# lukedan/libfluid

Hardware: AMD Instinct MI355X
Metric: particle_steps_per_sec (higher is better)
Workload: dtype f32

## Files before the change

libfluid_amd/csrc/common.h:

```cpp
#pragma once

#include <hip/hip_runtime.h>
#include <stdint.h>

#include <string>
#include <vector>

#include "../../include/libfluid_amd.h"
#include "slots.h"

hipError_t lfa_pool_malloc(void **p, size_t bytes);
hipError_t lfa_pool_free(void *p);
void lfa_pool_nosync_begin();
void lfa_pool_nosync_end();
template <typename T> inline hipError_t lfa_hip_malloc(T **p, size_t bytes) { return lfa_pool_malloc((void **)p, bytes); }
#define hipMalloc(p, n) lfa_hip_malloc((p), (n))
#define hipFree(p) lfa_pool_free((void *)(p))
struct lfa_stream_set;
lfa_stream_set *lfa_pool_take_set(int device);
void lfa_pool_park_set(lfa_stream_set *q);

#define LFA_TILE 8
#define LFA_TILE_CELLS 512
#define LFA_HALO 10
#define LFA_HALO_CELLS 1000
#define LFA_WAVE 64

#define CT_AIR 1
#define CT_FLUID 2
#define CT_SOLID 4
#define CT_OUTSIDE 0x80

#define AB_UNKNOWN 0x40
#define AB_FLUID 0x80

struct ParticleSoA {
	uint32_t *key = nullptr;
	float *t[3] = {nullptr, nullptr, nullptr};
	float *v[3] = {nullptr, nullptr, nullptr};
	float *c[9] = {nullptr};
	uint32_t *id = nullptr;
	void *base = nullptr;
};

#define LFA_CLOSED_MAX_UNKNOWNS 64

struct GridDims {
	int nx, ny, nz;
	int ntx, nty, ntz;
	int nt;
};

struct lfa_knobs {
	int mg_no_persist = 0;
	int mg_dist_single = 0;
	int mg_co_fault = 0;
	int mg_no_top = 0;
	int mg_no_prune = 0;
	int mg_dist_levels = 0;
	int mg_no_closed = 0;
	int mg_no_tagged = 0;
};

struct lfa_sim {
	int device = 0;
	lfa_knobs knobs;
	hipStream_t stream = nullptr;
	hipStream_t stream2 = nullptr;
	hipEvent_t ev_fork = nullptr, ev_join = nullptr;
	hipStream_t stream3 = nullptr;
	hipEvent_t ev_cfork = nullptr, ev_cjoin = nullptr;
	bool overlap_correction = true;
	bool corr_in_flight = false;
	bool counts_fresh = false;
	bool move_pending = false;
	bool corr_begun = false;
	bool corr_undo_valid = false;
	uint32_t *corr_ovf = nullptr;
	int corr_parts_tiles = 0;
	GridDims g{};
	size_t nc = 0, ncp = 0;
	lfa_params prm{};
	std::string err;

	size_t np = 0, pcap = 0;
	ParticleSoA pb[2];
	int cur = 0;
	uint32_t *rank = nullptr;
	bool binned = false;

	struct lfa_dist *dist = nullptr;
	int slab_lo = 0, slab_hi = 0;
	int slab_align = 0;
	int *ptiles_all = nullptr;
	int p_off = 0, n_ptiles_all = 0;
	int n_own_first = 0, n_own_last = 0;
	int n_ghost_lo = 0, n_ghost_hi = 0;
	int *halo_tiles = nullptr;
	int n_halo[4] = {0, 0, 0, 0};
	void *xbuf[4] = {nullptr, nullptr, nullptr, nullptr};
	size_t xcap[4] = {0, 0, 0, 0};
	double *dist_red = nullptr;
	size_t np_live = 0;
	bool holes = false;
	size_t arrivals_at = 0, n_arrivals = 0;
	size_t ghost_at[2] = {0, 0}, n_ghost_particles = 0;

	uint32_t *tile_count = nullptr, *tile_start = nullptr;
	uint32_t *tile_flag = nullptr, *tile_scan = nullptr;
	uint32_t *grid_flag = nullptr;
	int *ptiles = nullptr, *dtiles = nullptr;
	int *tile_pslot = nullptr;
	int n_ptiles = 0, n_dtiles = 0;
	uint32_t *scan_tmp = nullptr;
	size_t scan_tmp_len = 0;
	uint32_t *h_pinned = nullptr;

	float *u = nullptr, *v = nullptr, *w = nullptr;
	float *uo = nullptr, *vo = nullptr, *wo = nullptr;
	uint8_t *ctype = nullptr, *solid = nullptr;
	uint32_t *cell_count = nullptr;
// ... 211 lines not shown
struct IngestParams {
	double off[3], h;
};
inline IngestParams lfa_ingest_params(const lfa_sim *s) {
	IngestParams ip;
	for (int k = 0; k < 3; ++k) ip.off[k] = s->prm.grid_offset[k];
	ip.h = s->prm.cell_size;
	return ip;
}

__device__ inline void cell_and_fraction(double pos, double off, double h, int n, int &cell, float &t) {
	double gp = (pos - off) / h;
	double m = gp < 0.0 ? 0.0 : gp;
	int c = m >= (double)n ? n - 1 : (int)m;
	if (c > n - 1) c = n - 1;
	double td = gp - (double)c;
	float tf = (float)td;
	if (!(tf > 0.0f)) tf = 0.0f;
	if (td < 1.0 && tf >= 1.0f) tf = 0.99999994f;
	if (tf > 1.0f) tf = 1.0f;
	cell = c;
	t = tf;
}

__device__ inline void particle_world_position(const GridDims &g, const IngestParams &ip, uint32_t b, float t0, float t1, float t2,
                                               double (&x)[3]) {
	int c[3];
	cell_coords(g, b, c);
	const float t[3] = {t0, t1, t2};
#pragma unroll
	for (int k = 0; k < 3; ++k) x[k] = ip.off[k] + ((double)c[k] + (double)t[k]) * ip.h;
}

__device__ inline void particle_zero_c_set_id(const ParticleSoA &p, size_t d, uint32_t id) {
#pragma unroll
	for (int k = 0; k < 9; ++k) p.c[k][d] = 0.0f;
	p.id[d] = id;
}

#define TC_CHUNKS 8
template <int CH>
__device__ inline void lfa_wave_tile_ranks(const uint32_t (&tile)[CH], uint32_t *tile_count, uint32_t (&my_rank)[CH]) {
	const int lane = threadIdx.x & 63;
	const unsigned long long lt = (1ull << lane) - 1ull;
	unsigned long long todo[CH];
#pragma unroll
	for (int c = 0; c < CH; ++c) {
		todo[c] = __ballot(tile[c] != 0xFFFFFFFFu);
		my_rank[c] = 0;
	}
	for (;;) {
		uint32_t t = 0xFFFFFFFFu;
		bool found = false;
#pragma unroll
		for (int c = 0; c < CH; ++c)
			if (!found && todo[c]) {
				t = __shfl(tile[c], __ffsll((long long)todo[c]) - 1, 64);
				found = true;
			}
		if (!found) break;
		unsigned long long same[CH];
		uint32_t total = 0;
#pragma unroll
		for (int c = 0; c < CH; ++c) {
			same[c] = __ballot(tile[c] == t) & todo[c];
			total += (uint32_t)__popcll(same[c]);
// ... 146 lines not shown
```

libfluid_amd/csrc/core.hip:

```cpp
#include <math.h>

#include <algorithm>
#include <stdarg.h>
#include <stdio.h>
#include <string.h>

#include <mutex>

#include "common.h"
#include "pcg.h"
#include "stream_set.h"

static thread_local std::string g_create_error;

int lfa_fail(lfa_sim *s, int code, const char *fmt, ...) {
	char buf[512];
	va_list ap;
	va_start(ap, fmt);
	vsnprintf(buf, sizeof buf, fmt, ap);
	va_end(ap);
	if (s) s->err = buf;
	else g_create_error = buf;
	return code;
}
// ... 288 lines not shown
		rc = lfa_fail(s, LFA_E_HIP, "hipHostMalloc failed");
	if (rc == LFA_OK) {
		hipLaunchKernelGGL(k_init_ctype, dim3((unsigned)((s->ncp + 255) / 256)), dim3(256), 0, s->stream, s->ctype,
		                   s->solid, s->g, s->ncp);
		if (hipGetLastError() != hipSuccess || hipStreamSynchronize(s->stream) != hipSuccess)
			rc = lfa_fail(s, LFA_E_HIP, "grid initialisation kernel failed (is the code object built for this GPU?)");
	}
	if (rc != LFA_OK) {
		g_create_error = s->err;
		lfa_destroy(s);
		return rc;
	}
	lfa_co_gate_handle(device, +1);
	s->gate_counted = true;
	*out = s;
	return LFA_OK;
}

static void free_soa(ParticleSoA &p) {
	if (p.base) (void)hipFree(p.base);
	p = ParticleSoA();
}

extern "C" void lfa_destroy(lfa_sim *s) {
	if (!s) return;
	(void)hipSetDevice(s->device);
	if (s->gate_counted) lfa_co_gate_handle(s->device, -1);
	if (s->stream) (void)hipStreamSynchronize(s->stream);
	if (s->stream2) (void)hipStreamSynchronize(s->stream2);
	if (s->stream3) (void)hipStreamSynchronize(s->stream3);
	lfa_pool_nosync_begin();
	free_soa(s->pb[0]);
	free_soa(s->pb[1]);
	void *ptrs[] = {s->c_home, s->fine_start, s->corr_ovf, s->tile_clear, s->tile_epoch, s->tile_closed, s->src_cell, s->src_lo, s->src_target, s->src_of, s->src_need, s->src_vel, s->src_slab.words, s->coerce_map, s->grid_flag, s->rank, s->vc_src, s->tile_count, s->tile_start, s->tile_flag, s->tile_scan, s->ptiles_all, s->dtiles, s->halo_tiles, s->dist_red,
	                s->xbuf[0], s->xbuf[1], s->xbuf[2], s->xbuf[3],
	                s->tile_pslot, s->scan_tmp, s->u, s->v, s->w, s->uo, s->vo, s->wo, s->ctype, s->solid,
	                s->cell_count, s->stage, s->acc, s->abits, s->vp, s->vr, s->vz, s->vs, s->vpre, s->vq, s->vs2, s->c_as, s->nbr_table,
	                s->partials, s->frame_part, s->pcg_state, s->pcg_hist, s->level_tiles, s->io_buf, s->raw_scan, s->c_diag, s->c_w[0],
	                s->c_w[1], s->c_w[2], s->c_unk, s->c_pre, s->c_r, s->c_x, s->c_r2, s->c_x2, s->a2inv, s->slot_l1,
	                s->l1_tiles, s->l1_l2, s->tracers.base};
	for (void *p : ptrs)
		if (p) (void)hipFree(p);
	if (s->dist) delete s->dist;
	s->dist = nullptr;
	lfa_mg_free(s);
	lfa_pool_nosync_end();
	for (hipEvent_t e : s->frame_ev)
		if (e) (void)hipEventDestroy(e);
	for (hipEvent_t e : s->sample_ev)
		if (e) (void)hipEventDestroy(e);
	for (hipEvent_t e : s->tracers.ev)
		if (e) (void)hipEventDestroy(e);
	if (s->stream && s->stream2 && s->stream3 && s->ev_fork && s->ev_join && s->ev_cfork && s->ev_cjoin && s->h_pinned) {
		lfa_stream_set *q = new lfa_stream_set();
		q->device = s->device;
		q->stream = s->stream; q->stream2 = s->stream2; q->stream3 = s->stream3;
		q->ev_fork = s->ev_fork; q->ev_join = s->ev_join; q->ev_cfork = s->ev_cfork; q->ev_cjoin = s->ev_cjoin;
		for (int i = 0; i < LFA_EV_COUNT; ++i) q->ev[i] = s->ev[i];
		q->ev_created = s->ev_created;
		q->h_pinned = s->h_pinned;
		lfa_pool_park_set(q);
	} else {
		if (s->h_pinned) (void)hipHostFree(s->h_pinned);
		if (s->ev_created)
			for (auto &e : s->ev) (void)hipEventDestroy(e);
		if (s->ev_fork) (void)hipEventDestroy(s->ev_fork);
		if (s->ev_join) (void)hipEventDestroy(s->ev_join);
// ... 32 lines not shown
	s->prm = *p;
	return LFA_OK;
}
extern "C" int lfa_get_params(const lfa_sim *s, lfa_params *p) {
	if (!s || !p) return LFA_E_INVALID;
	*p = s->prm;
	return LFA_OK;
}
extern "C" int lfa_synchronize(lfa_sim *s) {
	if (!s) return LFA_E_INVALID;
	LFA_HIP(s, hipStreamSynchronize(s->stream));
	if (s->corr_in_flight) LFA_HIP(s, hipStreamSynchronize(s->stream3));
	return LFA_OK;
}
extern "C" void *lfa_stream(lfa_sim *s) { return s ? (void *)s->stream : nullptr; }
extern "C" uint64_t lfa_num_particles(const lfa_sim *s) { return s ? s->np : 0; }

int lfa_ensure_io(lfa_sim *s, size_t bytes) {
	if (bytes <= s->io_cap) return LFA_OK;
	if (s->io_buf) LFA_HIP(s, hipFree(s->io_buf));
	s->io_buf = nullptr;
	s->io_cap = 0;
	hipError_t e = hipMalloc(&s->io_buf, bytes);
	if (e != hipSuccess) return lfa_fail(s, LFA_E_OOM, "hipMalloc(%zu) for the boundary buffer failed", bytes);
	s->io_cap = bytes;
	return LFA_OK;
}

static int alloc_soa(lfa_sim *s, ParticleSoA &p, size_t cap) {
	p = ParticleSoA();
	hipError_t e = hipMalloc(&p.base, cap * 17 * 4);
	if (e != hipSuccess) return lfa_fail(s, LFA_E_OOM, "hipMalloc of particle SoA (%zu particles) failed", cap);
	float *f = (float *)p.base;
	p.key = (uint32_t *)f;
	for (int k = 0; k < 3; ++k) p.t[k] = f + cap * (1 + k);
	for (int k = 0; k < 3; ++k) p.v[k] = f + cap * (4 + k);
	for (int k = 0; k < 9; ++k) p.c[k] = f + cap * (7 + k);
	p.id = (uint32_t *)(f + cap * 16);
	return LFA_OK;
}

int lfa_particles_alloc(lfa_sim *s, size_t n) {
	if (n <= s->pcap) return LFA_OK;
	LFA_HIP(s, hipStreamSynchronize(s->stream));
	const size_t cap = (n + 1023) & ~(size_t)1023;
	ParticleSoA nb[2];
	uint32_t *rank = nullptr, *vc_src = nullptr;
	int rc = alloc_soa(s, nb[0], cap);
	if (rc == LFA_OK) rc = alloc_soa(s, nb[1], cap);
	if (rc == LFA_OK && hipMalloc(&rank, cap * 4) != hipSuccess) rc = lfa_fail(s, LFA_E_OOM, "hipMalloc of the rank array failed");
	if (rc == LFA_OK && hipMalloc(&vc_src, cap * 4) != hipSuccess) rc = lfa_fail(s, LFA_E_OOM, "hipMalloc of the source-index array failed");
	if (rc != LFA_OK) {
		free_soa(nb[0]);
		free_soa(nb[1]);
		if (rank) (void)hipFree(rank);
		if (vc_src) (void)hipFree(vc_src);
		return rc;
	}
	free_soa(s->pb[0]);
	free_soa(s->pb[1]);
	if (s->rank) (void)hipFree(s->rank);
	if (s->vc_src) (void)hipFree(s->vc_src);
	s->pb[0] = nb[0];
	s->pb[1] = nb[1];
	s->rank = rank;
	s->vc_src = vc_src;
	s->vc_pending = false;
	s->pcap = cap;
	return LFA_OK;
}

int lfa_particles_reserve(lfa_sim *s, size_t n_keep, size_t n_total) {
	if (n_total <= s->pcap) return LFA_OK;
	LFA_TRY(lfa_particles_materialize(s));
	LFA_HIP(s, hipStreamSynchronize(s->stream));
	const size_t cap = ((n_total + n_total / 8) + 1023) & ~(size_t)1023;
	ParticleSoA keep = s->pb[s->cur];
	const size_t old_cap = s->pcap;
	s->pb[s->cur] = ParticleSoA();
	s->pcap = 0;
	int rc = lfa_particles_alloc(s, cap);
	if (rc != LFA_OK) {
		s->pb[s->cur] = keep;
		s->pcap = old_cap;
		return rc;
	}
	ParticleSoA &dst = s->pb[s->cur];
	const uint32_t *src_arrays[17];
	uint32_t *dst_arrays[17];
	src_arrays[0] = keep.key; dst_arrays[0] = dst.key;
	for (int k = 0; k < 3; ++k) { src_arrays[1 + k] = (uint32_t *)keep.t[k]; dst_arrays[1 + k] = (uint32_t *)dst.t[k]; }
	for (int k = 0; k < 3; ++k) { src_arrays[4 + k] = (uint32_t *)keep.v[k]; dst_arrays[4 + k] = (uint32_t *)dst.v[k]; }
	for (int k = 0; k < 9; ++k) { src_arrays[7 + k] = (uint32_t *)keep.c[k]; dst_arrays[7 + k] = (uint32_t *)dst.c[k]; }
	src_arrays[16] = keep.id; dst_arrays[16] = dst.id;
	for (int a = 0; a < 17; ++a)
		if (n_keep) LFA_HIP(s, hipMemcpyAsync(dst_arrays[a], src_arrays[a], n_keep * 4, hipMemcpyDeviceToDevice, s->stream));
	LFA_HIP(s, hipStreamSynchronize(s->stream));
	free_soa(keep);
	return LFA_OK;
}

__global__ void k_ingest(const double *aos, size_t n, ParticleSoA p, GridDims g, IngestParams ip, int slab_lo, int slab_hi) {
	size_t i = (size_t)blockIdx.x * blockDim.x + threadIdx.x;
	if (i >= n) return;
	const double *q = aos + i * 19;
	int c[3];
	float t[3];
	cell_and_fraction(q[0], ip.off[0], ip.h, g.nx, c[0], t[0]);
	cell_and_fraction(q[1], ip.off[1], ip.h, g.ny, c[1], t[1]);
	cell_and_fraction(q[2], ip.off[2], ip.h, g.nz, c[2], t[2]);
	p.key[i] = ((c[2] >> 3) >= slab_lo && (c[2] >> 3) < slab_hi) ? blocked_index(g, c[0], c[1], c[2]) : 0xFFFFFFFFu;
#pragma unroll
	for (int k = 0; k < 3; ++k) {
		p.t[k][i] = t[k];
		p.v[k][i] = (float)q[3 + k];
	}
#pragma unroll
	for (int k = 0; k < 9; ++k) p.c[k][i] = (float)q[6 + k];
	p.id[i] = (uint32_t)i;
}

extern "C" int lfa_upload_particles(lfa_sim *s, const void *aos152, uint64_t n) {
	if (!s || (!aos152 && n)) return LFA_E_INVALID;
	s->vc_pending = false;
	s->c_home_valid = false;
	s->move_pending = false;
	s->vmax2_valid = false;
	if (!(s->prm.cell_size > 0.0)) return lfa_fail(s, LFA_E_INVALID, "set cell_size (lfa_set_params) before uploading");
	if (n >= ((uint64_t)1 << 32)) return lfa_fail(s, LFA_E_INVALID, "more than 2^32 particles");
	LFA_HIP(s, hipSetDevice(s->device));
	LFA_TRY(lfa_corr_commit(s));
	LFA_TRY(lfa_particles_alloc(s, n));
	s->np = n;
	s->np_live = n;
	s->next_global_id = n;
	s->binned = false;
	s->system_valid = false;
	s->unknown_count_valid = false;
	s->cur = 0;
	if (n == 0) return LFA_OK;
	LFA_TRY(lfa_ensure_io(s, n * 152));
	LFA_HIP(s, hipMemcpyAsync(s->io_buf, aos152, n * 152, hipMemcpyHostToDevice, s->stream));
	const IngestParams ip = lfa_ingest_params(s);
	hipLaunchKernelGGL(k_ingest, dim3((unsigned)((n + 255) / 256)), dim3(256), 0, s->stream, (const double *)s->io_buf,
	                   (size_t)n, s->pb[0], s->g, ip, s->slab_lo, s->slab_hi);
	LFA_LAUNCH_CHECK(s);
	LFA_HIP(s, hipStreamSynchronize(s->stream));
	return LFA_OK;
}

__global__ void k_valid_flags(const uint32_t *key, size_t n, uint32_t *valid) {
	size_t i = (size_t)blockIdx.x * blockDim.x + threadIdx.x;
	if (i < n) valid[i] = key[i] != 0xFFFFFFFFu ? 1u : 0u;
}
__global__ void k_export_ids(const uint32_t *key, const uint32_t *id, const uint32_t *slot, size_t n, uint32_t *out) {
	size_t i = (size_t)blockIdx.x * blockDim.x + threadIdx.x;
	if (i < n && key[i] != 0xFFFFFFFFu) out[slot ? slot[i] : i] = id[i];
}

__global__ void k_export(double *aos, size_t n, ParticleSoA p, GridDims g, IngestParams ip, int flags, int by_slot, const uint32_t *slot,
                         ParticleSoA old, int have_old, const float *c_home, size_t c_home_stride) {
	size_t i = (size_t)blockIdx.x * blockDim.x + threadIdx.x;
	if (i >= n) return;
	uint32_t b = p.key[i];
	if (slot && b == 0xFFFFFFFFu) return;
	double *q = aos + (by_slot ? (slot ? (size_t)slot[i] : i) : (size_t)p.id[i]) * 19;
	if (flags & LFA_DL_POSITIONS) {
		double x[3];
		particle_world_position(g, ip, b, p.t[0][i], p.t[1][i], p.t[2][i], x);
#pragma unroll
		for (int k = 0; k < 3; ++k) {
			q[k] = x[k];
			q[15 + k] = x[k];
		}
		if (have_old) {
			particle_world_position(g, ip, old.key[i], old.t[0][i], old.t[1][i], old.t[2][i], x);
#pragma unroll
			for (int k = 0; k < 3; ++k) q[15 + k] = x[k];
		}
	}
#pragma unroll
	for (int k = 0; k < 3; ++k) q[3 + k] = (double)p.v[k][i];
#pragma unroll
	for (int k = 0; k < 9; ++k) q[6 + k] = (double)(c_home ? c_home[k * c_home_stride + p.id[i]] : p.c[k][i]);
	if (!(flags & LFA_DL_KEEP_RAW)) ((uint64_t *)q)[18] = raw_from_blocked(g, b);
}

int lfa_slab_download_slots(lfa_sim *s, const uint32_t **slot) {
	*slot = nullptr;
	if (!s->dist || !s->holes || !s->np_live) return LFA_OK;
	hipLaunchKernelGGL(k_valid_flags, dim3((unsigned)((s->np_live + 255) / 256)), dim3(256), 0, s->stream, (const uint32_t *)s->pb[s->cur].key,
	                   s->np_live, s->rank);
	LFA_LAUNCH_CHECK(s);
	uint32_t *tot = (uint32_t *)(s->pcg_state + LFA_DW_SCAN_TOTAL);
	LFA_TRY(lfa_exclusive_scan_u32(s, s->rank, s->rank, s->np_live, tot));
	uint32_t h = 0;
	LFA_HIP(s, hipMemcpyAsync(&h, tot, 4, hipMemcpyDeviceToHost, s->stream));
	LFA_HIP(s, hipStreamSynchronize(s->stream));
	if ((size_t)h != s->np) return lfa_fail(s, LFA_E_INVALID, "slab download: %u resident records but %zu expected", h, s->np);
	*slot = s->rank;
	return LFA_OK;
}

__global__ void __launch_bounds__(256) k_close_holes(size_t n, ParticleSoA src, ParticleSoA dst, const uint32_t *slot, size_t n_dst) {
	const size_t i = (size_t)blockIdx.x * 256 + threadIdx.x;
	if (i >= n || src.key[i] == 0xFFFFFFFFu) return;
	const size_t d = slot[i];
	if (d >= n_dst) return;
	dst.key[d] = src.key[i];
#pragma unroll
	for (int k = 0; k < 3; ++k) {
		dst.t[k][d] = src.t[k][i];
		dst.v[k][d] = src.v[k][i];
	}
#pragma unroll
	for (int k = 0; k < 9; ++k) dst.c[k][d] = src.c[k][i];
	dst.id[d] = src.id[i];
}

int lfa_particles_close_holes(lfa_sim *s, size_t n_rec) {
	hipLaunchKernelGGL(k_valid_flags, dim3((unsigned)((n_rec + 255) >> 8)), dim3(256), 0, s->stream, (const uint32_t *)s->pb[s->cur].key,
	                   n_rec, s->rank);
	LFA_LAUNCH_CHECK(s);
	size_t n_dst = 0;
	LFA_TRY(lfa_scan_total(s, s->rank, s->rank, n_rec, (uint32_t *)(s->pcg_state + LFA_DW_SCAN_TOTAL), LFA_PIN_RESIDENT, &n_dst));
	if (s->binned && n_dst != s->np) return lfa_fail(s, LFA_E_INVALID, "seeding: %u resident records but %zu expected", (uint32_t)n_dst, s->np);
	hipLaunchKernelGGL(k_close_holes, dim3((unsigned)((n_rec + 255) >> 8)), dim3(256), 0, s->stream, n_rec, s->pb[s->cur], s->pb[s->cur ^ 1],
	                   (const uint32_t *)s->rank, n_dst);
	LFA_LAUNCH_CHECK(s);
	s->cur ^= 1;
	s->binned = false;
	s->np = s->np_live = n_dst;
	s->holes = false;
	return LFA_OK;
}

extern "C" int lfa_download_particles(lfa_sim *s, void *aos152, uint64_t n, int flags) {
	if (!s || (!aos152 && n)) return LFA_E_INVALID;
	LFA_HIP(s, hipSetDevice(s->device));
	LFA_TRY(lfa_particles_materialize(s));
	if (n != s->np) return lfa_fail(s, LFA_E_INVALID, "download of %llu particles but %zu are resident",
	                                (unsigned long long)n, s->np);
	if (n == 0) return LFA_OK;
	if (s->dist && !s->binned)
		return lfa_fail(s, LFA_E_INVALID, "slab decomposition: call lfa_hash_particles before downloading particles");
	LFA_TRY(lfa_corr_join(s));
	const uint32_t *slot = nullptr;
	LFA_TRY(lfa_slab_download_slots(s, &slot));
	LFA_TRY(lfa_ensure_io(s, n * 152));
	LFA_HIP(s, hipMemcpyAsync(s->io_buf, aos152, n * 152, hipMemcpyHostToDevice, s->stream));
	const IngestParams ip = lfa_ingest_params(s);
	const size_t n_rec = s->binned ? s->np_live : s->np;
	hipLaunchKernelGGL(k_export, dim3((unsigned)((n_rec + 255) / 256)), dim3(256), 0, s->stream, (double *)s->io_buf,
	                   n_rec, s->pb[s->cur], s->g, ip, flags, s->dist ? 1 : 0, slot, s->pb[s->cur ^ 1],
	                   (s->move_pending && !s->dist) ? 1 : 0, s->c_home_valid ? (const float *)s->c_home : (const float *)nullptr,
	                   s->c_home_cap);
	LFA_LAUNCH_CHECK(s);
	LFA_HIP(s, hipMemcpyAsync(aos152, s->io_buf, n * 152, hipMemcpyDeviceToHost, s->stream));
	LFA_HIP(s, hipStreamSynchronize(s->stream));
	return LFA_OK;
}

extern "C" int lfa_download_particle_ids(lfa_sim *s, uint32_t *ids, uint64_t n) {
	if (!s || (!ids && n)) return LFA_E_INVALID;
	LFA_HIP(s, hipSetDevice(s->device));
	if (n != s->np) return lfa_fail(s, LFA_E_INVALID, "download of %llu ids but %zu particles are resident", (unsigned long long)n, s->np);
	if (n == 0) return LFA_OK;
	LFA_TRY(lfa_corr_join(s));
	if (!s->dist) {
		for (uint64_t i = 0; i < n; ++i) ids[i] = (uint32_t)i;
		return LFA_OK;
	}
	if (!s->binned) return lfa_fail(s, LFA_E_INVALID, "slab decomposition: call lfa_hash_particles before downloading ids");
	const uint32_t *slot = nullptr;
	LFA_TRY(lfa_slab_download_slots(s, &slot));
	if (slot) {
		LFA_TRY(lfa_ensure_io(s, n * 4));
		hipLaunchKernelGGL(k_export_ids, dim3((unsigned)((s->np_live + 255) / 256)), dim3(256), 0, s->stream, (const uint32_t *)s->pb[s->cur].key,
		                   (const uint32_t *)s->pb[s->cur].id, slot, s->np_live, (uint32_t *)s->io_buf);
		LFA_LAUNCH_CHECK(s);
		LFA_HIP(s, hipMemcpyAsync(ids, s->io_buf, n * 4, hipMemcpyDeviceToHost, s->stream));
		LFA_HIP(s, hipStreamSynchronize(s->stream));
		return LFA_OK;
	}
	LFA_HIP(s, hipMemcpyAsync(ids, s->pb[s->cur].id, n * 4, hipMemcpyDeviceToHost, s->stream));
	LFA_HIP(s, hipStreamSynchronize(s->stream));
	return LFA_OK;
}

__device__ inline uint64_t splitmix64(uint64_t x) {
	x ^= x >> 30; x *= 0xBF58476D1CE4E5B9ull;
	x ^= x >> 27; x *= 0x94D049BB133111EBull;
	x ^= x >> 31;
	return x;
}
__global__ void k_seed_block(size_t n, size_t first, ParticleSoA p, GridDims g, IngestParams ip, int lox, int loy, int loz,
                             int ex, int ey, uint64_t seed, int global_ids) {
	size_t j = (size_t)blockIdx.x * blockDim.x + threadIdx.x;
	if (j >= n) return;
	const size_t i = j + first;
	size_t ci = i >> 3;
	int sub = (int)(i & 7);
	int cell[3] = {lox + (int)(ci % ex), loy + (int)((ci / ex) % ey), loz + (int)(ci / ((size_t)ex * ey))};
	int sb[3] = {sub & 1, (sub >> 1) & 1, (sub >> 2) & 1};
	int c[3];
	float t[3];
	const int nn[3] = {g.nx, g.ny, g.nz};
#pragma unroll
	for (int a = 0; a < 3; ++a) {
		uint64_t ctr = 3ull * (uint64_t)i + (uint64_t)a;
		uint64_t x = seed + (ctr + 1ull) * 0x9E3779B97F4A7C15ull;
		double uu = (double)(splitmix64(x) >> 11) * (1.0 / 9007199254740992.0);
		double pos = ip.off[a] + ((double)cell[a] + ((double)sb[a] + uu) * 0.5) * ip.h;
		cell_and_fraction(pos, ip.off[a], ip.h, nn[a], c[a], t[a]);
	}
	p.key[j] = blocked_index(g, c[0], c[1], c[2]);
#pragma unroll
	for (int k = 0; k < 3; ++k) {
		p.t[k][j] = t[k];
		p.v[k][j] = 0.0f;
	}
	particle_zero_c_set_id(p, j, (uint32_t)(global_ids ? i : j));
}

extern "C" int lfa_seed_block(lfa_sim *s, const int64_t lo[3], const int64_t hi[3], uint64_t seed) {
	if (!s || !lo || !hi) return LFA_E_INVALID;
	LFA_TRY(lfa_corr_commit(s));
	LFA_TRY(lfa_particles_materialize(s));
	if (!(s->prm.cell_size > 0.0)) return lfa_fail(s, LFA_E_INVALID, "set cell_size before seeding");
	const int nn[3] = {s->g.nx, s->g.ny, s->g.nz};
	for (int a = 0; a < 3; ++a)
		if (lo[a] < 0 || hi[a] > nn[a] || lo[a] >= hi[a]) return lfa_fail(s, LFA_E_INVALID, "seed block outside the grid");
	int64_t zlo = lo[2], zhi = hi[2];
	if (s->dist) {
		zlo = zlo > (int64_t)s->slab_lo * 8 ? zlo : (int64_t)s->slab_lo * 8;
		zhi = zhi < (int64_t)s->slab_hi * 8 ? zhi : (int64_t)s->slab_hi * 8;
		if (zhi < zlo) zhi = zlo;
	}
	const size_t per_layer = (size_t)(hi[0] - lo[0]) * (size_t)(hi[1] - lo[1]) * 8;
	const size_t n = per_layer * (size_t)(zhi - zlo), first = per_layer * (size_t)(zlo - lo[2]);
	if (per_layer * (size_t)(hi[2] - lo[2]) >= ((size_t)1 << 32)) return lfa_fail(s, LFA_E_INVALID, "more than 2^32 particles");
	LFA_HIP(s, hipSetDevice(s->device));
	LFA_TRY(lfa_particles_alloc(s, n));
	s->next_global_id = per_layer * (size_t)(hi[2] - lo[2]);
	s->np = n;
	s->np_live = n;
	s->c_home_valid = false;
	s->vmax2_valid = false;
	s->binned = false;
	s->grid_valid = false;
	s->system_valid = false;
	s->unknown_count_valid = false;
	s->cur = 0;
	const IngestParams ip = lfa_ingest_params(s);
// ... 84 lines not shown
	if (!s->uo) return lfa_fail(s, LFA_E_INVALID, "no old grid: FLIP P2G has not run");
	return export_cells(s, aos32, s->uo, s->vo, s->wo, true);
}

__global__ void k_import_cells(const CellAos *in, GridDims g, size_t nc, float *u, float *v, float *w, uint8_t *ctype,
                               uint8_t *solid) {
	size_t r = (size_t)blockIdx.x * blockDim.x + threadIdx.x;
	if (r >= nc) return;
	int x = (int)(r % g.nx), y = (int)((r / g.nx) % g.ny), z = (int)(r / ((size_t)g.nx * g.ny));
	uint32_t b = blocked_index(g, x, y, z);
	CellAos c = in[r];
	u[b] = (float)c.vel[0]; v[b] = (float)c.vel[1]; w[b] = (float)c.vel[2];
	ctype[b] = c.type & 7;
	solid[b] = (c.type & CT_SOLID) ? 1 : 0;
}

extern "C" int lfa_upload_cells(lfa_sim *s, const void *aos32) {
	if (!s || !aos32) return LFA_E_INVALID;
	++s->solid_epoch;
	LFA_HIP(s, hipSetDevice(s->device));
	LFA_TRY(lfa_corr_join(s));
	LFA_TRY(lfa_ensure_io(s, s->nc * 32));
	LFA_HIP(s, hipMemcpyAsync(s->io_buf, aos32, s->nc * 32, hipMemcpyHostToDevice, s->stream));
	hipLaunchKernelGGL(k_import_cells, dim3((unsigned)((s->nc + 255) / 256)), dim3(256), 0, s->stream,
	                   (const CellAos *)s->io_buf, s->g, s->nc, s->u, s->v, s->w, s->ctype, s->solid);
	LFA_LAUNCH_CHECK(s);
	LFA_HIP(s, hipStreamSynchronize(s->stream));
	s->grid_valid = false;
	s->bg[0] = s->bg[1] = s->bg[2] = 0.0;
	s->system_valid = false;
	return LFA_OK;
}

__global__ void __launch_bounds__(256) k_tile_count(const uint32_t *key, size_t n, uint32_t *tile_count, uint32_t *rank) {
	const int lane = threadIdx.x & 63;
	const size_t wave = ((size_t)blockIdx.x * blockDim.x + threadIdx.x) >> 6;
	const size_t i0 = wave * (64 * TC_CHUNKS) + lane;
	uint32_t tile[TC_CHUNKS], my_rank[TC_CHUNKS];
#pragma unroll
	for (int c = 0; c < TC_CHUNKS; ++c) {
		const size_t i = i0 + 64 * c;
		const uint32_t k = i < n ? key[i] : 0xFFFFFFFFu;
		tile[c] = k != 0xFFFFFFFFu ? k >> 9 : 0xFFFFFFFFu;
	}
	lfa_wave_tile_ranks(tile, tile_count, my_rank);
#pragma unroll
	for (int c = 0; c < TC_CHUNKS; ++c) {
		const size_t i = i0 + 64 * c;
		if (tile[c] != 0xFFFFFFFFu) rank[i] = my_rank[c];
	}
}

__global__ void k_tile_flags(const uint32_t *tile_count, uint32_t *flag, int nt) {
	int t = blockIdx.x * blockDim.x + threadIdx.x;
	if (t < nt) flag[t] = tile_count[t] > 0 ? 1u : 0u;
}
__global__ void k_compact_tiles(const uint32_t *flag, const uint32_t *scan, int *list, int *slot_of, int nt) {
	int t = blockIdx.x * blockDim.x + threadIdx.x;
	if (t >= nt) return;
	if (flag[t]) {
		list[scan[t]] = t;
		if (slot_of) slot_of[t] = (int)scan[t];
	} else if (slot_of) {
		slot_of[t] = -1;
	}
}
__global__ void k_dilate(const int *ptiles, int n_ptiles, uint32_t *flag, GridDims g) {
	int i = blockIdx.x * blockDim.x + threadIdx.x;
	if (i >= n_ptiles * 27) return;
	int t = ptiles[i / 27], o = i % 27, tx, ty, tz;
	tile_coords(g, t, tx, ty, tz);
	int x = tx + o % 3 - 1, y = ty + (o / 3) % 3 - 1, z = tz + o / 9 - 1;
	if ((unsigned)x < (unsigned)g.ntx && (unsigned)y < (unsigned)g.nty && (unsigned)z < (unsigned)g.ntz)
		flag[x + g.ntx * (y + g.nty * z)] = 1u;
}

__global__ void k_tile_scatter(size_t n, ParticleSoA src, ParticleSoA dst, const uint32_t *rank,
                               const uint32_t *tile_start, const uint32_t *tile_count, int shuffle, uint32_t *from) {
	size_t i = (size_t)blockIdx.x * blockDim.x + threadIdx.x;
	if (i >= n) return;
	uint32_t key = src.key[i], tile = key >> 9, r = rank[i];
	if (key == 0xFFFFFFFFu) return;
	if (shuffle) {
		uint32_t cnt = tile_count[tile];
		if (cnt % 1000003u != 0) r = (uint32_t)(((uint64_t)r * 1000003ull) % cnt);
	}
	size_t d = (size_t)tile_start[tile] + r;
	dst.key[d] = key;
#pragma unroll
	for (int k = 0; k < 3; ++k) dst.t[k][d] = src.t[k][i];
	dst.id[d] = src.id[i];
	from[d] = (uint32_t)i;
}
__global__ void k_c_to_home(size_t n, ParticleSoA p, float *home, size_t stride) {
	size_t i = (size_t)blockIdx.x * blockDim.x + threadIdx.x;
	if (i >= n || p.key[i] == 0xFFFFFFFFu) return;
	const size_t j = p.id[i];
#pragma unroll
	for (int k = 0; k < 9; ++k) home[k * stride + j] = p.c[k][i];
}
__global__ void k_c_from_home(size_t n, ParticleSoA p, const float *home, size_t stride) {
	size_t i = (size_t)blockIdx.x * blockDim.x + threadIdx.x;
	if (i >= n || p.key[i] == 0xFFFFFFFFu) return;
	const size_t j = p.id[i];
#pragma unroll
	for (int k = 0; k < 9; ++k) p.c[k][i] = home[k * stride + j];
}
__global__ void k_gather_vc(size_t n, ParticleSoA old, ParticleSoA cur, const uint32_t *from, int with_c) {
	size_t d = (size_t)blockIdx.x * blockDim.x + threadIdx.x;
	if (d >= n) return;
	const uint32_t i = from[d];
#pragma unroll
	for (int k = 0; k < 3; ++k) cur.v[k][d] = old.v[k][i];
	if (with_c) {
#pragma unroll
		for (int k = 0; k < 9; ++k) cur.c[k][d] = old.c[k][i];
	}
}

#define CC_UNROLL 16
__global__ void __launch_bounds__(256)
k_cell_count(const int *dtiles, int n_dtiles, const uint32_t *key, const uint32_t *tile_start, uint32_t *cell_count) {
	__shared__ uint32_t cnt[LFA_TILE_CELLS];
	for (int slot = blockIdx.x; slot < n_dtiles; slot += gridDim.x) {
		int tile = dtiles[slot];
		cnt[threadIdx.x] = 0;
		cnt[threadIdx.x + 256] = 0;
		__syncthreads();
		uint32_t b = tile_start[tile], e = tile_start[tile + 1];
		for (uint32_t base = b + threadIdx.x; base - threadIdx.x < e; base += 256 * CC_UNROLL) {
			uint32_t k[CC_UNROLL];
#pragma unroll
			for (int q = 0; q < CC_UNROLL; ++q) {
				const uint32_t i = base + 256 * q;
				k[q] = key[i < e ? i : e - 1];
			}
// ... 82 lines not shown
	LFA_LAUNCH_CHECK(s);
	return LFA_OK;
}

int lfa_particles_materialize(lfa_sim *s) {
	if (!s->vc_pending) return LFA_OK;
	LFA_TRY(lfa_corr_commit(s));
	s->vc_pending = false;
	LFA_HIP(s, hipSetDevice(s->device));
	const size_t n = s->np_live;
	if (!n) return LFA_OK;
	hipLaunchKernelGGL(k_gather_vc, dim3((unsigned)((n + 255) / 256)), dim3(256), 0, s->stream, n, s->pb[s->cur ^ 1], s->pb[s->cur],
	                   (const uint32_t *)s->vc_src, s->vc_with_c ? 1 : 0);
	LFA_LAUNCH_CHECK(s);
	return LFA_OK;
}

extern "C" int lfa_hash_particles(lfa_sim *s) { return lfa_hash_particles_impl(s, false); }
int lfa_hash_particles_impl(lfa_sim *s, bool counts_done) {
	if (!s) return LFA_E_INVALID;
	LFA_HIP(s, hipSetDevice(s->device));
	LFA_TRY(lfa_corr_commit(s));
	LFA_TRY(lfa_particles_materialize(s));
	const GridDims &g = s->g;
	const int nt = g.nt, L = g.ntx * g.nty;
	const size_t n = s->binned ? s->np_live : s->np;
	ParticleSoA &src = s->pb[s->cur], &dst = s->pb[s->cur ^ 1];
	const int own_lo = s->slab_lo * L, own_hi = s->slab_hi * L;
	const int all_lo = lfa_has_lo(s) ? own_lo - L : own_lo, all_hi = lfa_has_hi(s) ? own_hi + L : own_hi;

	if (!counts_done) {
		LFA_HIP(s, hipMemsetAsync(s->tile_count, 0, (size_t)(nt + 1) * 4, s->stream));
		if (n) {
			hipLaunchKernelGGL(k_tile_count, dim3((unsigned)((n + 256 * TC_CHUNKS - 1) / (256 * TC_CHUNKS))), dim3(256), 0, s->stream, src.key, n,
			                   s->tile_count, s->rank);
			LFA_LAUNCH_CHECK(s);
		}
	}
	LFA_TRY(lfa_exclusive_scan_u32(s, s->tile_count, s->tile_start, (size_t)nt + 1, nullptr));
	LFA_HIP(s, hipMemcpyAsync(s->h_pinned + LFA_PIN_NP_LIVE, s->tile_start + nt, 4, hipMemcpyDeviceToHost, s->stream));

	hipLaunchKernelGGL(k_tile_flags, dim3((nt + 255) / 256), dim3(256), 0, s->stream, s->tile_count, s->tile_flag, nt);
	LFA_LAUNCH_CHECK(s);
	LFA_TRY(lfa_dist_exchange_tile_layers_u32(s, s->tile_flag));
	hipLaunchKernelGGL(k_fill_i32, dim3((nt + 255) / 256), dim3(256), 0, s->stream, s->tile_pslot, nt, -1);
	LFA_LAUNCH_CHECK(s);
	const bool one_sync = !s->dist;
	if (one_sync) {
		uint32_t *tot = (uint32_t *)s->pcg_state + LFA_DW_N_PTILES;
		LFA_TRY(compact_tiles_async(s, s->tile_flag, 0, nt, s->ptiles_all, s->tile_pslot, tot));
		LFA_HIP(s, hipMemsetAsync(s->tile_flag, 0, (size_t)(nt + 1) * 4, s->stream));
		hipLaunchKernelGGL(k_dilate_slots, dim3((nt + 255) / 256), dim3(256), 0, s->stream, (const int *)s->tile_pslot, s->tile_flag, g);
		LFA_LAUNCH_CHECK(s);
		LFA_TRY(compact_tiles_async(s, s->tile_flag, 0, nt, s->dtiles, nullptr, (uint32_t *)s->pcg_state + LFA_DW_N_DTILES));
		LFA_HIP(s, hipMemcpyAsync(s->h_pinned + LFA_PIN_N_PTILES, tot, 8, hipMemcpyDeviceToHost, s->stream));
		LFA_HIP(s, hipStreamSynchronize(s->stream));
		s->n_ptiles_all = (int)s->h_pinned[LFA_PIN_N_PTILES];
		s->n_dtiles = (int)s->h_pinned[LFA_PIN_N_DTILES];
		s->p_off = 0;
		s->n_ptiles = s->n_ptiles_all;
		s->n_own_first = s->n_own_last = s->n_ghost_lo = s->n_ghost_hi = 0;
		s->ptiles = s->ptiles_all;
	} else {
		uint32_t *tot = (uint32_t *)s->pcg_state + LFA_DW_SLAB;
		LFA_TRY(compact_tiles_async(s, s->tile_flag, all_lo, all_hi, s->ptiles_all, s->tile_pslot, tot));
		int marks[4] = {own_lo, own_lo + L < own_hi ? own_lo + L : own_hi, own_hi - L > own_lo ? own_hi - L : own_lo, own_hi};
		int *didx = s->pcg_state + LFA_DW_SLAB_MARKS;
// ... 17 lines not shown
		LFA_HIP(s, hipMemcpyAsync(s->h_pinned + LFA_PIN_SLAB, tot, LFA_SLAB_WORDS * 4, hipMemcpyDeviceToHost, s->stream));
		LFA_HIP(s, hipStreamSynchronize(s->stream));
		const uint32_t *h = s->h_pinned + LFA_PIN_SLAB;
		s->n_ptiles_all = (int)h[LFA_SLAB_N_PTILES];
		int vals[4];
		for (int k = 0; k < 4; ++k) vals[k] = marks[k] >= all_hi ? s->n_ptiles_all : (int)h[LFA_SLAB_MARK_SCAN + k];
		s->p_off = vals[0];
		s->n_ptiles = vals[3] - vals[0];
		s->n_own_first = vals[1] - vals[0];
		s->n_own_last = vals[3] - vals[2];
		s->n_ghost_lo = s->p_off;
		s->n_ghost_hi = s->n_ptiles_all - vals[3];
		s->ptiles = s->ptiles_all + s->p_off;
		s->n_dtiles = (int)h[LFA_SLAB_N_DTILES];
		for (int w = 0; w < 4; ++w) s->n_halo[w] = (int)h[LFA_SLAB_N_HALO + w];
	}
	s->np_live = s->h_pinned[LFA_PIN_NP_LIVE];
	if (s->dist) s->np = s->np_live;
	s->holes = false;
	s->n_arrivals = 0;
	s->move_pending = false;
	if (n) {
		const dim3 sgrid((unsigned)((n + 255) / 256));
		const bool home = s->prm.simulation_method != LFA_APIC;
		if (home && !s->c_home_valid) {
			LFA_TRY(lfa_c_home_ensure(s, s->dist ? std::max<size_t>(s->pcap, (size_t)s->next_global_id) : s->pcap));
			hipLaunchKernelGGL(k_c_to_home, sgrid, dim3(256), 0, s->stream, n, src, s->c_home, s->c_home_cap);
			LFA_LAUNCH_CHECK(s);
			s->c_home_valid = true;
		} else if (!home && s->c_home_valid) {
			LFA_TRY(lfa_c_home_restore(s));
		}
		hipLaunchKernelGGL(k_tile_scatter, sgrid, dim3(256), 0, s->stream, n, src, dst, s->rank, s->tile_start, s->tile_count,
		                   s->binned ? 0 : 1, s->vc_src);
		LFA_LAUNCH_CHECK(s);
		s->cur ^= 1;
		s->vc_pending = true;
		s->vc_extent = n;
		s->vc_with_c = !home;
	}
	if (s->n_dtiles) {
		int grid = s->n_dtiles < 8192 ? s->n_dtiles : 8192;
		hipLaunchKernelGGL(k_cell_count, dim3(grid), dim3(256), 0, s->stream, s->dtiles, s->n_dtiles,
		                   s->pb[s->cur].key, s->tile_start, s->cell_count);
		LFA_LAUNCH_CHECK(s);
	}
	s->binned = true;
	s->system_valid = false;
	s->unknown_count_valid = false;
	return LFA_OK;
}

int lfa_dist_build_halo_lists(lfa_sim *s, const uint32_t *flag, int *lists, int n[4]) {
	const int L = s->g.ntx * s->g.nty;
	const int lo[4] = {s->slab_lo * L, (s->slab_hi - 1) * L, (s->slab_lo - 1) * L, s->slab_hi * L};
	const bool on[4] = {lfa_has_lo(s), lfa_has_hi(s), lfa_has_lo(s), lfa_has_hi(s)};
	uint32_t *tot = (uint32_t *)s->pcg_state + LFA_DW_SLAB + LFA_SLAB_N_HALO;
	LFA_HIP(s, hipMemsetAsync(tot, 0, 16, s->stream));
	for (int w = 0; w < 4; ++w)
		if (on[w]) LFA_TRY(compact_tiles_async(s, flag, lo[w], lo[w] + L, lists + (size_t)w * L, nullptr, tot + w));
	LFA_HIP(s, hipMemcpyAsync(s->h_pinned + LFA_PIN_SLAB + LFA_SLAB_N_HALO, tot, 16, hipMemcpyDeviceToHost, s->stream));
	LFA_HIP(s, hipStreamSynchronize(s->stream));
	for (int w = 0; w < 4; ++w) n[w] = (int)s->h_pinned[LFA_PIN_SLAB + LFA_SLAB_N_HALO + w];
	return LFA_OK;
}

__global__ void k_raw_unknown_flags(GridDims g, size_t nc, const uint32_t *cell_count, const uint32_t *tile_flag,
                                    uint32_t *flag, int z0, int z1) {
	size_t r = (size_t)blockIdx.x * blockDim.x + threadIdx.x;
	if (r >= nc) return;
	int x = (int)(r % g.nx), y = (int)((r / g.nx) % g.ny), z = (int)(r / ((size_t)g.nx * g.ny));
	uint32_t b = blocked_index(g, x, y, z);
	flag[r] = (z >= z0 && z < z1 && tile_flag[b >> 9] && cell_count[b] > 0) ? 1u : 0u;
}

int lfa_number_unknowns(lfa_sim *s) {
	if (s->unknown_count_valid) return LFA_OK;
// ... 245 lines not shown
```

libfluid_amd/csrc/dist.hip:

```cpp
#include <dlfcn.h>
#include <fcntl.h>
#include <math.h>
#include <sched.h>
#include <string.h>
#include <sys/mman.h>
#include <sys/stat.h>
#include <unistd.h>
#include <rccl/rccl.h>

#include <algorithm>
#include <atomic>
#include <chrono>
#include <condition_variable>
#include <mutex>
#include <vector>

#include "common.h"

namespace {
struct FieldList {
	void *ptr[8];
	int words[8];
	int n, tile_words;
};
// ... 254 lines not shown
}

int lfa_dist_allreduce(lfa_sim *s, const double *partials, int n, int slot, bool is_max) {
	hipLaunchKernelGGL(k_reduce_partials, dim3(1), dim3(256), 0, s->stream, partials, n, s->dist_red + slot, is_max ? 1 : 0);
	LFA_LAUNCH_CHECK(s);
	return s->dist->allreduce(s, s->dist_red + slot, 1, is_max);
}


double *lfa_dist_gather_buf(lfa_sim *s, int parity) { return s->dist_red + LFA_DR_GATHER + (size_t)parity * (3 * s->dist->nranks + 1); }
int lfa_dist_gather_pair(lfa_sim *s, const double *pmax, int n_max, const double *psum, int n_sum, int parity) {
	return lfa_dist_gather_triple(s, pmax, n_max, psum, n_sum, nullptr, 0, parity);
}
int lfa_dist_gather_triple(lfa_sim *s, const double *pmax, int n_max, const double *psum, int n_sum, const double *psum2, int n_sum2,
                           int parity) {
	const int n = s->dist->nranks;
	if (n > 32) return lfa_fail(s, LFA_E_UNSUPPORTED, "more than 32 slabs");
	double *out = lfa_dist_gather_buf(s, parity);
	hipLaunchKernelGGL(k_gather_pair, dim3(1), dim3(256), 0, s->stream, pmax, n_max, psum, n_sum, psum2, n_sum2, out, n, s->dist->rank,
	                   (const int *)s->pcg_state);
	LFA_LAUNCH_CHECK(s);
	return s->dist->allreduce_buf(s, out, (size_t)3 * n + 1, LFA_RED_F64, false);
}

namespace {
__global__ void __launch_bounds__(256)
k_pack_leavers(size_t n, ParticleSoA p, int tiles_per_layer, int slab_lo, int slab_hi, uint32_t *counters, uint32_t *buf_lo,
               uint32_t *buf_hi, int count_only, const float *c_home, size_t c_home_stride, ParticleSoA pvc, const uint32_t *from,
               int c_deferred) {
	size_t i = (size_t)blockIdx.x * blockDim.x + threadIdx.x;
	int dest = -1;
	uint32_t key = 0xFFFFFFFFu;
	if (i < n) {
		key = p.key[i];
		if (key != 0xFFFFFFFFu) {
			const int tz = (int)(key >> 9) / tiles_per_layer;
			dest = tz < slab_lo ? 0 : (tz >= slab_hi ? 1 : -1);
		}
	}
	const int lane = threadIdx.x & 63;
#pragma unroll
	for (int d = 0; d < 2; ++d) {
		const unsigned long long m = __ballot(dest == d);
		if (!m) continue;
		const int leader = __ffsll((long long)m) - 1;
		uint32_t base = 0;
		if (lane == leader) base = atomicAdd(&counters[d], (uint32_t)__popcll(m));
		base = __shfl(base, leader, 64);
		if (dest == d && !count_only) {
			uint32_t *rec = (d == 0 ? buf_lo : buf_hi) + (size_t)(base + (uint32_t)__popcll(m & ((1ull << lane) - 1ull))) * 17;
			rec[0] = key;
			const size_t j = from ? (size_t)from[i] : i;
#pragma unroll
			for (int k = 0; k < 3; ++k) {
				rec[1 + k] = __float_as_uint(p.t[k][i]);
				rec[4 + k] = __float_as_uint(from ? pvc.v[k][j] : p.v[k][i]);
			}
#pragma unroll
			for (int k = 0; k < 9; ++k)
				rec[7 + k] = __float_as_uint(c_home ? c_home[k * c_home_stride + p.id[i]]
				                                    : (from && c_deferred ? pvc.c[k][j] : p.c[k][i]));
			rec[16] = p.id[i];
			p.key[i] = 0xFFFFFFFFu;
		}
	}
}
__global__ void k_offset_u32(const uint32_t *in, uint32_t *out, int n, uint32_t base) {
	int i = blockIdx.x * blockDim.x + threadIdx.x;
	if (i < n) out[i] = in[i] + base;
}
__global__ void __launch_bounds__(256) k_unpack_arrivals(size_t n, const uint32_t *buf, ParticleSoA p, size_t at, float *c_home,
                                                         size_t c_home_stride, ParticleSoA pvc, uint32_t *from, size_t ext) {
	size_t i = (size_t)blockIdx.x * blockDim.x + threadIdx.x;
	if (i >= n) return;
	const uint32_t *rec = buf + i * 17;
	const size_t d = at + i, e = from ? ext + i : d;
	const ParticleSoA &q = from ? pvc : p;
	p.key[d] = rec[0];
#pragma unroll
	for (int k = 0; k < 3; ++k) {
		p.t[k][d] = __uint_as_float(rec[1 + k]);
		q.v[k][e] = __uint_as_float(rec[4 + k]);
	}
#pragma unroll
	for (int k = 0; k < 9; ++k) {
		if (c_home) c_home[k * c_home_stride + rec[16]] = __uint_as_float(rec[7 + k]);
		else q.c[k][e] = __uint_as_float(rec[7 + k]);
	}
	p.id[d] = rec[16];
	if (from) from[d] = (uint32_t)e;
}
}

int lfa_particles_reserve(lfa_sim *s, size_t n_keep, size_t n_total);

int lfa_dist_migrate(lfa_sim *s, bool vc_dead) {
	if (!s->dist) return LFA_OK;
	(void)vc_dead;
	const size_t n = s->binned ? s->np_live : s->np;
	uint32_t *cnt = (uint32_t *)(s->dist_red + LFA_DR_MIGRATE_COUNTS);
	LFA_HIP(s, hipMemsetAsync(cnt, 0, 16, s->stream));
	const int tpl = s->g.ntx * s->g.nty;
	const dim3 grid((unsigned)((n + 255) / 256 ? (n + 255) / 256 : 1));
	ParticleSoA &p = s->pb[s->cur];
	hipLaunchKernelGGL(k_pack_leavers, grid, dim3(256), 0, s->stream, n, p, tpl, s->slab_lo, s->slab_hi, cnt, (uint32_t *)nullptr,
	                   (uint32_t *)nullptr, 1, (const float *)nullptr, (size_t)0, p, (const uint32_t *)nullptr, 0);
	LFA_LAUNCH_CHECK(s);
	LFA_TRY(s->dist->exchange(s, lfa_has_lo(s) ? cnt + 0 : nullptr, lfa_has_lo(s) ? 4 : 0, lfa_has_lo(s) ? cnt + 2 : nullptr,
	                          lfa_has_lo(s) ? 4 : 0, lfa_has_hi(s) ? cnt + 1 : nullptr, lfa_has_hi(s) ? 4 : 0,
	                          lfa_has_hi(s) ? cnt + 3 : nullptr, lfa_has_hi(s) ? 4 : 0));
	uint32_t h[4];
	LFA_HIP(s, hipMemcpyAsync(h, cnt, 16, hipMemcpyDeviceToHost, s->stream));
	LFA_HIP(s, hipStreamSynchronize(s->stream));
	if (!lfa_has_lo(s)) h[0] = h[2] = 0;
	if (!lfa_has_hi(s)) h[1] = h[3] = 0;
	for (int w = 0; w < 4; ++w) LFA_TRY(lfa_dist_ensure_xbuf(s, w, (size_t)h[w] * 68));
// ... 34 lines not shown
	if (!s->dist) return LFA_OK;
	const int L = s->g.ntx * s->g.nty;
	const size_t own_lo = (size_t)s->slab_lo * L, own_hi = (size_t)s->slab_hi * L;
	LFA_TRY(lfa_dist_exchange_tile_layers_u32(s, s->tile_count));
	uint32_t hs[4];
	const size_t marks[4] = {own_lo, own_lo + L < own_hi ? own_lo + L : own_hi, own_hi - L > own_lo ? own_hi - L : own_lo, own_hi};
	for (int k = 0; k < 4; ++k)
		LFA_HIP(s, hipMemcpyAsync(&hs[k], s->tile_start + marks[k], 4, hipMemcpyDeviceToHost, s->stream));
	uint32_t *tot = (uint32_t *)(s->dist_red + LFA_DR_GHOST_TOTALS);
	size_t n_g[2] = {0, 0};
	uint32_t hg[2] = {0, 0};
	if (lfa_has_lo(s)) LFA_TRY(lfa_exclusive_scan_u32(s, s->tile_count + own_lo - L, s->tile_scan + own_lo - L, (size_t)L, tot));
	if (lfa_has_hi(s)) LFA_TRY(lfa_exclusive_scan_u32(s, s->tile_count + own_hi, s->tile_scan + own_hi, (size_t)L, tot + 1));
	LFA_HIP(s, hipMemcpyAsync(hg, tot, 8, hipMemcpyDeviceToHost, s->stream));
	LFA_HIP(s, hipStreamSynchronize(s->stream));
	n_g[0] = lfa_has_lo(s) ? hg[0] : 0;
	n_g[1] = lfa_has_hi(s) ? hg[1] : 0;
	const size_t n = s->np_live;
	LFA_TRY(lfa_particles_reserve(s, n, n + n_g[0] + n_g[1]));
	ParticleSoA &p = s->pb[s->cur];
	const size_t at_hi = n, at_lo = n + n_g[1];
	if (lfa_has_hi(s)) {
		hipLaunchKernelGGL(k_offset_u32, dim3((L + 255) / 256), dim3(256), 0, s->stream, s->tile_scan + own_hi, s->tile_start + own_hi,
		                   L, (uint32_t)at_hi);
		LFA_LAUNCH_CHECK(s);
	}
	if (lfa_has_lo(s)) {
		hipLaunchKernelGGL(k_offset_u32, dim3((L + 255) / 256), dim3(256), 0, s->stream, s->tile_scan + own_lo - L,
		                   s->tile_start + own_lo - L, L, (uint32_t)at_lo);
		LFA_LAUNCH_CHECK(s);
	}
	const size_t send_lo_at = hs[0], send_lo_n = lfa_has_lo(s) ? hs[1] - hs[0] : 0;
	const size_t send_hi_at = hs[2], send_hi_n = lfa_has_hi(s) ? hs[3] - hs[2] : 0;
	uint32_t *arr[5] = {p.key, (uint32_t *)p.t[0], (uint32_t *)p.t[1], (uint32_t *)p.t[2], p.id};
	for (int a = 0; a < 5; ++a)
		LFA_TRY(s->dist->exchange(s, arr[a] + send_lo_at, send_lo_n * 4, arr[a] + at_lo, n_g[0] * 4, arr[a] + send_hi_at,
		                          send_hi_n * 4, arr[a] + at_hi, n_g[1] * 4));
	s->ghost_at[0] = at_lo;
	s->ghost_at[1] = at_hi;
	s->n_ghost_particles = n_g[0] + n_g[1];
	return LFA_OK;
}

struct lfa_hub {
	int n = 0;
	std::mutex m;
	std::condition_variable cv;
	int arrived = 0;
	long generation = 0;
	struct Mail {
		const void *lo = nullptr, *hi = nullptr;
		size_t n_lo = 0, n_hi = 0;
		double val = 0.0;
		std::vector<uint8_t> buf;
	};
	std::vector<Mail> mail;
	bool failed = false;
	bool barrier() {
		std::unique_lock<std::mutex> lk(m);
		if (failed) return false;
		long gen = generation;
		if (++arrived == n) {
			arrived = 0;
			++generation;
			cv.notify_all();
			return true;
		}
		if (!cv.wait_for(lk, std::chrono::seconds(20), [&] { return generation != gen || failed; }) || failed) {
			failed = true;
			cv.notify_all();
// ... 493 lines not shown
```

libfluid_amd/csrc/frame.hip:

```cpp
#include "common.h"

#include <cmath>
#include <cstring>
#include <limits>

#define FRAME_GRID_CAP 1024
#define FRAME_FIELDS 11
#define FRAME_PART_DOUBLES ((FRAME_GRID_CAP + 1) * FRAME_FIELDS)

struct FrameAcc {
	double e, ea, m, lo[3], hi[3];
	unsigned long long n, nin;
};
__device__ inline FrameAcc frame_neutral() {
	FrameAcc a;
	a.e = a.ea = a.m = 0.0;
#pragma unroll
	for (int k = 0; k < 3; ++k) {
		a.lo[k] = INFINITY;
		a.hi[k] = -INFINITY;
	}
	a.n = a.nin = 0ull;
	return a;
}
// ... 42 lines not shown
	a.m = f[2 * stride];
#pragma unroll
	for (int k = 0; k < 3; ++k) {
		a.lo[k] = f[(3 + k) * stride];
		a.hi[k] = f[(6 + k) * stride];
	}
	a.n = (unsigned long long)__double_as_longlong(f[9 * stride]);
	a.nin = (unsigned long long)__double_as_longlong(f[10 * stride]);
	return a;
}

__device__ inline void frame_block_reduce(FrameAcc &a) {
	__shared__ double lds[4][FRAME_FIELDS];
#pragma unroll
	for (int o = 32; o > 0; o >>= 1) {
		const FrameAcc b = frame_shfl_xor(a, o);
		frame_merge(a, b);
	}
	if ((threadIdx.x & 63) == 0) frame_store(a, lds[threadIdx.x >> 6], 1);
	__syncthreads();
	if (threadIdx.x == 0)
		for (int w = 1; w < 4; ++w) {
			const FrameAcc b = frame_load(lds[w], 1);
			frame_merge(a, b);
		}
}

struct FrameParams {
	IngestParams ip;
	double g[3];
};

template <bool OCC>
__global__ void __launch_bounds__(256) k_frame_stats(size_t n, const uint32_t *key, const float *t0, const float *t1, const float *t2,
                                                     const float *v0, const float *v1, const float *v2, GridDims g, FrameParams q,
                                                     uint32_t *occupation, double *part) {
	FrameAcc a = frame_neutral();
	for (size_t i = (size_t)blockIdx.x * 256 + threadIdx.x; i < n; i += (size_t)gridDim.x * 256) {
		const uint32_t b = key[i];
		if (b == 0xFFFFFFFFu) continue;
		double x[3];
		particle_world_position(g, q.ip, b, t0[i], t1[i], t2[i], x);
		const double vx = (double)v0[i], vy = (double)v1[i], vz = (double)v2[i];
		double sq = vx * vx;
		sq += vy * vy;
		sq += vz * vz;
		double dot = q.g[0] * x[0];
		dot += q.g[1] * x[1];
		dot += q.g[2] * x[2];
		const double half = 0.5 * sq;
		a.e += half - dot;
		a.ea += half + fabs(dot);
		a.m = sq > a.m ? sq : a.m;
#pragma unroll
		for (int k = 0; k < 3; ++k) {
			a.lo[k] = x[k] < a.lo[k] ? x[k] : a.lo[k];
			a.hi[k] = x[k] > a.hi[k] ? x[k] : a.hi[k];
		}
		++a.n;
		const int ix = (int)((x[0] - q.ip.off[0]) / q.ip.h), iy = (int)((x[1] - q.ip.off[1]) / q.ip.h), iz = (int)((x[2] - q.ip.off[2]) / q.ip.h);
		if (in_grid(g, ix, iy, iz)) {
			++a.nin;
			if (OCC) atomicAdd(&occupation[(size_t)ix + (size_t)g.nx * ((size_t)iy + (size_t)g.ny * (size_t)iz)], 1u);
		}
	}
	frame_block_reduce(a);
	if (threadIdx.x == 0) frame_store(a, part + blockIdx.x, FRAME_GRID_CAP);
}

__global__ void __launch_bounds__(256) k_frame_finish(int n_part, double *part) {
	FrameAcc a = frame_neutral();
	for (int i = (int)threadIdx.x; i < n_part; i += 256) {
		const FrameAcc b = frame_load(part + i, FRAME_GRID_CAP);
		frame_merge(a, b);
	}
	frame_block_reduce(a);
	if (threadIdx.x == 0) frame_store(a, part + (size_t)FRAME_GRID_CAP * FRAME_FIELDS, 1);
}

__global__ void __launch_bounds__(256) k_export_positions(double *xyz, size_t n, size_t n_out, const uint32_t *key, const float *t0,
                                                          const float *t1, const float *t2, const uint32_t *id, GridDims g, IngestParams ip,
                                                          int by_slot, const uint32_t *slot) {
	const size_t i = (size_t)blockIdx.x * 256 + threadIdx.x;
	if (i >= n) return;
	const uint32_t b = key[i];
	if (b == 0xFFFFFFFFu) return;
	const size_t d = by_slot ? (slot ? (size_t)slot[i] : i) : (size_t)id[i];
	if (d >= n_out) return;
	double x[3];
	particle_world_position(g, ip, b, t0[i], t1[i], t2[i], x);
#pragma unroll
	for (int k = 0; k < 3; ++k) xyz[3 * d + k] = x[k];
}

static void frame_neutral_host(struct lfa_frame_stats *out) {
	memset(out, 0, sizeof(*out));
	for (int k = 0; k < 3; ++k) {
		out->lo[k] = std::numeric_limits<double>::infinity();
		out->hi[k] = -std::numeric_limits<double>::infinity();
	}
}

extern "C" int lfa_frame_stats(lfa_sim *s, struct lfa_frame_stats *out, uint32_t *occupation) {
	if (!s) return LFA_E_INVALID;
	if (!out) return lfa_fail(s, LFA_E_INVALID, "lfa_frame_stats: out is NULL");
	if (!(s->prm.cell_size > 0.0)) return lfa_fail(s, LFA_E_INVALID, "set cell_size (lfa_set_params) before lfa_frame_stats");
	LFA_HIP(s, hipSetDevice(s->device));
	LFA_TRY(lfa_particles_materialize(s));
	if (s->np == 0) {
		frame_neutral_host(out);
		if (occupation) memset(occupation, 0, s->nc * 4);
		s->frame_timed = false;
		return LFA_OK;
	}
	if (s->dist && !s->binned)
		return lfa_fail(s, LFA_E_INVALID, "slab decomposition: call lfa_hash_particles before downloading particles");
	LFA_TRY(lfa_corr_join(s));
	if (!s->frame_part) {
		hipError_t e = hipMalloc(&s->frame_part, (size_t)FRAME_PART_DOUBLES * 8);
		if (e != hipSuccess) return lfa_fail(s, LFA_E_OOM, "hipMalloc of the frame summary's partials failed");
	}
	for (hipEvent_t &e : s->frame_ev)
		if (!e) LFA_HIP(s, hipEventCreate(&e));
	if (occupation) LFA_TRY(lfa_ensure_io(s, s->nc * 4));
	FrameParams q;
	q.ip = lfa_ingest_params(s);
	for (int k = 0; k < 3; ++k) q.g[k] = s->prm.gravity[k];
	const size_t n_rec = s->binned ? s->np_live : s->np;
	size_t blocks = (n_rec + 255) / 256;
	if (blocks > FRAME_GRID_CAP) blocks = FRAME_GRID_CAP;
	const ParticleSoA &p = s->pb[s->cur];
	s->frame_timed = false;
	LFA_HIP(s, hipEventRecord(s->frame_ev[0], s->stream));
	if (occupation) {
		LFA_HIP(s, hipMemsetAsync(s->io_buf, 0, s->nc * 4, s->stream));
		hipLaunchKernelGGL(k_frame_stats<true>, dim3((unsigned)blocks), dim3(256), 0, s->stream, n_rec, (const uint32_t *)p.key,
		                   (const float *)p.t[0], (const float *)p.t[1], (const float *)p.t[2], (const float *)p.v[0], (const float *)p.v[1],
		                   (const float *)p.v[2], s->g, q, (uint32_t *)s->io_buf, s->frame_part);
	} else {
		hipLaunchKernelGGL(k_frame_stats<false>, dim3((unsigned)blocks), dim3(256), 0, s->stream, n_rec, (const uint32_t *)p.key,
		                   (const float *)p.t[0], (const float *)p.t[1], (const float *)p.t[2], (const float *)p.v[0], (const float *)p.v[1],
		                   (const float *)p.v[2], s->g, q, (uint32_t *)nullptr, s->frame_part);
	}
	LFA_LAUNCH_CHECK(s);
	hipLaunchKernelGGL(k_frame_finish, dim3(1), dim3(256), 0, s->stream, (int)blocks, s->frame_part);
	LFA_LAUNCH_CHECK(s);
	LFA_HIP(s, hipEventRecord(s->frame_ev[1], s->stream));
	double r[FRAME_FIELDS];
	LFA_HIP(s, hipMemcpyAsync(r, s->frame_part + (size_t)FRAME_GRID_CAP * FRAME_FIELDS, sizeof(r), hipMemcpyDeviceToHost, s->stream));
	if (occupation) LFA_HIP(s, hipMemcpyAsync(occupation, s->io_buf, s->nc * 4, hipMemcpyDeviceToHost, s->stream));
	LFA_HIP(s, hipStreamSynchronize(s->stream));
	s->frame_timed = true;
	out->energy = r[0];
	out->energy_abs = r[1];
	out->max_speed2 = r[2];
	for (int k = 0; k < 3; ++k) {
		out->lo[k] = r[3 + k];
		out->hi[k] = r[6 + k];
	}
	memcpy(&out->n, &r[9], 8);
	memcpy(&out->n_in_grid, &r[10], 8);
	return LFA_OK;
}

extern "C" int lfa_frame_stats_time(lfa_sim *s, double *ms) {
	if (!s || !ms) return LFA_E_INVALID;
	if (!s->frame_timed) return lfa_fail(s, LFA_E_INVALID, "lfa_frame_stats_time: no lfa_frame_stats has run on the device");
	LFA_HIP(s, hipSetDevice(s->device));
	float f = 0.0f;
	LFA_HIP(s, hipEventElapsedTime(&f, s->frame_ev[0], s->frame_ev[1]));
	*ms = (double)f;
	return LFA_OK;
}

extern "C" int lfa_download_positions(lfa_sim *s, double *xyz, uint64_t n) {
	if (!s || (!xyz && n)) return LFA_E_INVALID;
	if (!(s->prm.cell_size > 0.0)) return lfa_fail(s, LFA_E_INVALID, "set cell_size (lfa_set_params) before lfa_download_positions");
	LFA_HIP(s, hipSetDevice(s->device));
	LFA_TRY(lfa_particles_materialize(s));
	if (n != s->np) return lfa_fail(s, LFA_E_INVALID, "download of %llu positions but %zu particles are resident",
	                                (unsigned long long)n, s->np);
	if (n == 0) return LFA_OK;
	if (s->dist && !s->binned)
		return lfa_fail(s, LFA_E_INVALID, "slab decomposition: call lfa_hash_particles before downloading particles");
	LFA_TRY(lfa_corr_join(s));
	const uint32_t *slot = nullptr;
	LFA_TRY(lfa_slab_download_slots(s, &slot));
	LFA_TRY(lfa_ensure_io(s, n * 24));
	const IngestParams ip = lfa_ingest_params(s);
	const size_t n_rec = s->binned ? s->np_live : s->np;
	const ParticleSoA &p = s->pb[s->cur];
	hipLaunchKernelGGL(k_export_positions, dim3((unsigned)((n_rec + 255) / 256)), dim3(256), 0, s->stream, (double *)s->io_buf, n_rec,
	                   (size_t)n, (const uint32_t *)p.key, (const float *)p.t[0], (const float *)p.t[1], (const float *)p.t[2],
	                   (const uint32_t *)p.id, s->g, ip, s->dist ? 1 : 0, slot);
	LFA_LAUNCH_CHECK(s);
	LFA_HIP(s, hipMemcpyAsync(xyz, s->io_buf, n * 24, hipMemcpyDeviceToHost, s->stream));
	LFA_HIP(s, hipStreamSynchronize(s->stream));
	return LFA_OK;
}
```

libfluid_amd/csrc/grid_ops.hip:

```cpp
#include "common.h"
#include "pcg.h"

namespace {

struct GridView {
	GridDims g;
	const uint8_t *ctype, *solid;
	const uint32_t *cell_count, *tile_flag;
};
__device__ inline bool is_unknown_at(const GridView &gv, int x, int y, int z) {
	if (!in_grid(gv.g, x, y, z)) return false;
	uint32_t b = blocked_index(gv.g, x, y, z);
	return gv.tile_flag[b >> 9] && gv.cell_count[b] > 0;
}

#define HT_UNKNOWN 8
__device__ inline void stage_halo_types(const GridView &gv, int tx, int ty, int tz, uint8_t *H) {
	for (int i = threadIdx.x; i < LFA_HALO_CELLS; i += 256) {
		const int x = 8 * tx + i % 10 - 1, y = 8 * ty + (i / 10) % 10 - 1, z = 8 * tz + i / 100 - 1;
		uint8_t t = CT_SOLID;
		if (in_grid(gv.g, x, y, z)) {
			const uint32_t b = blocked_index(gv.g, x, y, z);
			if (gv.tile_flag[b >> 9]) t = (uint8_t)((gv.ctype[b] & 7) | (gv.cell_count[b] > 0 ? HT_UNKNOWN : 0));
			else t = gv.solid[b] ? CT_SOLID : CT_AIR;
// ... 262 lines not shown
#pragma unroll
			for (int k = 0; k < 8; ++k) {
				const float px = f[0] - (float)(k & 1), py = f[1] - (float)((k >> 1) & 1), pz = f[2] - (float)(k >> 2);
				const float sx = px > 0.f ? -1.f : 1.f, sy = py > 0.f ? -1.f : 1.f, sz = pz > 0.f ? -1.f : 1.f;
				const float ax = 1.f - fabsf(px), ay = 1.f - fabsf(py), az = 1.f - fabsf(pz);
				cx = cx + (sx * ay * az * gp.inv_h) * s[k];
				cy = cy + (ax * sy * az * gp.inv_h) * s[k];
				cz = cz + (ax * ay * sz * gp.inv_h) * s[k];
			}
			cvec[3 * comp] = cx; cvec[3 * comp + 1] = cy; cvec[3 * comp + 2] = cz;
		}
	}
	if (METHOD == LFA_FLIP_BLEND) {
#pragma unroll
		for (int k = 0; k < 3; ++k) vout[k] = vnew[k] + (vp[k] - vold[k]) * gp.blend;
	} else {
#pragma unroll
		for (int k = 0; k < 3; ++k) vout[k] = vnew[k];
	}
	return vout[0] * vout[0] + vout[1] * vout[1] + vout[2] * vout[2];
}
template <int METHOD>
__device__ inline void g2p_store(const ParticleSoA &p, uint32_t i, const float (&vout)[3], const float (&cvec)[9]) {
#pragma unroll
	for (int k = 0; k < 3; ++k) p.v[k][i] = vout[k];
	if (METHOD == LFA_APIC) {
#pragma unroll
		for (int k = 0; k < 9; ++k) p.c[k][i] = cvec[k];
	}
}
template <int METHOD, typename Corner, typename Fetch>
__device__ inline float g2p_particle(const ParticleSoA &p, uint32_t i, const ParticleSoA &pold, uint32_t j, const G2PParams &gp,
                                    Corner &&corner, Fetch &&fetch) {
	const float t[3] = {p.t[0][i], p.t[1][i], p.t[2][i]};
	float vp[3] = {0.0f, 0.0f, 0.0f}, vout[3], cvec[9];
	if (METHOD == LFA_FLIP_BLEND) {
#pragma unroll
		for (int k = 0; k < 3; ++k) vp[k] = pold.v[k][j];
	}
	const float v2 = g2p_transfer<METHOD>(t, vp, gp, corner, fetch, vout, cvec);
	g2p_store<METHOD>(p, i, vout, cvec);
	return v2;
}

template <typename A, typename B, typename C, typename D>
__device__ inline void lfa_take_delivery(A &a, B &b, C &c, D &d) {
	asm volatile("" : "+v"(a), "+v"(b), "+v"(c), "+v"(d) : : "memory");
}

#define G2P_LV_CAP 256
#ifndef G2P_THREADS
#define G2P_THREADS 256
#endif
template <int METHOD, bool STALE>
__global__ void __launch_bounds__(G2P_THREADS)
k_g2p(const int *ptiles, int n_ptiles, GridDims g, ParticleSoA p, const uint32_t *tile_start, const float *u,
      const float *v, const float *w, const float *uo, const float *vo, const float *wo, G2PParams gp, uint32_t *leavers,
      uint32_t *n_leavers, ParticleSoA pold, const uint32_t *from, uint32_t *vmax2_bits) {
	constexpr int NF = METHOD == LFA_FLIP_BLEND ? 6 : 3;
	__shared__ float lds[NF * LFA_HALO_CELLS];
	__shared__ uint32_t lv[STALE ? G2P_LV_CAP : 1], lv_n, lv_base;
	float vmax2 = 0.0f;
	for (int slot = blockIdx.x; slot < n_ptiles; slot += gridDim.x) {
		const int tile = ptiles[slot];
		int tx, ty, tz;
		tile_coords(g, tile, tx, ty, tz);
		constexpr int HR = (LFA_HALO_CELLS + G2P_THREADS - 1) / G2P_THREADS;
// ... 4 lines not shown
#pragma unroll
		for (int r = 0; r < HR; ++r) {
			const int i = min((int)threadIdx.x + G2P_THREADS * r, LFA_HALO_CELLS - 1);
			const int x = tx * 8 + i % 10 - 1, y = ty * 8 + (i / 10) % 10 - 1, z = tz * 8 + i / 100 - 1;
			hb[r] = blocked_index(g, min(max(x, 0), g.nx - 1), min(max(y, 0), g.ny - 1), min(max(z, 0), g.nz - 1));
		}
#pragma unroll
		for (int r = 0; r < HR; ++r) {
#pragma unroll
			for (int f = 0; f < NF; ++f) hv[r][f] = F[f][hb[r]];
		}
		__syncthreads();
		if (STALE && threadIdx.x == 0) lv_n = 0;
#pragma unroll
		for (int r = 0; r < HR; ++r) {
			const int i = (int)threadIdx.x + G2P_THREADS * r;
			if (i < LFA_HALO_CELLS) {
				const int c[3] = {tx * 8 + i % 10 - 1, ty * 8 + (i / 10) % 10 - 1, tz * 8 + i / 100 - 1};
#pragma unroll
				for (int f = 0; f < NF; ++f) {
					const int comp = f % 3;
					lds[f * LFA_HALO_CELLS + i] = (c[comp] < 0 || c[comp] >= nn[comp] - 1) ? 0.0f : hv[r][f];
				}
			}
		}
		__syncthreads();
		const uint32_t beg = tile_start[tile], end = tile_start[tile + 1];
		constexpr bool FLIP = METHOD == LFA_FLIP_BLEND;
		struct Regs {
			uint32_t key;
			float t[3], vp[3];
		} cur, nxt;
		auto load = [&](uint32_t i, uint32_t j, Regs &r) {
			r.key = p.key[i];
#pragma unroll
			for (int k = 0; k < 3; ++k) {
				r.t[k] = p.t[k][i];
				r.vp[k] = FLIP ? pold.v[k][j] : 0.0f;
			}
		};
		if (beg < end) {
			const uint32_t last = end - 1;
			uint32_t i = beg + threadIdx.x;
			uint32_t jn = 0;
			if (FLIP) jn = from ? from[min(i + G2P_THREADS, last)] : min(i + G2P_THREADS, last);
			load(min(i, last), FLIP ? (from ? from[min(i, last)] : min(i, last)) : 0u, cur);
			lfa_take_delivery(cur.key, cur.t[0], cur.t[1], cur.t[2]);
			if (FLIP) lfa_take_delivery(jn, cur.vp[0], cur.vp[1], cur.vp[2]);
			for (; i < end; i += G2P_THREADS) {
				const uint32_t in = min(i + G2P_THREADS, last);
				uint32_t jnn = 0;
				if (FLIP) jnn = from ? from[min(i + 2 * G2P_THREADS, last)] : min(i + 2 * G2P_THREADS, last);
				load(in, jn, nxt);
				jn = jnn;
				const uint32_t key = cur.key;
				const bool leaver = STALE && (int)(key >> 9) != tile;
				float vout[3], cvec[9];
				if (leaver) {
					const uint32_t at = atomicAdd(&lv_n, 1u);
					if (at < G2P_LV_CAP) lv[at] = i;
					else leavers[atomicAdd(n_leavers, 1u)] = i;
				} else {
					const int l = (int)(key & 511);
					const int cell = ((l & 7) + 1) + 10 * (((l >> 3) & 7) + 1) + 100 * ((l >> 6) + 1);
					const float v2 = g2p_transfer<METHOD>(
					    cur.t, cur.vp, gp, [&](int b0, int b1, int b2) { return cell + b0 + 10 * b1 + 100 * b2; },
					    [&](int field, int, int base, int k) { return lds[field * LFA_HALO_CELLS + base + (k & 1) + 10 * ((k >> 1) & 1) + 100 * (k >> 2)]; },
					    vout, cvec);
					vmax2 = fmaxf(vmax2, v2);
				}
// ... 2 lines not shown
				if (FLIP) lfa_take_delivery(jn, cur.vp[0], cur.vp[1], cur.vp[2]);
				if (!leaver) g2p_store<METHOD>(p, i, vout, cvec);
			}
		}
		if (STALE) {
			__syncthreads();
			const uint32_t n = lv_n < G2P_LV_CAP ? lv_n : G2P_LV_CAP;
			if (threadIdx.x == 0 && n) lv_base = atomicAdd(n_leavers, n);
			__syncthreads();
			for (uint32_t k = threadIdx.x; k < n; k += G2P_THREADS) leavers[lv_base + k] = lv[k];
		}
	}
	vmax2 = wave_max(vmax2);
	if ((threadIdx.x & 63) == 0 && vmax2 > 0.0f) atomicMax(vmax2_bits, __float_as_uint(vmax2));
}

__global__ void k_g2p_append_range(uint32_t *leavers, uint32_t *n_leavers, uint32_t first, uint32_t count) {
	__shared__ uint32_t base;
	const uint32_t i = blockIdx.x * blockDim.x + threadIdx.x;
	const uint32_t mine = count - min(count, blockIdx.x * blockDim.x);
	if (threadIdx.x == 0) base = atomicAdd(n_leavers, mine < blockDim.x ? mine : blockDim.x);
	__syncthreads();
	if (i < count) leavers[base + threadIdx.x] = first + i;
}

template <int METHOD>
__global__ void __launch_bounds__(256)
k_g2p_leavers(GridDims g, ParticleSoA p, const float *u, const float *v, const float *w, const float *uo, const float *vo,
              const float *wo, G2PParams gp, const uint32_t *leavers, const uint32_t *n_leavers, ParticleSoA pold, const uint32_t *from,
              uint32_t *vmax2_bits) {
	const uint32_t n = *n_leavers;
	float vmax2 = 0.0f;
	for (uint32_t k = blockIdx.x * 256 + threadIdx.x; k < n; k += gridDim.x * 256) {
		const uint32_t i = leavers[k], key = p.key[i];
		if (key == 0xFFFFFFFFu) continue;
		const int tile = (int)(key >> 9), l = (int)(key & 511);
		int tx, ty, tz;
		tile_coords(g, tile, tx, ty, tz);
		const int cx = tx * 8 + (l & 7), cy = ty * 8 + ((l >> 3) & 7), cz = tz * 8 + (l >> 6);
		const float *F[6] = {u, v, w, uo, vo, wo};
		const float v2 = g2p_particle<METHOD>(
		    p, i, pold, (METHOD == LFA_FLIP_BLEND && from) ? from[i] : i, gp,
		    [&](int b0, int b1, int b2) { return make_int3(cx + b0, cy + b1, cz + b2); },
		    [&](int field, int comp, int3 c, int k) { return clamped_sample(g, F[field], comp, c.x + (k & 1), c.y + ((k >> 1) & 1), c.z + (k >> 2)); });
		vmax2 = fmaxf(vmax2, v2);
	}
	vmax2 = wave_max(vmax2);
	if ((threadIdx.x & 63) == 0 && vmax2 > 0.0f) atomicMax(vmax2_bits, __float_as_uint(vmax2));
}
}

static int grid_blocks(int n) { return n < 16384 ? (n > 0 ? n : 1) : 16384; }

int lfa_dist_refresh_grid(lfa_sim *s, bool with_topology) {
	if (!s->dist) return LFA_OK;
	void *f[9];
	int e[9], n = 0;
	f[n] = s->u; e[n++] = 4;
	f[n] = s->v; e[n++] = 4;
	f[n] = s->w; e[n++] = 4;
	if (with_topology) {
		f[n] = s->ctype; e[n++] = 1;
		f[n] = s->cell_count; e[n++] = 4;
		if (s->prm.simulation_method == LFA_FLIP_BLEND && s->uo) {
			f[n] = s->uo; e[n++] = 4;
			f[n] = s->vo; e[n++] = 4;
			f[n] = s->wo; e[n++] = 4;
// ... 147 lines not shown
```

libfluid_amd/csrc/mesher.hip:

```cpp
#include "common.h"
#include "mc_tables.h"

#include <math.h>
#include <stdio.h>
#include <string.h>

#include <algorithm>

struct lfa_mesher {
	int device = 0;
	hipStream_t stream = nullptr;
	uint64_t n[3] = {0, 0, 0};
	uint64_t z0 = 0, nzl = 0, s_lo = 0, s_hi = 0, c_lo = 0, c_hi = 0, own_lo = 0;
	uint32_t *ids = nullptr;
	size_t ncell = 0, npts = 0;
	double off[3] = {0, 0, 0}, cs = 0.0, extent = 0.5;
	uint64_t radius = 2;
	double *values = nullptr;
	uint32_t *cell_start = nullptr;
	uint32_t *cell_fill = nullptr;
	uint32_t *order = nullptr;
	double *pos = nullptr;
	double *spos = nullptr;
	uint8_t *blk_flag = nullptr;
// ... 612 lines not shown
		if (q) MSH_HIP(m, hipFree(q));
	m->pos = nullptr; m->order = nullptr; m->spos = nullptr; m->ids = nullptr;
	m->pcap = 0;
	MSH_HIP(m, hipMalloc(&m->pos, n * 24));
	MSH_HIP(m, hipMalloc(&m->spos, n * 24));
	MSH_HIP(m, hipMalloc(&m->order, n * 4));
	MSH_HIP(m, hipMalloc(&m->ids, n * 4));
	m->pcap = n;
	return LFA_OK;
}

extern "C" int lfa_mesher_sample_ids(lfa_mesher *m, const double *positions, const uint32_t *ids, uint64_t n, double r) {
	if (!m || (!positions && n)) return LFA_E_INVALID;
	if (n >= (1ull << 32)) return mfail(m, LFA_E_INVALID, "lfa_mesher_sample: more than 2^32 particles");
	MSH_HIP(m, hipSetDevice(m->device));
	int rc = ensure_particle_capacity(m, (size_t)n);
	if (rc != LFA_OK) return rc;
	if (n) MSH_HIP(m, hipMemcpyAsync(m->pos, positions, (size_t)n * 24, hipMemcpyHostToDevice, m->stream));
	if (n && ids) MSH_HIP(m, hipMemcpyAsync(m->ids, ids, (size_t)n * 4, hipMemcpyHostToDevice, m->stream));
	rc = sample_device_positions(m, m->pos, n, r, ids ? (const uint32_t *)m->ids : (const uint32_t *)nullptr);
	if (rc != LFA_OK) return rc;
	MSH_HIP(m, hipStreamSynchronize(m->stream));
	return LFA_OK;
}
extern "C" int lfa_mesher_sample(lfa_mesher *m, const double *positions, uint64_t n, double r) {
	return lfa_mesher_sample_ids(m, positions, nullptr, n, r);
}

__global__ void k_sim_positions(ParticleSoA p, size_t first, size_t n, size_t out_at, int by_slot, GridDims g, double ox, double oy,
                                double oz, double h, double *pos, uint32_t *ids) {
	const size_t k = (size_t)blockIdx.x * blockDim.x + threadIdx.x;
	if (k >= n) return;
	const size_t i = first + k;
	const uint32_t b = p.key[i];
	const int tile = (int)(b >> 9), l = (int)(b & 511);
	int tx, ty, tz;
	tile_coords(g, tile, tx, ty, tz);
	const int c[3] = {tx * 8 + (l & 7), ty * 8 + ((l >> 3) & 7), tz * 8 + (l >> 6)};
	const double off[3] = {ox, oy, oz};
	const size_t at = by_slot ? out_at + k : (size_t)p.id[i];
	double *q = pos + 3 * at;
#pragma unroll
	for (int d = 0; d < 3; ++d) q[d] = off[d] + ((double)c[d] + (double)p.t[d][i]) * h;
	if (by_slot) ids[at] = p.id[i];
}

extern "C" int lfa_mesher_sample_sim(lfa_mesher *m, lfa_sim *s, double r) {
	if (!m || !s) return LFA_E_INVALID;
	if (s->device != m->device) return mfail(m, LFA_E_INVALID, "lfa_mesher_sample_sim: handles live on different devices");
	MSH_HIP(m, hipSetDevice(m->device));
	if (lfa_corr_join(s) < 0) return mfail(m, LFA_E_HIP, "lfa_mesher_sample_sim: joining the simulation's position correction failed");
	size_t n = s->np, n_live = s->np;
	if (s->dist) {
		if (!s->binned || s->holes) return mfail(m, LFA_E_INVALID, "lfa_mesher_sample_sim: slab decomposition: call lfa_hash_particles first");
		const double h = s->prm.cell_size, lo = s->prm.grid_offset[2] + h * 8.0 * (double)(lfa_has_lo(s) ? s->slab_lo - 1 : 0),
		             hi = s->prm.grid_offset[2] + h * 8.0 * (double)(lfa_has_hi(s) ? s->slab_hi + 1 : s->g.ntz);
		const double need_lo = m->off[2] + m->cs * ((double)m->s_lo - (double)m->radius), need_hi = m->off[2] + m->cs * ((double)m->s_hi + (double)m->radius);
		if ((lfa_has_lo(s) && need_lo < lo) || (lfa_has_hi(s) && need_hi > hi))
			return mfail(m, LFA_E_INVALID, "lfa_mesher_sample_sim: the mesher window reaches beyond this rank's slab and ghost tile layers");
		if (lfa_particles_materialize(s) != LFA_OK || lfa_dist_exchange_ghost_particles(s) != LFA_OK)
			return mfail(m, LFA_E_HIP, lfa_last_error(s));
		n_live = s->np_live;
		n = n_live + s->n_ghost_particles;
	}
	if (n >= (1ull << 32)) return mfail(m, LFA_E_INVALID, "lfa_mesher_sample_sim: more than 2^32 particles");
	int rc = ensure_particle_capacity(m, n);
	if (rc != LFA_OK) return rc;
	MSH_HIP(m, hipStreamSynchronize(s->stream));
	if (n) {
		hipLaunchKernelGGL(k_sim_positions, dim3((unsigned)((n + 255) / 256)), dim3(256), 0, m->stream, s->pb[s->cur], (size_t)0, n,
		                   (size_t)0, s->dist ? 1 : 0, s->g, s->prm.grid_offset[0], s->prm.grid_offset[1], s->prm.grid_offset[2],
		                   s->prm.cell_size, m->pos, m->ids);
		MSH_HIP(m, hipGetLastError());
	}
	rc = sample_device_positions(m, m->pos, n, r, s->dist ? (const uint32_t *)m->ids : (const uint32_t *)nullptr);
	if (rc != LFA_OK) return rc;
// ... 356 lines not shown
```

libfluid_amd/csrc/p2g.hip:

```cpp
#include "common.h"

namespace {

__device__ inline void axis_bf(float t, bool own, int &b, float &f) {
	if (own) {
		b = t >= 1.0f ? 0 : -1;
		f = t >= 1.0f ? 0.0f : t;
	} else {
		b = t < 0.5f ? -1 : 0;
		f = t < 0.5f ? t + 0.5f : t - 0.5f;
	}
}

template <bool APIC, bool QUIRK, typename AddFn>
__device__ inline void scatter_particle(int lx, int ly, int lz, const float t[3], const float v[3], const float c[9],
                                        float hworld, int rot, AddFn add) {
	if (QUIRK) {
#pragma unroll
		for (int comp = 0; comp < 3; ++comp) {
			float w1[3][3], a1[3][3];
			const float *cc = c + 3 * comp;
#pragma unroll
			for (int a = 0; a < 3; ++a)
#pragma unroll
// ... 72 lines not shown
		            wz[2] = {r2 ? wz_hi : wz_lo, r2 ? wz_lo : wz_hi};
		const uint32_t ox[2] = {r0 ? 8u : 0u, r0 ? 0u : 8u}, oy[2] = {r1 ? 80u : 0u, r1 ? 0u : 80u};
		const uint32_t oz[2] = {a0 + (r2 ? 800u : 0u), a0 + (r2 ? 0u : 800u)};
		const uint32_t oxy[4] = {ox[0] + oy[0], ox[1] + oy[0], ox[0] + oy[1], ox[1] + oy[1]};
		float ax[2] = {0.f, 0.f}, ay[2] = {0.f, 0.f}, az[2] = {0.f, 0.f};
		const float vs = v[comp] * sv;
		if (APIC) {
			const float *cc = c + 3 * comp;
			const float ax_lo = (-hworld * cc[0] * f[0]) * sv, ax_hi = (-hworld * cc[0] * (f[0] - 1.0f)) * sv;
			const float ay_lo = (-hworld * cc[1] * f[1]) * sv, ay_hi = (-hworld * cc[1] * (f[1] - 1.0f)) * sv;
			const float az_lo = (-hworld * cc[2] * f[2]) * sv, az_hi = (-hworld * cc[2] * (f[2] - 1.0f)) * sv;
			ax[0] = r0 ? ax_hi : ax_lo; ax[1] = r0 ? ax_lo : ax_hi;
			ay[0] = r1 ? ay_hi : ay_lo; ay[1] = r1 ? ay_lo : ay_hi;
			az[0] = r2 ? az_hi : az_lo; az[1] = r2 ? az_lo : az_hi;
		}
#pragma unroll
		for (int n = 0; n < 8; ++n) {
			const int i = n & 1, j = (n >> 1) & 1, k = n >> 2;
			const float wgt = (wx[i] * wy[j]) * wz[k];
			const float val = APIC ? vs + ((ax[i] + ay[j]) + az[k]) : vs;
			unsigned long long *a = (unsigned long long *)((char *)acc + (oxy[i + 2 * j] + oz[k]));
			atomicAdd(a, conv(wgt * val));
			atomicAdd(a + LFA_HALO_CELLS, conv(wgt));
		}
	}
}

struct ParticleRegs {
	uint32_t key;
	float t[3], v[3], c[9];
};
template <bool APIC>
__device__ inline void load_particle(const ParticleSoA &p, const ParticleSoA &pvc, uint32_t i, uint32_t j, ParticleRegs &r) {
	r.key = p.key[i];
#pragma unroll
	for (int k = 0; k < 3; ++k) {
		r.t[k] = p.t[k][i];
		r.v[k] = pvc.v[k][j];
	}
	if (APIC) {
#pragma unroll
		for (int k = 0; k < 9; ++k) r.c[k] = pvc.c[k][j];
	}
}

#ifndef P2G_THREADS
#define P2G_THREADS 512
#endif
template <bool APIC, bool QUIRK>
__global__ void __launch_bounds__(P2G_THREADS)
k_p2g_binned(const int *ptiles, int n_ptiles, ParticleSoA p, ParticleSoA pvc, const uint32_t *from, const uint32_t *tile_start,
             float *stage, float hworld, int rot_mask) {
	__shared__ unsigned long long acc[6 * LFA_HALO_CELLS];
	for (int slot = blockIdx.x; slot < n_ptiles; slot += gridDim.x) {
		const int tile = ptiles[slot];
		for (int i = threadIdx.x; i < 6 * LFA_HALO_CELLS; i += P2G_THREADS) acc[i] = 0ull;
		__syncthreads();
		const uint32_t beg = tile_start[tile], end = tile_start[tile + 1];
		ParticleRegs cur, nxt;
		uint32_t i = beg + threadIdx.x;
		uint32_t jn = i + P2G_THREADS < end ? (from ? from[i + P2G_THREADS] : i + P2G_THREADS) : 0u;
		if (i < end) load_particle<APIC>(p, pvc, i, from ? from[i] : i, cur);
		for (; i < end; i += P2G_THREADS) {
			const uint32_t in = i + P2G_THREADS;
			const uint32_t jnn = in + P2G_THREADS < end ? (from ? from[in + P2G_THREADS] : in + P2G_THREADS) : 0u;
			if (in < end) load_particle<APIC>(p, pvc, in, jn, nxt);
			jn = jnn;
			const int l = (int)(cur.key & 511);
			if (!QUIRK)
				scatter_particle_lds<APIC>(acc, l & 7, (l >> 3) & 7, l >> 6, cur.t, cur.v, cur.c, hworld, (int)(threadIdx.x & rot_mask));
// ... 2 lines not shown
				                       [&](int comp, int hx, int hy, int hz, float wv, float wgt) {
					                       unsigned long long *a = acc + comp * 2 * LFA_HALO_CELLS + hx + 10 * hy + 100 * hz;
					                       atomicAdd(a, to_fixed(wv, P2G_FIX_SCALE_V));
					                       atomicAdd(a + LFA_HALO_CELLS, to_fixed(wgt, P2G_FIX_SCALE_W));
				                       });
			cur = nxt;
		}
		__syncthreads();
		float *out = stage + (size_t)slot * 6 * LFA_HALO_CELLS;
		for (int k = threadIdx.x; k < 6 * LFA_HALO_CELLS; k += P2G_THREADS) {
			const int ch = k / LFA_HALO_CELLS;
			out[k] = (float)((double)(long long)acc[ch * LFA_HALO_CELLS + lfa_stage_source(k - ch * LFA_HALO_CELLS)] *
			                 ((ch & 1) ? 1.0 / P2G_FIX_SCALE_W : 1.0 / P2G_FIX_SCALE_V));
		}
		__syncthreads();
	}
}

__global__ void k_zero_acc(const int *dtiles, int n_dtiles, float *acc, size_t ncp) {
	int slot = blockIdx.x;
	if (slot >= n_dtiles) return;
	size_t base = (size_t)dtiles[slot] * LFA_TILE_CELLS;
	for (int k = 0; k < 6; ++k) {
		acc[k * ncp + base + threadIdx.x] = 0.0f;
		acc[k * ncp + base + 256 + threadIdx.x] = 0.0f;
	}
}

template <bool APIC, bool QUIRK>
__global__ void __launch_bounds__(256)
k_p2g_atomic(size_t n, ParticleSoA p, float *acc, size_t ncp, GridDims g, float hworld) {
	size_t i = (size_t)blockIdx.x * blockDim.x + threadIdx.x;
	if (i >= n) return;
	const uint32_t key = p.key[i];
	const int tile = (int)(key >> 9), l = (int)(key & 511);
	int tx, ty, tz;
	tile_coords(g, tile, tx, ty, tz);
	const int cx = tx * 8 + (l & 7), cy = ty * 8 + ((l >> 3) & 7), cz = tz * 8 + (l >> 6);
	float t[3] = {p.t[0][i], p.t[1][i], p.t[2][i]};
	float v[3] = {p.v[0][i], p.v[1][i], p.v[2][i]};
	float c[9];
	if (APIC) {
#pragma unroll
		for (int k = 0; k < 9; ++k) c[k] = p.c[k][i];
	}
	scatter_particle<APIC, QUIRK>(0, 0, 0, t, v, c, hworld, 0, [&](int comp, int hx, int hy, int hz, float wv, float wgt) {
		int x = cx + hx - 1, y = cy + hy - 1, z = cz + hz - 1;
		if (!in_grid(g, x, y, z)) return;
		size_t b = blocked_index(g, x, y, z);
		unsafeAtomicAdd(acc + (size_t)(2 * comp) * ncp + b, wv);
		unsafeAtomicAdd(acc + (size_t)(2 * comp + 1) * ncp + b, wgt);
	});
}

struct FinalizeParams {
	int method;
	float g[3];
	int fuse_gravity;
};

template <bool BINNED>
__global__ void __launch_bounds__(256)
k_p2g_finalize(const int *dtiles, int n_dtiles, GridDims g, const int *tile_pslot, const float *stage, const float *acc,
               size_t ncp, const uint32_t *cell_count, const uint8_t *solid, float *u, float *v, float *w, float *uo,
               float *vo, float *wo, uint8_t *ctype, FinalizeParams fp) {
	__shared__ int ps27[27];
	for (int slot = blockIdx.x; slot < n_dtiles; slot += gridDim.x) {
		const int tile = dtiles[slot];
		int tx, ty, tz;
		tile_coords(g, tile, tx, ty, tz);
		if (BINNED) {
			__syncthreads();
// ... 240 lines not shown
```

libfluid_amd/csrc/particles.hip:

```cpp
#include <math.h>

#include <algorithm>
#include <utility>

#include "common.h"
#include "pcg.h"

namespace {

__device__ inline bool solid_or_outside(const GridDims &g, const uint8_t *solid, int x, int y, int z) {
	if (!in_grid(g, x, y, z)) return true;
	return solid[blocked_index(g, x, y, z)] != 0;
}

__device__ inline void collide(const GridDims &g, const uint8_t *solid, double from[3], double to[3], double skin) {
	for (int bounce = 0; bounce < 3; ++bounce) {
		bool hit = false;
		double diff[3], inv[3], t[3];
		int cur[3], last[3], adv[3];
#pragma unroll
		for (int d = 0; d < 3; ++d) {
			cur[d] = (int)floor(from[d]);
			last[d] = (int)floor(to[d]);
			diff[d] = to[d] - from[d];
// ... 101 lines not shown
};

__global__ void __launch_bounds__(256) k_tile_has_solid(const uint8_t *solid, int nt, uint8_t *tile_solid) {
	for (int t = blockIdx.x; t < nt; t += gridDim.x) {
		const uint8_t *c = solid + (size_t)t * LFA_TILE_CELLS;
		const int any = __syncthreads_or((c[threadIdx.x] | c[threadIdx.x + 256]) != 0);
		if (threadIdx.x == 0) tile_solid[t] = (uint8_t)(any ? 1 : 0);
	}
}
__global__ void k_tile_clear(GridDims g, const uint8_t *tile_solid, uint8_t *tile_clear) {
	const int t = blockIdx.x * blockDim.x + threadIdx.x;
	if (t >= g.nt) return;
	int tx, ty, tz;
	tile_coords(g, t, tx, ty, tz);
	int any = 0;
	for (int dz = -1; dz <= 1; ++dz)
		for (int dy = -1; dy <= 1; ++dy)
			for (int dx = -1; dx <= 1; ++dx) {
				const int x = tx + dx, y = ty + dy, z = tz + dz;
				if ((unsigned)x < (unsigned)g.ntx && (unsigned)y < (unsigned)g.nty && (unsigned)z < (unsigned)g.ntz)
					any |= tile_solid[x + g.ntx * (y + g.nty * z)];
			}
	tile_clear[t] = (uint8_t)(any ? 0 : 1);
}

struct AdvectSlot {
	uint32_t key;
	float t[3];
	float v[3];
	uint32_t clear;
	uint32_t src;
};
__device__ inline void advect_load(size_t i, const ParticleSoA &p, AdvectSlot &a) {
	a.key = p.key[i];
#pragma unroll
	for (int d = 0; d < 3; ++d) {
		a.t[d] = p.t[d][i];
		a.v[d] = p.v[d][i];
	}
}
template <bool COERCE>
__device__ inline void advect_load_by_key(const uint8_t *coerce_map, const uint8_t *tile_clear, AdvectSlot &a) {
	const uint32_t k = a.key != 0xFFFFFFFFu ? a.key : 0u;
	a.clear = tile_clear[k >> 9];
	a.src = COERCE ? (uint32_t)coerce_map[k] : 0u;
}
template <bool COERCE>
__device__ inline uint32_t advect_move(AdvectSlot &a, const GridDims &g, const uint8_t *solid, const MoveParams &mp, const float *src_vel) {
	const uint32_t key = a.key;
	if (key == 0xFFFFFFFFu) return key;
	int c[3];
	cell_of_key(g, key, c);
	const int nn[3] = {g.nx, g.ny, g.nz};
	if (COERCE && a.src) {
#pragma unroll
		for (int d = 0; d < 3; ++d) a.v[d] = src_vel[3 * (a.src - 1) + d];
	}
	double from[3], to[3];
#pragma unroll
	for (int d = 0; d < 3; ++d) {
		from[d] = (double)c[d] + (double)a.t[d];
		double x = from[d] + (double)a.v[d] * mp.dt_over_h;
		const double lo = mp.skin, hi = (double)nn[d] - mp.skin;
		to[d] = x < lo ? lo : (hi < x ? hi : x);
	}
	const bool open_water = (a.clear & 1) && fabs(to[0] - from[0]) < 7.0 && fabs(to[1] - from[1]) < 7.0 &&
	                        fabs(to[2] - from[2]) < 7.0;
	if (!open_water && mp.collide) collide(g, solid, from, to, mp.skin);
	int nc[3];
#pragma unroll
	for (int d = 0; d < 3; ++d) split_position(to[d], nn[d], nc[d], a.t[d]);
	a.key = blocked_index(g, nc[0], nc[1], nc[2]);
	return a.key;
}
template <bool COERCE>
__device__ inline void advect_store(size_t i, const ParticleSoA &p, const MoveParams &mp, const AdvectSlot &a) {
	if (a.key == 0xFFFFFFFFu) return;
	p.key[i] = a.key;
#pragma unroll
	for (int d = 0; d < 3; ++d) p.t[d][i] = a.t[d];
	if (COERCE && a.src) {
#pragma unroll
		for (int d = 0; d < 3; ++d) p.v[d][i] = a.v[d];
		if (mp.c_home) {
			const size_t j = p.id[i];
#pragma unroll
			for (int k = 0; k < 9; ++k) mp.c_home[k * mp.c_home_stride + j] = 0.0f;
		} else {
#pragma unroll
			for (int k = 0; k < 9; ++k) p.c[k][i] = 0.0f;
		}
	}
}

template <bool COERCE>
__global__ void __launch_bounds__(256)
k_advect_collide(size_t n, ParticleSoA p, GridDims g, const uint8_t *solid, MoveParams mp, const uint8_t *coerce_map,
                 const float *src_vel, const uint8_t *tile_clear) {
	const size_t i = (size_t)blockIdx.x * blockDim.x + threadIdx.x;
	if (i >= n) return;
	AdvectSlot a;
	advect_load(i, p, a);
	advect_load_by_key<COERCE>(coerce_map, tile_clear, a);
	advect_move<COERCE>(a, g, solid, mp, src_vel);
	advect_store<COERCE>(i, p, mp, a);
}

#define AC_CHUNKS 8
template <bool COERCE>
__global__ void __launch_bounds__(256)
k_advect_collide_count(size_t n, ParticleSoA p, GridDims g, const uint8_t *solid, MoveParams mp, const uint8_t *coerce_map,
                       const float *src_vel, const uint8_t *tile_clear, uint32_t *tile_count, uint32_t *rank) {
	const int lane = threadIdx.x & 63;
// ... 44 lines not shown
#define FB_N (FBX * FB * FBZ)
#define FB_ROWS (FB * FBZ)
#define FINE_CAP 5632
#define FINE_CAP_BIG 12288
#define FIDX_THREADS 512
#define FIDX_CNT (((FT3 + 1 + FIDX_THREADS - 1) / FIDX_THREADS) * FIDX_THREADS)
#define FIDX_STAGE 4608

__device__ inline int fine_coord(int l, float t) {
	const int f = (int)(((float)l + t) * FT_INV);
	return f < FT - 1 ? f : FT - 1;
}
__device__ inline int fine_coord_x(int l, float t) {
	const int f = (int)(((float)l + t) * FTX_INV);
	return f < FTX - 1 ? f : FTX - 1;
}
__device__ inline float4 fine_record(int lx, int ly, int lz, float t0, float t1, float t2, uint32_t index) {
	const uint32_t b0 = (__float_as_uint(t0) & 0x3FFFFFFFu) | ((uint32_t)(lx & 3) << 30);
	const uint32_t b1 = (__float_as_uint(t1) & 0x3FFFFFFFu) | ((uint32_t)(lx >> 2) << 31) | ((uint32_t)(ly & 1) << 30);
	const uint32_t b2 = (__float_as_uint(t2) & 0x3FFFFFFFu) | ((uint32_t)(lz & 1) << 31);
	return make_float4(__uint_as_float(b0), __uint_as_float(b1), __uint_as_float(b2), __uint_as_float(index));
}
__device__ inline void fine_decode_at(const float4 &r, int y0, int z0, float t[3], int l[3]) {
	const uint32_t b0 = __float_as_uint(r.x), b1 = __float_as_uint(r.y), b2 = __float_as_uint(r.z);
	t[0] = __uint_as_float(b0 & 0x3FFFFFFFu); t[1] = __uint_as_float(b1 & 0x3FFFFFFFu); t[2] = __uint_as_float(b2 & 0x3FFFFFFFu);
	l[0] = (int)(b0 >> 30) | ((int)(b1 >> 31) << 2);
	l[1] = y0 + ((y0 ^ (int)(b1 >> 30)) & 1);
	l[2] = z0 + ((z0 ^ (int)(b2 >> 31)) & 1);
}
__device__ inline void fine_decode(const float4 &r, int fy, int fz, float t[3], int l[3]) {
	fine_decode_at(r, (8 * fy) / FT, (8 * fz) / FT, t, l);
}

__global__ void __launch_bounds__(FIDX_THREADS)
k_build_fine_index(const int *ptiles, int n_ptiles, const uint32_t *key, const float *t0, const float *t1, const float *t2,
                   const uint32_t *tile_start, const uint32_t *tile_count, uint32_t *fine_start, float4 *spos, uint32_t *key_copy) {
	__shared__ uint32_t cnt[FIDX_CNT / 2];
	__shared__ uint32_t wsum[FIDX_THREADS / 64];
	__shared__ float4 stage[FIDX_STAGE];
	static_assert(FIDX_CNT % (2 * FIDX_THREADS) == 0 && FIDX_STAGE % FIDX_THREADS == 0 && FIDX_STAGE < 65536 && FIDX_CNT <= 4 * FIDX_STAGE,
	              "index kernel sizing");
	constexpr int PER = FIDX_CNT / FIDX_THREADS;
	uint32_t *cnt_big = (uint32_t *)stage;
	auto fine_of = [&](uint32_t i, int l[3], float t[3]) -> int {
		const uint32_t k = key[i];
		l[0] = (int)(k & 7); l[1] = (int)((k >> 3) & 7); l[2] = (int)((k >> 6) & 7);
		t[0] = t0[i]; t[1] = t1[i]; t[2] = t2[i];
		return fine_coord_x(l[0], t[0]) + FTX * (fine_coord(l[1], t[1]) + FT * fine_coord(l[2], t[2]));
	};
	constexpr int RPT = FIDX_STAGE / FIDX_THREADS;
	for (int slot = blockIdx.x; slot < n_ptiles; slot += gridDim.x) {
		const int tile = ptiles[slot];
		const uint32_t b = tile_start[tile], e = b + tile_count[tile];
		const bool staged = e - b <= FIDX_STAGE;
		if (staged) {
#pragma unroll
			for (int k = 0; k < PER / 2; ++k) cnt[threadIdx.x + FIDX_THREADS * k] = 0;
		} else {
#pragma unroll
			for (int k = 0; k < PER; ++k) cnt_big[threadIdx.x + FIDX_THREADS * k] = 0;
		}
		__syncthreads();
		uint32_t rf[RPT];
		float r0[RPT], r1[RPT], r2[RPT];
		if (staged) {
			const uint32_t last = e > b ? e - 1 : 0u;
#pragma unroll
			for (int r = 0; r < RPT; ++r) {
				const uint32_t i = min(b + threadIdx.x + FIDX_THREADS * r, last);
				rf[r] = key[i];
				r0[r] = t0[i]; r1[r] = t1[i]; r2[r] = t2[i];
			}
#pragma unroll
			for (int r = 0; r < RPT; ++r) {
				if (b + threadIdx.x + FIDX_THREADS * r < e) {
					const int l[3] = {(int)(rf[r] & 7), (int)((rf[r] >> 3) & 7), (int)((rf[r] >> 6) & 7)};
					const int f = fine_coord_x(l[0], r0[r]) + FTX * (fine_coord(l[1], r1[r]) + FT * fine_coord(l[2], r2[r]));
					rf[r] = ((uint32_t)f << 9) | (uint32_t)(l[0] | (l[1] << 3) | (l[2] << 6));
					atomicAdd(&cnt[f >> 1], 1u << (16 * (f & 1)));
				} else {
					rf[r] = 0xFFFFFFFFu;
				}
			}
		} else {
			for (uint32_t i = b + threadIdx.x; i < e; i += FIDX_THREADS) {
				int l[3];
				float t[3];
				atomicAdd(&cnt_big[fine_of(i, l, t)], 1u);
			}
		}
		__syncthreads();
		uint32_t c[PER], incl = 0;
#pragma unroll
		for (int k = 0; k < PER; ++k) {
			c[k] = staged ? (cnt[(PER / 2) * threadIdx.x + k / 2] >> (16 * (k & 1))) & 0xFFFFu : cnt_big[PER * threadIdx.x + k];
			incl += c[k];
		}
		const uint32_t sum = incl;
		const int lane = threadIdx.x & 63, wid = threadIdx.x >> 6;
#pragma unroll
		for (int o = 1; o < 64; o <<= 1) {
			uint32_t t = __shfl_up(incl, o, 64);
			if (lane >= o) incl += t;
		}
// ... 5 lines not shown
#pragma unroll
		for (int k = 0; k < PER; ++k) {
			const int f = PER * threadIdx.x + k;
			if (!staged) cnt_big[f] = ex;
			else if (k & 1) cnt[f >> 1] = (ex - c[k - (k & 1)]) | (ex << 16);
			if (!staged && f <= FT3) fine_start[(size_t)tile * FT_STRIDE + f] = b + ex;
			ex += c[k];
		}
		__syncthreads();
		if (staged) {
#pragma unroll
			for (int r = 0; r < RPT; ++r)
				if (rf[r] != 0xFFFFFFFFu) {
					const uint32_t f = rf[r] >> 9;
					const uint32_t at = (atomicAdd(&cnt[f >> 1], 1u << (16 * (f & 1))) >> (16 * (f & 1))) & 0xFFFFu;
					stage[at] = fine_record((int)(rf[r] & 7), (int)((rf[r] >> 3) & 7), (int)((rf[r] >> 6) & 7), r0[r], r1[r], r2[r],
					                        b + threadIdx.x + FIDX_THREADS * r);
				}
			if (key_copy) {
#pragma unroll
				for (int r = 0; r < RPT; ++r)
					if (rf[r] != 0xFFFFFFFFu) key_copy[b + threadIdx.x + FIDX_THREADS * r] = ((uint32_t)tile << 9) | (rf[r] & 511u);
			}
			__syncthreads();
			for (int f = threadIdx.x; f <= FT3; f += FIDX_THREADS)
				fine_start[(size_t)tile * FT_STRIDE + f] = b + (f ? (cnt[(f - 1) >> 1] >> (16 * ((f - 1) & 1))) & 0xFFFFu : 0u);
			for (uint32_t k = threadIdx.x; k < e - b; k += FIDX_THREADS) spos[b + k] = stage[k];
		} else {
			for (uint32_t i = b + threadIdx.x; i < e; i += FIDX_THREADS) {
				int l[3];
				float t[3];
				const uint32_t at = atomicAdd(&cnt_big[fine_of(i, l, t)], 1u);
				spos[b + at] = fine_record(l[0], l[1], l[2], t[0], t[1], t[2], i);
				if (key_copy) key_copy[i] = key[i];
			}
		}
		__syncthreads();
	}
}

__device__ inline int fine_source(const GridDims &g, const uint32_t *tile_count, int tx, int ty, int tz, int gx, int gy, int gz, int &fx,
                                  int &fy, int &fz) {
	const int dx = gx < 0 ? -1 : (gx >= FTX ? 1 : 0), dy = gy < 0 ? -1 : (gy >= FT ? 1 : 0), dz = gz < 0 ? -1 : (gz >= FT ? 1 : 0);
	fx = gx - FTX * dx; fy = gy - FT * dy; fz = gz - FT * dz;
	const int x = tx + dx, y = ty + dy, z = tz + dz;
	if ((unsigned)x >= (unsigned)g.ntx || (unsigned)y >= (unsigned)g.nty || (unsigned)z >= (unsigned)g.ntz) return -1;
	const int tile = x + g.ntx * (y + g.nty * z);
	return tile_count[tile] ? tile : -1;
}

__device__ inline void correct_collide_record(size_t rk, const ParticleSoA &p, uint32_t *out_key, float *out_tx, float *out_ty, float *out_tz,
                                              const GridDims &g, const uint8_t *solid, const uint32_t *tile_count, const uint32_t *fine_start,
                                              const float4 *spos, const MoveParams &mp, const uint32_t *only_flagged, const int *tile_pslot,
                                              int p_off, const uint32_t *key_before) {
	const float4 me = spos[rk];
	const size_t i = __float_as_uint(me.w);
	const uint32_t key_i = key_before ? key_before[i] : p.key[i];
	if (key_i == 0xFFFFFFFFu) return;
	const int tile = (int)(key_i >> 9);
	const int l[3] = {(int)(key_i & 7), (int)((key_i >> 3) & 7), (int)((key_i >> 6) & 7)};
	const float t[3] = {__uint_as_float(__float_as_uint(me.x) & 0x3FFFFFFFu), __uint_as_float(__float_as_uint(me.y) & 0x3FFFFFFFu),
	                    __uint_as_float(__float_as_uint(me.z) & 0x3FFFFFFFu)};
	const int f[3] = {fine_coord_x(l[0], t[0]), fine_coord(l[1], t[1]), fine_coord(l[2], t[2])};
	if (only_flagged) {
		const int work = CORR_PARTS * (tile_pslot[tile] - p_off) + f[2] / FT_PL;
		if (!((only_flagged[1 + (work >> 5)] >> (work & 31)) & 1u)) return;
	}
	int tx, ty, tz;
	tile_coords(g, tile, tx, ty, tz);
	const int nn[3] = {g.nx, g.ny, g.nz};
	const float inv_re2 = (float)mp.inv_re2;
	double spring[3] = {0.0, 0.0, 0.0};
	for (int dz = -1; dz <= 1; ++dz)
		for (int dy = -1; dy <= 1; ++dy)
			for (int dx = -2; dx <= 2; ++dx) {
				int sf[3];
				const int src = fine_source(g, tile_count, tx, ty, tz, f[0] + dx, f[1] + dy, f[2] + dz, sf[0], sf[1], sf[2]);
				if (src < 0) continue;
				const uint32_t *fs = fine_start + (size_t)src * FT_STRIDE + (sf[0] + FTX * (sf[1] + FT * sf[2]));
				const uint32_t kb = fs[0], ke = fs[1];
				int stx, sty, stz;
				tile_coords(g, src, stx, sty, stz);
				for (uint32_t k = kb; k < ke; ++k) {
					const float4 rec = spos[k];
					if (__float_as_uint(rec.w) == (uint32_t)i) continue;
					float nt[3];
					int nl[3];
					fine_decode(rec, sf[1], sf[2], nt, nl);
					const float ddx = ((float)(8 * (tx - stx) + l[0] - nl[0]) + t[0]) - nt[0];
					const float ddy = ((float)(8 * (ty - sty) + l[1] - nl[1]) + t[1]) - nt[1];
					const float ddz = ((float)(8 * (tz - stz) + l[2] - nl[2]) + t[2]) - nt[2];
					const float d2 = ddx * ddx + ddy * ddy + ddz * ddz;
					if (d2 < 1e-12f) {
						const uint32_t j = __float_as_uint(rec.w);
						spring[0] += hash_unit((uint32_t)i, j, 0); spring[1] += hash_unit((uint32_t)i, j, 1);
						spring[2] += hash_unit((uint32_t)i, j, 2);
					} else {
						const float kl = 1.0f - d2 * inv_re2;
						if (kl > 0.0f) {
							const float fr = kl * kl * kl * rsqrtf(d2);
							spring[0] += (double)(fr * ddx); spring[1] += (double)(fr * ddy); spring[2] += (double)(fr * ddz);
						}
					}
				}
			}
	const int c[3] = {8 * tx + l[0], 8 * ty + l[1], 8 * tz + l[2]};
	double from[3], to[3];
#pragma unroll
	for (int d = 0; d < 3; ++d) {
		from[d] = (double)c[d] + (double)t[d];
		double x = from[d] + spring[d] * mp.corr;
		to[d] = x < 0.0 ? 0.0 : ((double)nn[d] < x ? (double)nn[d] : x);
	}
	if (mp.collide) collide(g, solid, from, to, mp.skin);
	int nc[3];
	float ntt[3];
#pragma unroll
	for (int d = 0; d < 3; ++d) split_position(to[d], nn[d], nc[d], ntt[d]);
	out_key[i] = blocked_index(g, nc[0], nc[1], nc[2]);
	out_tx[i] = ntt[0]; out_ty[i] = ntt[1]; out_tz[i] = ntt[2];
}

__global__ void __launch_bounds__(256)
k_correct_collide(size_t n, ParticleSoA p, uint32_t *out_key, float *out_tx, float *out_ty, float *out_tz, GridDims g,
                   const uint8_t *solid, const uint32_t *tile_count, const uint32_t *fine_start, const float4 *spos, MoveParams mp,
                   const uint32_t *only_flagged, const int *tile_pslot, int p_off, const uint32_t *key_before) {
	if (only_flagged && only_flagged[0] == 0) return;
	for (size_t rk = (size_t)blockIdx.x * blockDim.x + threadIdx.x; rk < n; rk += (size_t)gridDim.x * blockDim.x)
		correct_collide_record(rk, p, out_key, out_tx, out_ty, out_tz, g, solid, tile_count, fine_start, spos, mp, only_flagged, tile_pslot,
		                       p_off, key_before);
}

#ifdef CORR_PROFILE
__device__ unsigned long long g_corr_prof[8];
#define CORR_STAMP(k)                                                                   \
	do {                                                                                \
		if (!ONLY && threadIdx.x == 0) {                                                \
			const unsigned long long now_ = wall_clock64();                             \
			atomicAdd(&g_corr_prof[k], now_ - stamp_);                                  \
			stamp_ = now_;                                                              \
		}                                                                               \
	} while (0)
#else
#define CORR_STAMP(k) do { } while (0)
#endif
template <int CAP, bool ONLY>
__global__ void __launch_bounds__(ONLY ? CORR_THREADS_BIG : CORR_THREADS, 4)
k_correct_fine(const int *ptiles, int n_ptiles, uint32_t *out_key, float *out_tx, float *out_ty, float *out_tz, GridDims g,
                const uint8_t *solid, const uint32_t *tile_count, const uint32_t *fine_start, const float4 *spos, MoveParams mp,
                uint32_t *overflow_tiles, const uint8_t *tile_clear, const uint32_t *only) {
	constexpr int T = ONLY ? CORR_THREADS_BIG : CORR_THREADS;
	constexpr int CNT0 = ((FB_N + 1 + 2 * T - 1) / (2 * T)) * (2 * T);
	constexpr int CNT = ONLY && CNT0 < 4096 ? 4096 : CNT0;
	__shared__ float px[CAP], py[CAP], pz[CAP];
	__shared__ uint16_t own[CNT];
	__shared__ uint32_t foff2[(FB_N + 2) / 2];
	const uint16_t *foff = (const uint16_t *)foff2;
	__shared__ __attribute__((aligned(16))) uint32_t rowd[FB_ROWS * 4];
	__shared__ uint32_t rowe[FB_ROWS];
	constexpr int ROW_NOT_OWN = -32768;
	__shared__ uint32_t ownoff[FT * FT_PL + 1];
	__shared__ int srct[27];
	__shared__ uint32_t wsum[T / 64];
	static_assert(CNT > FB_N && CNT % (2 * T) == 0 && FBX % 2 == 0 && CAP < 32768 && CNT < 32768, "own list and cell rounds sizing");
	const int nn[3] = {g.nx, g.ny, g.nz};
	const int lane = threadIdx.x & 63, wid = threadIdx.x >> 6;
	if (ONLY && only[0] == 0) return;
	constexpr int SLICES = ONLY ? CORR_BIG_SLICES : 1;
	for (int item = blockIdx.x; item < SLICES * CORR_PARTS * n_ptiles; item += gridDim.x) {
		int work = item / SLICES;
		const int slice = item % SLICES;
		if (!ONLY && (item / (8 * CORR_PARTS)) * 8 + 8 <= n_ptiles)
			work = CORR_PARTS * ((item / (8 * CORR_PARTS)) * 8 + item % 8) + (item % (8 * CORR_PARTS)) / 8;
		if (ONLY && !((only[1 + (work >> 5)] >> (work & 31)) & 1u)) continue;
		const int tile = ptiles[work / CORR_PARTS], part = work % CORR_PARTS;
		int tx, ty, tz;
		tile_coords(g, tile, tx, ty, tz);
		const int own_lo = part * FT_PL, own_n = (own_lo + FT_PL <= FT ? FT_PL : FT - own_lo);
		const int gz0 = own_lo - 1;
		const int nzb = own_n + 2;
		const int nrows = FB * nzb, nown_rows = FT * (nzb - 2);
// ... 266 lines not shown
			sy += s2y.x + s2y.y;
			sz += s2z.x + s2z.y;
#ifdef CORR_PROFILE
			if (!ONLY && threadIdx.x == 0) atomicAdd(&g_corr_prof[4], wall_clock64() - w0_);
#endif
			float tme[3];
			int lme[3];
			const float4 rec = spos[grec];
			const uint32_t yz = rowe[myrow];
			fine_decode_at(rec, (int)(yz & 7u), (int)((yz >> 3) & 7u), tme, lme);
			const uint32_t jj = __float_as_uint(rec.w);
			const int c[3] = {8 * tx + lme[0], 8 * ty + lme[1], 8 * tz + lme[2]};
			const double spring[3] = {(double)sx, (double)sy, (double)sz};
			double from[3], to[3];
#pragma unroll
			for (int d = 0; d < 3; ++d) {
				from[d] = (double)c[d] + (double)tme[d];
				to[d] = from[d] + spring[d] * mp.corr;
			}
			if (!(lean && fabs(to[0] - from[0]) < 7.0 && fabs(to[1] - from[1]) < 7.0 && fabs(to[2] - from[2]) < 7.0)) {
#pragma unroll
				for (int d = 0; d < 3; ++d) to[d] = to[d] < 0.0 ? 0.0 : ((double)nn[d] < to[d] ? (double)nn[d] : to[d]);
				if (mp.collide) {
					if (!open_water || fabs(to[0] - from[0]) >= 7.0 || fabs(to[1] - from[1]) >= 7.0 || fabs(to[2] - from[2]) >= 7.0)
						collide(g, solid, from, to, mp.skin);
					else
						collide_walls_only(g, to, mp.skin);
				}
			}
			int nc[3];
			float nt[3];
#pragma unroll
			for (int d = 0; d < 3; ++d) split_position(to[d], nn[d], nc[d], nt[d]);
			out_key[jj] = blocked_index(g, nc[0], nc[1], nc[2]);
			out_tx[jj] = nt[0]; out_ty[jj] = nt[1]; out_tz[jj] = nt[2];
		}
#ifdef CORR_PROFILE
		CORR_STAMP(2);
		__syncthreads();
		CORR_STAMP(3);
#endif
	}
}

}
#ifdef CORR_PROFILE
extern "C" int lfa_debug_corr_prof(uint64_t out[8], int reset) {
	unsigned long long h[8] = {0};
	if (hipMemcpyFromSymbol(h, HIP_SYMBOL(g_corr_prof), sizeof h) != hipSuccess) return -1;
	for (int i = 0; i < 8; ++i) out[i] = h[i];
	if (reset) {
		unsigned long long z[8] = {0};
		if (hipMemcpyToSymbol(HIP_SYMBOL(g_corr_prof), z, sizeof z) != hipSuccess) return -1;
	}
	return 0;
}
#endif

static MoveParams move_params(const lfa_sim *s, double dt) {
	MoveParams mp;
	const double h = s->prm.cell_size, re = h / sqrt(2.0);
	mp.dt_over_h = dt / h;
	mp.skin = s->prm.boundary_skin_width / h;
	mp.corr = dt * s->prm.correction_stiffness * re / h;
	mp.inv_re2 = h * h / (re * re);
	mp.collide = 1;
	mp.c_home = s->c_home_valid ? s->c_home : nullptr;
	mp.c_home_stride = s->c_home_cap;
// ... 6 lines not shown
	const size_t i = (size_t)blockIdx.x * blockDim.x + threadIdx.x;
	if (i < n) map[cell[i]] = (uint8_t)src1[i];
}
__global__ void k_source_need(const uint32_t *cell, const uint32_t *lo, const uint32_t *target, size_t n, const uint32_t *cell_count,
                              const uint32_t *tile_flag, uint32_t *need) {
	const size_t i = (size_t)blockIdx.x * blockDim.x + threadIdx.x;
	if (i >= n) return;
	const uint32_t b = cell[i];
	const uint32_t have = lo[i] != 0xFFFFFFFFu ? lo[i] : (tile_flag[b >> 9] ? cell_count[b] : 0u);
	need[i] = target[i] > have ? target[i] - have : 0u;
}
__global__ void k_source_need_scatter(const uint32_t *need, const uint32_t *gidx, size_t n, float *all) {
	const size_t i = (size_t)blockIdx.x * blockDim.x + threadIdx.x;
	if (i < n) all[gidx[i]] = (float)need[i];
}
__global__ void k_source_need_gather(const float *all, size_t n, uint32_t *need) {
	const size_t i = (size_t)blockIdx.x * blockDim.x + threadIdx.x;
	if (i < n) need[i] = (uint32_t)all[i];
}
__device__ inline uint64_t mix64(uint64_t x) {
	x ^= x >> 30; x *= 0xBF58476D1CE4E5B9ull;
	x ^= x >> 27; x *= 0x94D049BB133111EBull;
	x ^= x >> 31;
	return x;
}
__global__ void k_source_seed(const uint32_t *cell, const uint32_t *src_of, const uint32_t *need, const uint32_t *off, size_t n,
                              const float *src_vel, ParticleSoA p, size_t base, uint64_t seed, uint64_t id_base) {
	const size_t i = (size_t)blockIdx.x * blockDim.x + threadIdx.x;
	if (i >= n) return;
	const uint32_t cnt = need[i], b = cell[i];
	const float *vel = src_vel + 3 * src_of[i];
	for (uint32_t j = 0; j < cnt; ++j) {
		const size_t d = base + off[i] + j;
		p.key[d] = b;
#pragma unroll
		for (int a = 0; a < 3; ++a) {
			const uint64_t r = mix64(seed + ((id_base + (uint64_t)(d - base)) * 3ull + (uint64_t)a + 1ull) * 0x9E3779B97F4A7C15ull + ((uint64_t)b << 40));
			float t = (float)(r >> 40) * (1.0f / 16777216.0f);
			p.t[a][d] = t;
			p.v[a][d] = vel[a];
		}
		particle_zero_c_set_id(p, d, (uint32_t)(id_base + (uint64_t)(d - base)));
	}
}
}

extern "C" int lfa_clear_sources(lfa_sim *s) {
	if (!s) return LFA_E_INVALID;
	s->sources.clear();
	s->sources_valid = false;
	return LFA_OK;
}

extern "C" int lfa_add_source(lfa_sim *s, const int32_t *xyz, uint64_t k, const double velocity[3], uint64_t root, int active,
                              int coerce_velocity) {
	if (!s || (!xyz && k) || !velocity) return LFA_E_INVALID;
	if (s->sources.size() >= 254) return lfa_fail(s, LFA_E_UNSUPPORTED, "more than 254 fluid sources");
	if (root > 16) return lfa_fail(s, LFA_E_INVALID, "target_density_cubic_root %llu: more than 4096 particles per cell", (unsigned long long)root);
	for (uint64_t i = 0; i < k; ++i)
		if (!in_grid(s->g, xyz[3 * i], xyz[3 * i + 1], xyz[3 * i + 2]))
			return lfa_fail(s, LFA_E_INVALID, "source cell (%d, %d, %d) outside the grid", xyz[3 * i], xyz[3 * i + 1], xyz[3 * i + 2]);
	lfa_sim::SourceHost h;
	h.xyz.assign(xyz, xyz + 3 * k);
	for (int d = 0; d < 3; ++d) h.vel[d] = velocity[d];
	h.root = root;
	h.active = active != 0;
	h.coerce = coerce_velocity != 0;
	s->sources.push_back(std::move(h));
	s->sources_valid = false;
	return LFA_OK;
}

int lfa_sources_sync(lfa_sim *s) {
	if (s->sources_valid) return LFA_OK;
// ... 330 lines not shown
		const uint8_t *cm = s->any_coerce ? (const uint8_t *)s->coerce_map : (const uint8_t *)nullptr;
		const float *sv = s->any_coerce ? (const float *)s->src_vel : (const float *)nullptr;
		if (with_count && !s->dist) {
			LFA_HIP(s, hipMemsetAsync(s->tile_count, 0, (size_t)(s->g.nt + 1) * 4, s->stream));
			const dim3 grid((unsigned)((n + 256 * AC_CHUNKS - 1) / (256 * AC_CHUNKS)));
			if (s->any_coerce)
				hipLaunchKernelGGL(k_advect_collide_count<true>, grid, dim3(256), 0, s->stream, n, s->pb[s->cur], s->g, s->solid,
				                   mp, cm, sv, (const uint8_t *)s->tile_clear, s->tile_count, s->rank);
			else
				hipLaunchKernelGGL(k_advect_collide_count<false>, grid, dim3(256), 0, s->stream, n, s->pb[s->cur], s->g, s->solid,
				                   mp, cm, sv, (const uint8_t *)s->tile_clear, s->tile_count, s->rank);
			s->counts_fresh = true;
		} else {
			const dim3 grid((unsigned)((n + 255) / 256));
			if (s->any_coerce)
				hipLaunchKernelGGL(k_advect_collide<true>, grid, dim3(256), 0, s->stream, n, s->pb[s->cur], s->g, s->solid, mp,
				                   cm, sv, (const uint8_t *)s->tile_clear);
			else
				hipLaunchKernelGGL(k_advect_collide<false>, grid, dim3(256), 0, s->stream, n, s->pb[s->cur], s->g, s->solid, mp,
				                   cm, sv, (const uint8_t *)s->tile_clear);
		}
		LFA_LAUNCH_CHECK(s);
	}
	if (!split) LFA_TRY(lfa_dist_migrate(s));
	s->unknown_count_valid = false;
	s->move_pending = split;
	return LFA_OK;
}
extern "C" int lfa_advect_collide(lfa_sim *s, double dt) { return advect_collide(s, dt, false); }
extern "C" int lfa_advect(lfa_sim *s, double dt) { return advect_collide(s, dt, false, true); }

namespace {
__global__ void __launch_bounds__(256)
k_collide_only(size_t n, ParticleSoA p, const uint32_t *old_key, const float *ot0, const float *ot1, const float *ot2, GridDims g,
               const uint8_t *solid, double skin) {
	const size_t i = (size_t)blockIdx.x * blockDim.x + threadIdx.x;
	if (i >= n) return;
	const uint32_t key = p.key[i];
	if (key == 0xFFFFFFFFu) return;
	const int nn[3] = {g.nx, g.ny, g.nz};
	int c[3], oc[3];
	cell_of_key(g, key, c);
	double from[3], to[3];
	const float ot[3] = {ot0 ? ot0[i] : p.t[0][i], ot1 ? ot1[i] : p.t[1][i], ot2 ? ot2[i] : p.t[2][i]};
	cell_of_key(g, old_key ? old_key[i] : key, oc);
#pragma unroll
	for (int d = 0; d < 3; ++d) {
		to[d] = (double)c[d] + (double)p.t[d][i];
		from[d] = (double)oc[d] + (double)ot[d];
	}
	collide(g, solid, from, to, skin);
	int nc[3];
	float nt[3];
#pragma unroll
	for (int d = 0; d < 3; ++d) split_position(to[d], nn[d], nc[d], nt[d]);
	p.key[i] = blocked_index(g, nc[0], nc[1], nc[2]);
#pragma unroll
	for (int d = 0; d < 3; ++d) p.t[d][i] = nt[d];
}
}

static int save_old_positions(lfa_sim *s, size_t n) {
	if (!n) return LFA_OK;
	ParticleSoA &cur = s->pb[s->cur], &oth = s->pb[s->cur ^ 1];
	LFA_HIP(s, hipMemcpyAsync(oth.key, cur.key, n * 4, hipMemcpyDeviceToDevice, s->stream));
	for (int d = 0; d < 3; ++d) LFA_HIP(s, hipMemcpyAsync(oth.t[d], cur.t[d], n * 4, hipMemcpyDeviceToDevice, s->stream));
	return LFA_OK;
}

extern "C" int lfa_collide(lfa_sim *s) {
	if (!s) return LFA_E_INVALID;
	LFA_HIP(s, hipSetDevice(s->device));
	LFA_TRY(lfa_corr_commit(s));
	const size_t n = s->binned ? s->np_live : s->np;
	const bool pending = s->move_pending;
	s->move_pending = false;
	if (!n) return lfa_dist_migrate(s);
	LFA_TRY(refresh_tile_clear(s));
	ParticleSoA &cur = s->pb[s->cur], &oth = s->pb[s->cur ^ 1];
	hipLaunchKernelGGL(k_collide_only, dim3((unsigned)((n + 255) / 256)), dim3(256), 0, s->stream, n, cur,
	                   pending ? (const uint32_t *)oth.key : (const uint32_t *)nullptr, pending ? (const float *)oth.t[0] : (const float *)nullptr,
	                   pending ? (const float *)oth.t[1] : (const float *)nullptr, pending ? (const float *)oth.t[2] : (const float *)nullptr, s->g,
	                   (const uint8_t *)s->solid, move_params(s, 0.0).skin);
	LFA_LAUNCH_CHECK(s);
	s->unknown_count_valid = false;
	return lfa_dist_migrate(s);
}

static float4 *correction_scratch(lfa_sim *s) {
	ParticleSoA &cur = s->pb[s->cur], &oth = s->pb[s->cur ^ 1];
	return (float4 *)(!s->vc_pending ? oth.v[0] : (s->vc_with_c ? cur.v[0] : oth.c[0]));
}

static int correct_build_index(lfa_sim *s, bool exchange = true) {
	const size_t n = s->np_live;
	if (!n && !s->dist) return LFA_OK;
	if (!s->fine_start) {
		const size_t bytes = (size_t)s->g.nt * FT_STRIDE * 4;
		hipError_t e = hipMalloc(&s->fine_start, bytes);
		if (e != hipSuccess) return lfa_fail(s, LFA_E_OOM, "hipMalloc of the fine-cell index (%zu bytes) failed", bytes);
	}
	if (s->dist && exchange) LFA_TRY(lfa_dist_exchange_ghost_particles(s));
	LFA_TRY(refresh_tile_clear(s));
	const int n_index = s->dist ? s->n_ptiles_all : s->n_ptiles;
	const int grid = n_index < 16384 ? (n_index > 0 ? n_index : 1) : 16384;
	ParticleSoA &cur = s->pb[s->cur];
	if (n) LFA_TRY(lfa_ev_record(s, LFA_EV_CORR_BEGIN));
	hipLaunchKernelGGL(k_build_fine_index, dim3(grid), dim3(FIDX_THREADS), 0, s->stream, s->dist ? s->ptiles_all : s->ptiles, n_index, cur.key,
	                   cur.t[0], cur.t[1], cur.t[2], s->tile_start, s->tile_count, s->fine_start, correction_scratch(s), s->pb[s->cur ^ 1].key);
	LFA_LAUNCH_CHECK(s);
	return LFA_OK;
}

static int correct_apply(lfa_sim *s, double dt, bool migrate = true, bool with_collide = true) {
	const size_t n = s->np_live;
	MoveParams mpc = move_params(s, dt);
	mpc.collide = with_collide ? 1 : 0;
	ParticleSoA &cur = s->pb[s->cur], &oth = s->pb[s->cur ^ 1];
	float4 *spos = correction_scratch(s);
	if (n) {
		const size_t ovf_words = ((size_t)CORR_PARTS * s->n_ptiles + 31) / 32 + 2;
		const size_t ovf_stride = ((size_t)CORR_PARTS * s->g.nt + 31) / 32 + 2;
		if (!s->corr_ovf) {
			hipError_t e = hipMalloc(&s->corr_ovf, 2 * ovf_stride * 4);
			if (e != hipSuccess) return lfa_fail(s, LFA_E_OOM, "hipMalloc of the correction's overflow bitmaps failed");
		}
		uint32_t *ovf = s->corr_ovf, *ovf2 = s->corr_ovf + ovf_stride;
		s->corr_parts_tiles = s->n_ptiles;
		LFA_HIP(s, hipMemsetAsync(ovf, 0, ovf_words * 4, s->stream));
		LFA_HIP(s, hipMemsetAsync(ovf2, 0, ovf_words * 4, s->stream));
		{
			const int work = CORR_PARTS * s->n_ptiles, g2 = work < 65536 ? (work > 0 ? work : 1) : 65536;
			LFA_TRY(lfa_ev_record(s, LFA_EV_CORR_INDEXED));
			hipLaunchKernelGGL((k_correct_fine<FINE_CAP, false>), dim3(g2), dim3(CORR_THREADS), 0, s->stream, s->ptiles, s->n_ptiles, cur.key,
			                   cur.t[0], cur.t[1], cur.t[2], s->g, s->solid, s->tile_count, s->fine_start, (const float4 *)spos, mpc, ovf,
			                   (const uint8_t *)s->tile_clear, (const uint32_t *)nullptr);
			LFA_LAUNCH_CHECK(s);
			LFA_TRY(lfa_ev_record(s, LFA_EV_CORR_TILED));
			hipLaunchKernelGGL((k_correct_fine<FINE_CAP_BIG, true>), dim3(std::min(CORR_BIG_SLICES * g2, 2048)), dim3(CORR_THREADS_BIG), 0, s->stream, s->ptiles,
			                   s->n_ptiles, cur.key, cur.t[0], cur.t[1], cur.t[2], s->g, s->solid, s->tile_count, s->fine_start,
			                   (const float4 *)spos, mpc, ovf2, (const uint8_t *)s->tile_clear, (const uint32_t *)ovf);
			LFA_LAUNCH_CHECK(s);
		}
		const uint32_t *fallback = ovf2;
		hipLaunchKernelGGL(k_correct_collide, dim3((unsigned)std::min<size_t>((n + 255) / 256, 16384)), dim3(256), 0, s->stream, n, cur, cur.key, cur.t[0],
		                   cur.t[1], cur.t[2], s->g, s->solid, s->tile_count, s->fine_start, (const float4 *)spos, mpc,
		                   fallback, (const int *)s->tile_pslot, s->p_off, (const uint32_t *)oth.key);
		LFA_LAUNCH_CHECK(s);
	}
	if (migrate) LFA_TRY(lfa_dist_migrate(s));
	s->unknown_count_valid = false;
	return LFA_OK;
}

extern "C" int lfa_correct_collide(lfa_sim *s, double dt) {
	if (!s) return LFA_E_INVALID;
	if (!s->binned) return lfa_fail(s, LFA_E_INVALID, "lfa_correct_collide: call lfa_hash_particles first");
	LFA_HIP(s, hipSetDevice(s->device));
	LFA_TRY(lfa_corr_commit(s));
	if (!s->np_live && !s->dist) return LFA_OK;
	LFA_TRY(correct_build_index(s));
	return correct_apply(s, dt);
}

extern "C" int lfa_correct(lfa_sim *s, double dt) {
	if (!s) return LFA_E_INVALID;
	if (!s->binned) return lfa_fail(s, LFA_E_INVALID, "lfa_correct: call lfa_hash_particles first");
	LFA_HIP(s, hipSetDevice(s->device));
	LFA_TRY(lfa_corr_commit(s));
	s->move_pending = false;
	if (!s->np_live && !s->dist) return LFA_OK;
	LFA_TRY(correct_build_index(s));
	ParticleSoA &cur = s->pb[s->cur], &oth = s->pb[s->cur ^ 1];
	for (int d = 0; d < 3 && s->np_live; ++d) LFA_HIP(s, hipMemcpyAsync(oth.t[d], cur.t[d], s->np_live * 4, hipMemcpyDeviceToDevice, s->stream));
	LFA_TRY(correct_apply(s, dt, false, false));
	s->move_pending = true;
	return LFA_OK;
}

int lfa_corr_join(lfa_sim *s) {
	if (!s->corr_in_flight) return LFA_OK;
	s->corr_in_flight = false;
	LFA_HIP(s, hipStreamWaitEvent(s->stream, s->ev_cjoin, 0));
	return LFA_OK;
}

static int correct_begin(lfa_sim *s, double dt, bool slab_exchanged) {
	if (!s) return LFA_E_INVALID;
	if (!s->binned) return lfa_fail(s, LFA_E_INVALID, "lfa_correct_collide_begin: call lfa_hash_particles first");
	if (s->dist && !slab_exchanged)
		return lfa_fail(s, LFA_E_UNSUPPORTED, "lfa_correct_collide_begin: slab decompositions exchange particles inside the correction (use lfa_correct_collide or lfa_time_step)");
	LFA_HIP(s, hipSetDevice(s->device));
	LFA_TRY(lfa_corr_commit(s));
	s->corr_begun = false;
	if (!s->np_live && !s->dist) return LFA_OK;
	LFA_HIP(s, hipEventRecord(s->ev_cfork, s->stream));
	LFA_HIP(s, hipStreamWaitEvent(s->stream3, s->ev_cfork, 0));
	hipStream_t main_stream = s->stream;
	s->stream = s->stream3;
	int rc = correct_build_index(s, false);
	if (rc == LFA_OK) rc = correct_apply(s, dt, false);
	s->stream = main_stream;
	const hipError_t e1 = s->timing ? hipEventRecord(s->ev[LFA_EV_STEP_CORRECT], s->stream3) : hipSuccess;
	const hipError_t e2 = hipEventRecord(s->ev_cjoin, s->stream3);
	s->corr_in_flight = true;
	s->corr_begun = true;
	s->corr_undo_valid = rc == LFA_OK && !s->dist;
	if (rc < 0) return rc;
	LFA_HIP(s, e1);
	LFA_HIP(s, e2);
	return LFA_OK;
}
extern "C" int lfa_correct_collide_begin(lfa_sim *s, double dt) { return correct_begin(s, dt, false); }

extern "C" int lfa_correct_collide_end(lfa_sim *s) {
	if (!s) return LFA_E_INVALID;
	LFA_HIP(s, hipSetDevice(s->device));
	return lfa_corr_join(s);
}

namespace {
__global__ void __launch_bounds__(256)
k_correct_undo(size_t n, const float4 *spos, const uint32_t *old_key, uint32_t *key, float *t0, float *t1, float *t2) {
	const size_t k = (size_t)blockIdx.x * blockDim.x + threadIdx.x;
	if (k >= n) return;
	const float4 rec = spos[k];
	const uint32_t i = __float_as_uint(rec.w);
	t0[i] = __uint_as_float(__float_as_uint(rec.x) & 0x3FFFFFFFu);
	t1[i] = __uint_as_float(__float_as_uint(rec.y) & 0x3FFFFFFFu);
	t2[i] = __uint_as_float(__float_as_uint(rec.z) & 0x3FFFFFFFu);
	key[k] = old_key[k];
}
}

extern "C" int lfa_correct_collide_undo(lfa_sim *s) {
	if (!s) return LFA_E_INVALID;
	if (!s->corr_begun) return LFA_OK;
	if (!s->corr_undo_valid)
		return lfa_fail(s, LFA_E_INVALID, "lfa_correct_collide_undo: positions, binning or solid cells have changed since lfa_correct_collide_begin");
	LFA_HIP(s, hipSetDevice(s->device));
	LFA_TRY(lfa_corr_commit(s));
	s->corr_begun = false;
	const size_t n = s->np_live;
	if (!n) return LFA_OK;
	ParticleSoA &cur = s->pb[s->cur], &oth = s->pb[s->cur ^ 1];
	hipLaunchKernelGGL(k_correct_undo, dim3((unsigned)((n + 255) / 256)), dim3(256), 0, s->stream, n, (const float4 *)correction_scratch(s),
	                   (const uint32_t *)oth.key, cur.key, cur.t[0], cur.t[1], cur.t[2]);
	LFA_LAUNCH_CHECK(s);
	return LFA_OK;
}

int lfa_g2p_stale(lfa_sim *s);
extern "C" int lfa_time_step(lfa_sim *s, double dt, double *residual, uint64_t *iterations) {
	if (!s) return LFA_E_INVALID;
	if (s->src_rng_on && s->dist && !(s->src_rng_flags & LFA_SEED_COLLECTIVE))
		return lfa_fail(s, LFA_E_UNSUPPORTED, "lfa_time_step: fluid sources that draw from the pcg32 (lfa_set_source_rng) on a slab decomposition");
	LFA_HIP(s, hipSetDevice(s->device));
	LFA_TRY(lfa_corr_commit(s));
	LFA_TRY(lfa_ev_record(s, LFA_EV_STEP_START));
	LFA_TRY(advect_collide(s, dt, true));
	LFA_TRY(lfa_ev_record(s, LFA_EV_STEP_ADVECT));
	{
		const bool counted = s->counts_fresh;
		s->counts_fresh = false;
		LFA_TRY(lfa_hash_particles_impl(s, counted));
	}
	if (!s->sources.empty()) LFA_TRY(lfa_update_sources(s, nullptr));
	LFA_TRY(lfa_ev_record(s, LFA_EV_STEP_BIN));
	const bool overlap = s->overlap_correction && (s->dist || s->np_live);
	LFA_TRY(lfa_p2g_run(s, true, dt));
	LFA_TRY(lfa_ev_record(s, LFA_EV_STEP_P2G));
	if (overlap) {
		if (s->dist) LFA_TRY(lfa_dist_exchange_ghost_particles(s));
		LFA_TRY(correct_begin(s, dt, true));
	}
	double res = 0.0;
	uint64_t it = 0;
	int rc = LFA_OK;
	auto grid_stages = [&]() -> int {
		rc = lfa_pcg_solve(s, dt, &res, &it);
// ... 98 lines not shown
```

libfluid_amd/csrc/seed.hip:

```cpp
#include "common.h"

#include <cmath>

#define PCG_MULT 6364136223846793005ull
#define PCG_INC 1442695040888963407ull

struct SeedJump {
	uint64_t mult[64], plus[64];
};
static constexpr SeedJump make_seed_jump() {
	SeedJump t{};
	uint64_t m = PCG_MULT, p = PCG_INC;
	for (int j = 0; j < 64; ++j) {
		t.mult[j] = m;
		t.plus[j] = p;
		p = (m + 1ull) * p;
		m = m * m;
	}
	return t;
}
static constexpr SeedJump h_jump = make_seed_jump();
__constant__ SeedJump c_jump = make_seed_jump();

static uint64_t pcg_advance(uint64_t state, uint64_t k) {
// ... 13 lines not shown
	double ret = sum / 18446744073709551616.0;
	if (ret >= 1.0) ret = 0x1.fffffffffffffp-1;
	return ret * (sub - 0.0) + 0.0;
}

__device__ inline uint64_t pcg_jump(uint64_t state, uint64_t draws, int nbits) {
	for (int j = 0; j < nbits; ++j)
		if ((draws >> j) & 1ull) state = state * c_jump.mult[j] + c_jump.plus[j];
	return state;
}
__device__ inline void seed_draw3(uint64_t &state, double width, int ltr, double (&u)[3]) {
	if (ltr) {
		u[0] = seed_uniform(state, width); u[1] = seed_uniform(state, width); u[2] = seed_uniform(state, width);
	} else {
		u[2] = seed_uniform(state, width); u[1] = seed_uniform(state, width); u[0] = seed_uniform(state, width);
	}
}
__device__ inline double seed_draw_z(uint64_t &state, double width, int ltr) {
	if (ltr) state = state * c_jump.mult[2] + c_jump.plus[2];
	const double z = seed_uniform(state, width);
	if (!ltr) state = state * c_jump.mult[2] + c_jump.plus[2];
	return z;
}
__device__ inline bool seed_owned(double z, const IngestParams &ip, int nz, int slab_lo, int slab_hi, int &cz, float &tz) {
	cell_and_fraction(z, ip.off[2], ip.h, nz, cz, tz);
	return (cz >> 3) >= slab_lo && (cz >> 3) < slab_hi;
}
__device__ inline void born_particle(const ParticleSoA &p, size_t d, const GridDims &g, const IngestParams &ip, const double (&x)[3], int cz,
                                     float tz, float v0, float v1, float v2, uint32_t id, double *pos_out) {
	int cx, cy;
	float tx, ty;
	cell_and_fraction(x[0], ip.off[0], ip.h, g.nx, cx, tx);
	cell_and_fraction(x[1], ip.off[1], ip.h, g.ny, cy, ty);
	p.key[d] = blocked_index(g, cx, cy, cz);
	p.t[0][d] = tx; p.t[1][d] = ty; p.t[2][d] = tz;
	p.v[0][d] = v0; p.v[1][d] = v1; p.v[2][d] = v2;
	particle_zero_c_set_id(p, d, id);
	if (pos_out) {
		pos_out[0] = x[0]; pos_out[1] = x[1]; pos_out[2] = x[2];
	}
}

struct SeedShape {
	IngestParams ip;
	double sub;
	double lo[3], hi[3];
	double r2;
	uint64_t n_cand, state;
	uint32_t s[3], ex, ey;
	uint32_t density, d3;
	int nbits;
	int sphere, ltr;
	int nz, slab_lo, slab_hi;
};

__device__ inline bool seed_candidate(const SeedShape &q, uint64_t i, double (&pos)[3]) {
	const uint32_t cell = (uint32_t)(i / q.d3), sub = (uint32_t)(i - (uint64_t)cell * q.d3);
	const uint32_t xy = q.ex * q.ey, cz = cell / xy, rem = cell - cz * xy, cy = rem / q.ex, cx = rem - cy * q.ex;
	const uint32_t dd = q.density * q.density, sx = sub / dd, srem = sub - sx * dd, sy = srem / q.density, sz = srem - sy * q.density;
	uint64_t st = pcg_jump(q.state, 6ull * i, q.nbits);
	double u[3];
	seed_draw3(st, q.sub, q.ltr, u);
	pos[0] = ((q.ip.off[0] + (double)(q.s[0] + cx) * q.ip.h) + (double)sx * q.sub) + u[0];
	pos[1] = ((q.ip.off[1] + (double)(q.s[1] + cy) * q.ip.h) + (double)sy * q.sub) + u[1];
	pos[2] = ((q.ip.off[2] + (double)(q.s[2] + cz) * q.ip.h) + (double)sz * q.sub) + u[2];
	if (q.sphere) {
		const double dx = pos[0] - q.lo[0], dy = pos[1] - q.lo[1], dz = pos[2] - q.lo[2];
		double r = dx * dx;
// ... 300 lines not shown
```

Before: 5.468 billion.

## Pack particle key and cell fractions into one 16-byte AoS position record

```diff
diff --git a/libfluid_amd/csrc/common.h b/libfluid_amd/csrc/common.h
--- a/libfluid_amd/csrc/common.h
+++ b/libfluid_amd/csrc/common.h
@@ -34,9 +34,14 @@
 #define AB_UNKNOWN 0x40
 #define AB_FLUID 0x80
 
+struct alignas(16) PosRec {
+	uint32_t key;
+	float t[3];
+};
+static_assert(sizeof(PosRec) == 16, "a position record is one 16-byte access");
+
 struct ParticleSoA {
-	uint32_t *key = nullptr;
-	float *t[3] = {nullptr, nullptr, nullptr};
+	PosRec *pos = nullptr;
 	float *v[3] = {nullptr, nullptr, nullptr};
 	float *c[9] = {nullptr};
 	uint32_t *id = nullptr;
@@ -87,6 +92,7 @@
 	ParticleSoA pb[2];
 	int cur = 0;
 	uint32_t *rank = nullptr;
+	uint32_t *bkey = nullptr;
 	bool binned = false;
 
 	struct lfa_dist *dist = nullptr;
@@ -364,6 +370,17 @@
 	for (int k = 0; k < 3; ++k) x[k] = ip.off[k] + ((double)c[k] + (double)t[k]) * ip.h;
 }
 
+__device__ inline PosRec pos_load(const PosRec *pos, size_t i) {
+	const uint4 q = *(const uint4 *)(pos + i);
+	PosRec r;
+	r.key = q.x;
+	r.t[0] = __uint_as_float(q.y); r.t[1] = __uint_as_float(q.z); r.t[2] = __uint_as_float(q.w);
+	return r;
+}
+__device__ inline void pos_store(PosRec *pos, size_t i, uint32_t key, float t0, float t1, float t2) {
+	*(uint4 *)(pos + i) = make_uint4(key, __float_as_uint(t0), __float_as_uint(t1), __float_as_uint(t2));
+}
+
 __device__ inline void particle_zero_c_set_id(const ParticleSoA &p, size_t d, uint32_t id) {
 #pragma unroll
 	for (int k = 0; k < 9; ++k) p.c[k][d] = 0.0f;
diff --git a/libfluid_amd/csrc/core.hip b/libfluid_amd/csrc/core.hip
--- a/libfluid_amd/csrc/core.hip
+++ b/libfluid_amd/csrc/core.hip
@@ -344,7 +344,7 @@
 	lfa_pool_nosync_begin();
 	free_soa(s->pb[0]);
 	free_soa(s->pb[1]);
-	void *ptrs[] = {s->c_home, s->fine_start, s->corr_ovf, s->tile_clear, s->tile_epoch, s->tile_closed, s->src_cell, s->src_lo, s->src_target, s->src_of, s->src_need, s->src_vel, s->src_slab.words, s->coerce_map, s->grid_flag, s->rank, s->vc_src, s->tile_count, s->tile_start, s->tile_flag, s->tile_scan, s->ptiles_all, s->dtiles, s->halo_tiles, s->dist_red,
+	void *ptrs[] = {s->c_home, s->fine_start, s->corr_ovf, s->tile_clear, s->tile_epoch, s->tile_closed, s->src_cell, s->src_lo, s->src_target, s->src_of, s->src_need, s->src_vel, s->src_slab.words, s->coerce_map, s->grid_flag, s->rank, s->vc_src, s->bkey, s->tile_count, s->tile_start, s->tile_flag, s->tile_scan, s->ptiles_all, s->dtiles, s->halo_tiles, s->dist_red,
 	                s->xbuf[0], s->xbuf[1], s->xbuf[2], s->xbuf[3],
 	                s->tile_pslot, s->scan_tmp, s->u, s->v, s->w, s->uo, s->vo, s->wo, s->ctype, s->solid,
 	                s->cell_count, s->stage, s->acc, s->abits, s->vp, s->vr, s->vz, s->vs, s->vpre, s->vq, s->vs2, s->c_as, s->nbr_table,
@@ -443,8 +443,7 @@
 	hipError_t e = hipMalloc(&p.base, cap * 17 * 4);
 	if (e != hipSuccess) return lfa_fail(s, LFA_E_OOM, "hipMalloc of particle SoA (%zu particles) failed", cap);
 	float *f = (float *)p.base;
-	p.key = (uint32_t *)f;
-	for (int k = 0; k < 3; ++k) p.t[k] = f + cap * (1 + k);
+	p.pos = (PosRec *)f;
 	for (int k = 0; k < 3; ++k) p.v[k] = f + cap * (4 + k);
 	for (int k = 0; k < 9; ++k) p.c[k] = f + cap * (7 + k);
 	p.id = (uint32_t *)(f + cap * 16);
@@ -456,26 +455,30 @@
 	LFA_HIP(s, hipStreamSynchronize(s->stream));
 	const size_t cap = (n + 1023) & ~(size_t)1023;
 	ParticleSoA nb[2];
-	uint32_t *rank = nullptr, *vc_src = nullptr;
+	uint32_t *rank = nullptr, *vc_src = nullptr, *bkey = nullptr;
 	int rc = alloc_soa(s, nb[0], cap);
 	if (rc == LFA_OK) rc = alloc_soa(s, nb[1], cap);
 	if (rc == LFA_OK && hipMalloc(&rank, cap * 4) != hipSuccess) rc = lfa_fail(s, LFA_E_OOM, "hipMalloc of the rank array failed");
 	if (rc == LFA_OK && hipMalloc(&vc_src, cap * 4) != hipSuccess) rc = lfa_fail(s, LFA_E_OOM, "hipMalloc of the source-index array failed");
+	if (rc == LFA_OK && hipMalloc(&bkey, cap * 4) != hipSuccess) rc = lfa_fail(s, LFA_E_OOM, "hipMalloc of the binned-key array failed");
 	if (rc != LFA_OK) {
 		free_soa(nb[0]);
 		free_soa(nb[1]);
 		if (rank) (void)hipFree(rank);
 		if (vc_src) (void)hipFree(vc_src);
+		if (bkey) (void)hipFree(bkey);
 		return rc;
 	}
 	free_soa(s->pb[0]);
 	free_soa(s->pb[1]);
 	if (s->rank) (void)hipFree(s->rank);
 	if (s->vc_src) (void)hipFree(s->vc_src);
+	if (s->bkey) (void)hipFree(s->bkey);
 	s->pb[0] = nb[0];
 	s->pb[1] = nb[1];
 	s->rank = rank;
 	s->vc_src = vc_src;
+	s->bkey = bkey;
 	s->vc_pending = false;
 	s->pcap = cap;
 	return LFA_OK;
@@ -499,12 +502,11 @@
 	ParticleSoA &dst = s->pb[s->cur];
 	const uint32_t *src_arrays[17];
 	uint32_t *dst_arrays[17];
-	src_arrays[0] = keep.key; dst_arrays[0] = dst.key;
-	for (int k = 0; k < 3; ++k) { src_arrays[1 + k] = (uint32_t *)keep.t[k]; dst_arrays[1 + k] = (uint32_t *)dst.t[k]; }
+	if (n_keep) LFA_HIP(s, hipMemcpyAsync(dst.pos, keep.pos, n_keep * sizeof(PosRec), hipMemcpyDeviceToDevice, s->stream));
 	for (int k = 0; k < 3; ++k) { src_arrays[4 + k] = (uint32_t *)keep.v[k]; dst_arrays[4 + k] = (uint32_t *)dst.v[k]; }
 	for (int k = 0; k < 9; ++k) { src_arrays[7 + k] = (uint32_t *)keep.c[k]; dst_arrays[7 + k] = (uint32_t *)dst.c[k]; }
 	src_arrays[16] = keep.id; dst_arrays[16] = dst.id;
-	for (int a = 0; a < 17; ++a)
+	for (int a = 4; a < 17; ++a)
 		if (n_keep) LFA_HIP(s, hipMemcpyAsync(dst_arrays[a], src_arrays[a], n_keep * 4, hipMemcpyDeviceToDevice, s->stream));
 	LFA_HIP(s, hipStreamSynchronize(s->stream));
 	free_soa(keep);
@@ -520,12 +522,9 @@
 	cell_and_fraction(q[0], ip.off[0], ip.h, g.nx, c[0], t[0]);
 	cell_and_fraction(q[1], ip.off[1], ip.h, g.ny, c[1], t[1]);
 	cell_and_fraction(q[2], ip.off[2], ip.h, g.nz, c[2], t[2]);
-	p.key[i] = ((c[2] >> 3) >= slab_lo && (c[2] >> 3) < slab_hi) ? blocked_index(g, c[0], c[1], c[2]) : 0xFFFFFFFFu;
-#pragma unroll
-	for (int k = 0; k < 3; ++k) {
-		p.t[k][i] = t[k];
-		p.v[k][i] = (float)q[3 + k];
-	}
+	pos_store(p.pos, i, ((c[2] >> 3) >= slab_lo && (c[2] >> 3) < slab_hi) ? blocked_index(g, c[0], c[1], c[2]) : 0xFFFFFFFFu, t[0], t[1], t[2]);
+#pragma unroll
+	for (int k = 0; k < 3; ++k) p.v[k][i] = (float)q[3 + k];
 #pragma unroll
 	for (int k = 0; k < 9; ++k) p.c[k][i] = (float)q[6 + k];
 	p.id[i] = (uint32_t)i;
@@ -560,32 +559,34 @@
 	return LFA_OK;
 }
 
-__global__ void k_valid_flags(const uint32_t *key, size_t n, uint32_t *valid) {
+__global__ void k_valid_flags(const PosRec *pos, size_t n, uint32_t *valid) {
 	size_t i = (size_t)blockIdx.x * blockDim.x + threadIdx.x;
-	if (i < n) valid[i] = key[i] != 0xFFFFFFFFu ? 1u : 0u;
-}
-__global__ void k_export_ids(const uint32_t *key, const uint32_t *id, const uint32_t *slot, size_t n, uint32_t *out) {
+	if (i < n) valid[i] = pos[i].key != 0xFFFFFFFFu ? 1u : 0u;
+}
+__global__ void k_export_ids(const PosRec *pos, const uint32_t *id, const uint32_t *slot, size_t n, uint32_t *out) {
 	size_t i = (size_t)blockIdx.x * blockDim.x + threadIdx.x;
-	if (i < n && key[i] != 0xFFFFFFFFu) out[slot ? slot[i] : i] = id[i];
+	if (i < n && pos[i].key != 0xFFFFFFFFu) out[slot ? slot[i] : i] = id[i];
 }
 
 __global__ void k_export(double *aos, size_t n, ParticleSoA p, GridDims g, IngestParams ip, int flags, int by_slot, const uint32_t *slot,
                          ParticleSoA old, int have_old, const float *c_home, size_t c_home_stride) {
 	size_t i = (size_t)blockIdx.x * blockDim.x + threadIdx.x;
 	if (i >= n) return;
-	uint32_t b = p.key[i];
+	const PosRec me = pos_load(p.pos, i);
+	const uint32_t b = me.key;
 	if (slot && b == 0xFFFFFFFFu) return;
 	double *q = aos + (by_slot ? (slot ? (size_t)slot[i] : i) : (size_t)p.id[i]) * 19;
 	if (flags & LFA_DL_POSITIONS) {
 		double x[3];
-		particle_world_position(g, ip, b, p.t[0][i], p.t[1][i], p.t[2][i], x);
+		particle_world_position(g, ip, b, me.t[0], me.t[1], me.t[2], x);
 #pragma unroll
 		for (int k = 0; k < 3; ++k) {
 			q[k] = x[k];
 			q[15 + k] = x[k];
 		}
 		if (have_old) {
-			particle_world_position(g, ip, old.key[i], old.t[0][i], old.t[1][i], old.t[2][i], x);
+			const PosRec was = pos_load(old.pos, i);
+			particle_world_position(g, ip, was.key, was.t[0], was.t[1], was.t[2], x);
 #pragma unroll
 			for (int k = 0; k < 3; ++k) q[15 + k] = x[k];
 		}
@@ -600,7 +601,7 @@
 int lfa_slab_download_slots(lfa_sim *s, const uint32_t **slot) {
 	*slot = nullptr;
 	if (!s->dist || !s->holes || !s->np_live) return LFA_OK;
-	hipLaunchKernelGGL(k_valid_flags, dim3((unsigned)((s->np_live + 255) / 256)), dim3(256), 0, s->stream, (const uint32_t *)s->pb[s->cur].key,
+	hipLaunchKernelGGL(k_valid_flags, dim3((unsigned)((s->np_live + 255) / 256)), dim3(256), 0, s->stream, (const PosRec *)s->pb[s->cur].pos,
 	                   s->np_live, s->rank);
 	LFA_LAUNCH_CHECK(s);
 	uint32_t *tot = (uint32_t *)(s->pcg_state + LFA_DW_SCAN_TOTAL);
@@ -615,22 +616,21 @@
 
 __global__ void __launch_bounds__(256) k_close_holes(size_t n, ParticleSoA src, ParticleSoA dst, const uint32_t *slot, size_t n_dst) {
 	const size_t i = (size_t)blockIdx.x * 256 + threadIdx.x;
-	if (i >= n || src.key[i] == 0xFFFFFFFFu) return;
+	if (i >= n) return;
+	const PosRec me = pos_load(src.pos, i);
+	if (me.key == 0xFFFFFFFFu) return;
 	const size_t d = slot[i];
 	if (d >= n_dst) return;
-	dst.key[d] = src.key[i];
-#pragma unroll
-	for (int k = 0; k < 3; ++k) {
-		dst.t[k][d] = src.t[k][i];
-		dst.v[k][d] = src.v[k][i];
-	}
+	pos_store(dst.pos, d, me.key, me.t[0], me.t[1], me.t[2]);
+#pragma unroll
+	for (int k = 0; k < 3; ++k) dst.v[k][d] = src.v[k][i];
 #pragma unroll
 	for (int k = 0; k < 9; ++k) dst.c[k][d] = src.c[k][i];
 	dst.id[d] = src.id[i];
 }
 
 int lfa_particles_close_holes(lfa_sim *s, size_t n_rec) {
-	hipLaunchKernelGGL(k_valid_flags, dim3((unsigned)((n_rec + 255) >> 8)), dim3(256), 0, s->stream, (const uint32_t *)s->pb[s->cur].key,
+	hipLaunchKernelGGL(k_valid_flags, dim3((unsigned)((n_rec + 255) >> 8)), dim3(256), 0, s->stream, (const PosRec *)s->pb[s->cur].pos,
 	                   n_rec, s->rank);
 	LFA_LAUNCH_CHECK(s);
 	size_t n_dst = 0;
@@ -687,7 +687,7 @@
 	LFA_TRY(lfa_slab_download_slots(s, &slot));
 	if (slot) {
 		LFA_TRY(lfa_ensure_io(s, n * 4));
-		hipLaunchKernelGGL(k_export_ids, dim3((unsigned)((s->np_live + 255) / 256)), dim3(256), 0, s->stream, (const uint32_t *)s->pb[s->cur].key,
+		hipLaunchKernelGGL(k_export_ids, dim3((unsigned)((s->np_live + 255) / 256)), dim3(256), 0, s->stream, (const PosRec *)s->pb[s->cur].pos,
 		                   (const uint32_t *)s->pb[s->cur].id, slot, s->np_live, (uint32_t *)s->io_buf);
 		LFA_LAUNCH_CHECK(s);
 		LFA_HIP(s, hipMemcpyAsync(ids, s->io_buf, n * 4, hipMemcpyDeviceToHost, s->stream));
@@ -725,12 +725,9 @@
 		double pos = ip.off[a] + ((double)cell[a] + ((double)sb[a] + uu) * 0.5) * ip.h;
 		cell_and_fraction(pos, ip.off[a], ip.h, nn[a], c[a], t[a]);
 	}
-	p.key[j] = blocked_index(g, c[0], c[1], c[2]);
-#pragma unroll
-	for (int k = 0; k < 3; ++k) {
-		p.t[k][j] = t[k];
-		p.v[k][j] = 0.0f;
-	}
+	pos_store(p.pos, j, blocked_index(g, c[0], c[1], c[2]), t[0], t[1], t[2]);
+#pragma unroll
+	for (int k = 0; k < 3; ++k) p.v[k][j] = 0.0f;
 	particle_zero_c_set_id(p, j, (uint32_t)(global_ids ? i : j));
 }
 
@@ -881,7 +878,7 @@
 	return LFA_OK;
 }
 
-__global__ void __launch_bounds__(256) k_tile_count(const uint32_t *key, size_t n, uint32_t *tile_count, uint32_t *rank) {
+__global__ void __launch_bounds__(256) k_tile_count(const PosRec *pos, size_t n, uint32_t *tile_count, uint32_t *rank) {
 	const int lane = threadIdx.x & 63;
 	const size_t wave = ((size_t)blockIdx.x * blockDim.x + threadIdx.x) >> 6;
 	const size_t i0 = wave * (64 * TC_CHUNKS) + lane;
@@ -889,7 +886,7 @@
 #pragma unroll
 	for (int c = 0; c < TC_CHUNKS; ++c) {
 		const size_t i = i0 + 64 * c;
-		const uint32_t k = i < n ? key[i] : 0xFFFFFFFFu;
+		const uint32_t k = i < n ? pos[i].key : 0xFFFFFFFFu;
 		tile[c] = k != 0xFFFFFFFFu ? k >> 9 : 0xFFFFFFFFu;
 	}
 	lfa_wave_tile_ranks(tile, tile_count, my_rank);
@@ -925,32 +922,32 @@
 }
 
 __global__ void k_tile_scatter(size_t n, ParticleSoA src, ParticleSoA dst, const uint32_t *rank,
-                               const uint32_t *tile_start, const uint32_t *tile_count, int shuffle, uint32_t *from) {
+                               const uint32_t *tile_start, const uint32_t *tile_count, int shuffle, uint32_t *from, uint32_t *bkey) {
 	size_t i = (size_t)blockIdx.x * blockDim.x + threadIdx.x;
 	if (i >= n) return;
-	uint32_t key = src.key[i], tile = key >> 9, r = rank[i];
+	const PosRec me = pos_load(src.pos, i);
+	uint32_t key = me.key, tile = key >> 9, r = rank[i];
 	if (key == 0xFFFFFFFFu) return;
 	if (shuffle) {
 		uint32_t cnt = tile_count[tile];
 		if (cnt % 1000003u != 0) r = (uint32_t)(((uint64_t)r * 1000003ull) % cnt);
 	}
 	size_t d = (size_t)tile_start[tile] + r;
-	dst.key[d] = key;
-#pragma unroll
-	for (int k = 0; k < 3; ++k) dst.t[k][d] = src.t[k][i];
+	pos_store(dst.pos, d, key, me.t[0], me.t[1], me.t[2]);
+	bkey[d] = key;
 	dst.id[d] = src.id[i];
 	from[d] = (uint32_t)i;
 }
 __global__ void k_c_to_home(size_t n, ParticleSoA p, float *home, size_t stride) {
 	size_t i = (size_t)blockIdx.x * blockDim.x + threadIdx.x;
-	if (i >= n || p.key[i] == 0xFFFFFFFFu) return;
+	if (i >= n || p.pos[i].key == 0xFFFFFFFFu) return;
 	const size_t j = p.id[i];
 #pragma unroll
 	for (int k = 0; k < 9; ++k) home[k * stride + j] = p.c[k][i];
 }
 __global__ void k_c_from_home(size_t n, ParticleSoA p, const float *home, size_t stride) {
 	size_t i = (size_t)blockIdx.x * blockDim.x + threadIdx.x;
-	if (i >= n || p.key[i] == 0xFFFFFFFFu) return;
+	if (i >= n || p.pos[i].key == 0xFFFFFFFFu) return;
 	const size_t j = p.id[i];
 #pragma unroll
 	for (int k = 0; k < 9; ++k) p.c[k][i] = home[k * stride + j];
@@ -1099,7 +1096,7 @@
 	if (!counts_done) {
 		LFA_HIP(s, hipMemsetAsync(s->tile_count, 0, (size_t)(nt + 1) * 4, s->stream));
 		if (n) {
-			hipLaunchKernelGGL(k_tile_count, dim3((unsigned)((n + 256 * TC_CHUNKS - 1) / (256 * TC_CHUNKS))), dim3(256), 0, s->stream, src.key, n,
+			hipLaunchKernelGGL(k_tile_count, dim3((unsigned)((n + 256 * TC_CHUNKS - 1) / (256 * TC_CHUNKS))), dim3(256), 0, s->stream, (const PosRec *)src.pos, n,
 			                   s->tile_count, s->rank);
 			LFA_LAUNCH_CHECK(s);
 		}
@@ -1183,7 +1180,7 @@
 			LFA_TRY(lfa_c_home_restore(s));
 		}
 		hipLaunchKernelGGL(k_tile_scatter, sgrid, dim3(256), 0, s->stream, n, src, dst, s->rank, s->tile_start, s->tile_count,
-		                   s->binned ? 0 : 1, s->vc_src);
+		                   s->binned ? 0 : 1, s->vc_src, s->bkey);
 		LFA_LAUNCH_CHECK(s);
 		s->cur ^= 1;
 		s->vc_pending = true;
@@ -1193,7 +1190,7 @@
 	if (s->n_dtiles) {
 		int grid = s->n_dtiles < 8192 ? s->n_dtiles : 8192;
 		hipLaunchKernelGGL(k_cell_count, dim3(grid), dim3(256), 0, s->stream, s->dtiles, s->n_dtiles,
-		                   s->pb[s->cur].key, s->tile_start, s->cell_count);
+		                   (const uint32_t *)s->bkey, s->tile_start, s->cell_count);
 		LFA_LAUNCH_CHECK(s);
 	}
 	s->binned = true;
diff --git a/libfluid_amd/csrc/dist.hip b/libfluid_amd/csrc/dist.hip
--- a/libfluid_amd/csrc/dist.hip
+++ b/libfluid_amd/csrc/dist.hip
@@ -310,7 +310,7 @@
 	int dest = -1;
 	uint32_t key = 0xFFFFFFFFu;
 	if (i < n) {
-		key = p.key[i];
+		key = p.pos[i].key;
 		if (key != 0xFFFFFFFFu) {
 			const int tz = (int)(key >> 9) / tiles_per_layer;
 			dest = tz < slab_lo ? 0 : (tz >= slab_hi ? 1 : -1);
@@ -331,7 +331,7 @@
 			const size_t j = from ? (size_t)from[i] : i;
 #pragma unroll
 			for (int k = 0; k < 3; ++k) {
-				rec[1 + k] = __float_as_uint(p.t[k][i]);
+				rec[1 + k] = __float_as_uint(p.pos[i].t[k]);
 				rec[4 + k] = __float_as_uint(from ? pvc.v[k][j] : p.v[k][i]);
 			}
 #pragma unroll
@@ -339,7 +339,7 @@
 				rec[7 + k] = __float_as_uint(c_home ? c_home[k * c_home_stride + p.id[i]]
 				                                    : (from && c_deferred ? pvc.c[k][j] : p.c[k][i]));
 			rec[16] = p.id[i];
-			p.key[i] = 0xFFFFFFFFu;
+			p.pos[i].key = 0xFFFFFFFFu;
 		}
 	}
 }
@@ -354,12 +354,9 @@
 	const uint32_t *rec = buf + i * 17;
 	const size_t d = at + i, e = from ? ext + i : d;
 	const ParticleSoA &q = from ? pvc : p;
-	p.key[d] = rec[0];
+	pos_store(p.pos, d, rec[0], __uint_as_float(rec[1]), __uint_as_float(rec[2]), __uint_as_float(rec[3]));
 #pragma unroll
-	for (int k = 0; k < 3; ++k) {
-		p.t[k][d] = __uint_as_float(rec[1 + k]);
-		q.v[k][e] = __uint_as_float(rec[4 + k]);
-	}
+	for (int k = 0; k < 3; ++k) q.v[k][e] = __uint_as_float(rec[4 + k]);
 #pragma unroll
 	for (int k = 0; k < 9; ++k) {
 		if (c_home) c_home[k * c_home_stride + rec[16]] = __uint_as_float(rec[7 + k]);
@@ -460,10 +457,10 @@
 	}
 	const size_t send_lo_at = hs[0], send_lo_n = lfa_has_lo(s) ? hs[1] - hs[0] : 0;
 	const size_t send_hi_at = hs[2], send_hi_n = lfa_has_hi(s) ? hs[3] - hs[2] : 0;
-	uint32_t *arr[5] = {p.key, (uint32_t *)p.t[0], (uint32_t *)p.t[1], (uint32_t *)p.t[2], p.id};
-	for (int a = 0; a < 5; ++a)
-		LFA_TRY(s->dist->exchange(s, arr[a] + send_lo_at, send_lo_n * 4, arr[a] + at_lo, n_g[0] * 4, arr[a] + send_hi_at,
-		                          send_hi_n * 4, arr[a] + at_hi, n_g[1] * 4));
+	LFA_TRY(s->dist->exchange(s, p.pos + send_lo_at, send_lo_n * sizeof(PosRec), p.pos + at_lo, n_g[0] * sizeof(PosRec), p.pos + send_hi_at,
+	                          send_hi_n * sizeof(PosRec), p.pos + at_hi, n_g[1] * sizeof(PosRec)));
+	LFA_TRY(s->dist->exchange(s, p.id + send_lo_at, send_lo_n * 4, p.id + at_lo, n_g[0] * 4, p.id + send_hi_at, send_hi_n * 4, p.id + at_hi,
+	                          n_g[1] * 4));
 	s->ghost_at[0] = at_lo;
 	s->ghost_at[1] = at_hi;
 	s->n_ghost_particles = n_g[0] + n_g[1];
diff --git a/libfluid_amd/csrc/frame.hip b/libfluid_amd/csrc/frame.hip
--- a/libfluid_amd/csrc/frame.hip
+++ b/libfluid_amd/csrc/frame.hip
@@ -98,15 +98,15 @@
 };
 
 template <bool OCC>
-__global__ void __launch_bounds__(256) k_frame_stats(size_t n, const uint32_t *key, const float *t0, const float *t1, const float *t2,
-                                                     const float *v0, const float *v1, const float *v2, GridDims g, FrameParams q,
+__global__ void __launch_bounds__(256) k_frame_stats(size_t n, const PosRec *pos, const float *v0, const float *v1, const float *v2, GridDims g, FrameParams q,
                                                      uint32_t *occupation, double *part) {
 	FrameAcc a = frame_neutral();
 	for (size_t i = (size_t)blockIdx.x * 256 + threadIdx.x; i < n; i += (size_t)gridDim.x * 256) {
-		const uint32_t b = key[i];
+		const PosRec me = pos_load(pos, i);
+		const uint32_t b = me.key;
 		if (b == 0xFFFFFFFFu) continue;
 		double x[3];
-		particle_world_position(g, q.ip, b, t0[i], t1[i], t2[i], x);
+		particle_world_position(g, q.ip, b, me.t[0], me.t[1], me.t[2], x);
 		const double vx = (double)v0[i], vy = (double)v1[i], vz = (double)v2[i];
 		double sq = vx * vx;
 		sq += vy * vy;
@@ -144,17 +144,17 @@
 	if (threadIdx.x == 0) frame_store(a, part + (size_t)FRAME_GRID_CAP * FRAME_FIELDS, 1);
 }
 
-__global__ void __launch_bounds__(256) k_export_positions(double *xyz, size_t n, size_t n_out, const uint32_t *key, const float *t0,
-                                                          const float *t1, const float *t2, const uint32_t *id, GridDims g, IngestParams ip,
+__global__ void __launch_bounds__(256) k_export_positions(double *xyz, size_t n, size_t n_out, const PosRec *pos, const uint32_t *id, GridDims g, IngestParams ip,
                                                           int by_slot, const uint32_t *slot) {
 	const size_t i = (size_t)blockIdx.x * 256 + threadIdx.x;
 	if (i >= n) return;
-	const uint32_t b = key[i];
+	const PosRec me = pos_load(pos, i);
+	const uint32_t b = me.key;
 	if (b == 0xFFFFFFFFu) return;
 	const size_t d = by_slot ? (slot ? (size_t)slot[i] : i) : (size_t)id[i];
 	if (d >= n_out) return;
 	double x[3];
-	particle_world_position(g, ip, b, t0[i], t1[i], t2[i], x);
+	particle_world_position(g, ip, b, me.t[0], me.t[1], me.t[2], x);
 #pragma unroll
 	for (int k = 0; k < 3; ++k) xyz[3 * d + k] = x[k];
 }
@@ -200,12 +200,12 @@
 	LFA_HIP(s, hipEventRecord(s->frame_ev[0], s->stream));
 	if (occupation) {
 		LFA_HIP(s, hipMemsetAsync(s->io_buf, 0, s->nc * 4, s->stream));
-		hipLaunchKernelGGL(k_frame_stats<true>, dim3((unsigned)blocks), dim3(256), 0, s->stream, n_rec, (const uint32_t *)p.key,
-		                   (const float *)p.t[0], (const float *)p.t[1], (const float *)p.t[2], (const float *)p.v[0], (const float *)p.v[1],
+		hipLaunchKernelGGL(k_frame_stats<true>, dim3((unsigned)blocks), dim3(256), 0, s->stream, n_rec, (const PosRec *)p.pos,
+		                   (const float *)p.v[0], (const float *)p.v[1],
 		                   (const float *)p.v[2], s->g, q, (uint32_t *)s->io_buf, s->frame_part);
 	} else {
-		hipLaunchKernelGGL(k_frame_stats<false>, dim3((unsigned)blocks), dim3(256), 0, s->stream, n_rec, (const uint32_t *)p.key,
-		                   (const float *)p.t[0], (const float *)p.t[1], (const float *)p.t[2], (const float *)p.v[0], (const float *)p.v[1],
+		hipLaunchKernelGGL(k_frame_stats<false>, dim3((unsigned)blocks), dim3(256), 0, s->stream, n_rec, (const PosRec *)p.pos,
+		                   (const float *)p.v[0], (const float *)p.v[1],
 		                   (const float *)p.v[2], s->g, q, (uint32_t *)nullptr, s->frame_part);
 	}
 	LFA_LAUNCH_CHECK(s);
@@ -257,7 +257,7 @@
 	const size_t n_rec = s->binned ? s->np_live : s->np;
 	const ParticleSoA &p = s->pb[s->cur];
 	hipLaunchKernelGGL(k_export_positions, dim3((unsigned)((n_rec + 255) / 256)), dim3(256), 0, s->stream, (double *)s->io_buf, n_rec,
-	                   (size_t)n, (const uint32_t *)p.key, (const float *)p.t[0], (const float *)p.t[1], (const float *)p.t[2],
+	                   (size_t)n, (const PosRec *)p.pos,
 	                   (const uint32_t *)p.id, s->g, ip, s->dist ? 1 : 0, slot);
 	LFA_LAUNCH_CHECK(s);
 	LFA_HIP(s, hipMemcpyAsync(xyz, s->io_buf, n * 24, hipMemcpyDeviceToHost, s->stream));
diff --git a/libfluid_amd/csrc/grid_ops.hip b/libfluid_amd/csrc/grid_ops.hip
--- a/libfluid_amd/csrc/grid_ops.hip
+++ b/libfluid_amd/csrc/grid_ops.hip
@@ -318,7 +318,8 @@
 template <int METHOD, typename Corner, typename Fetch>
 __device__ inline float g2p_particle(const ParticleSoA &p, uint32_t i, const ParticleSoA &pold, uint32_t j, const G2PParams &gp,
                                     Corner &&corner, Fetch &&fetch) {
-	const float t[3] = {p.t[0][i], p.t[1][i], p.t[2][i]};
+	const PosRec me = pos_load(p.pos, i);
+	const float t[3] = {me.t[0], me.t[1], me.t[2]};
 	float vp[3] = {0.0f, 0.0f, 0.0f}, vout[3], cvec[9];
 	if (METHOD == LFA_FLIP_BLEND) {
 #pragma unroll
@@ -389,10 +390,11 @@
 			float t[3], vp[3];
 		} cur, nxt;
 		auto load = [&](uint32_t i, uint32_t j, Regs &r) {
-			r.key = p.key[i];
+			const PosRec me = pos_load(p.pos, i);
+			r.key = me.key;
 #pragma unroll
 			for (int k = 0; k < 3; ++k) {
-				r.t[k] = p.t[k][i];
+				r.t[k] = me.t[k];
 				r.vp[k] = FLIP ? pold.v[k][j] : 0.0f;
 			}
 		};
@@ -461,7 +463,7 @@
 	const uint32_t n = *n_leavers;
 	float vmax2 = 0.0f;
 	for (uint32_t k = blockIdx.x * 256 + threadIdx.x; k < n; k += gridDim.x * 256) {
-		const uint32_t i = leavers[k], key = p.key[i];
+		const uint32_t i = leavers[k], key = p.pos[i].key;
 		if (key == 0xFFFFFFFFu) continue;
 		const int tile = (int)(key >> 9), l = (int)(key & 511);
 		int tx, ty, tz;
diff --git a/libfluid_amd/csrc/mesher.hip b/libfluid_amd/csrc/mesher.hip
--- a/libfluid_amd/csrc/mesher.hip
+++ b/libfluid_amd/csrc/mesher.hip
@@ -668,7 +668,8 @@
 	const size_t k = (size_t)blockIdx.x * blockDim.x + threadIdx.x;
 	if (k >= n) return;
 	const size_t i = first + k;
-	const uint32_t b = p.key[i];
+	const PosRec me = pos_load(p.pos, i);
+	const uint32_t b = me.key;
 	const int tile = (int)(b >> 9), l = (int)(b & 511);
 	int tx, ty, tz;
 	tile_coords(g, tile, tx, ty, tz);
@@ -677,7 +678,7 @@
 	const size_t at = by_slot ? out_at + k : (size_t)p.id[i];
 	double *q = pos + 3 * at;
 #pragma unroll
-	for (int d = 0; d < 3; ++d) q[d] = off[d] + ((double)c[d] + (double)p.t[d][i]) * h;
+	for (int d = 0; d < 3; ++d) q[d] = off[d] + ((double)c[d] + (double)me.t[d]) * h;
 	if (by_slot) ids[at] = p.id[i];
 }
 
diff --git a/libfluid_amd/csrc/p2g.hip b/libfluid_amd/csrc/p2g.hip
--- a/libfluid_amd/csrc/p2g.hip
+++ b/libfluid_amd/csrc/p2g.hip
@@ -128,10 +128,11 @@
 };
 template <bool APIC>
 __device__ inline void load_particle(const ParticleSoA &p, const ParticleSoA &pvc, uint32_t i, uint32_t j, ParticleRegs &r) {
-	r.key = p.key[i];
+	const PosRec me = pos_load(p.pos, i);
+	r.key = me.key;
 #pragma unroll
 	for (int k = 0; k < 3; ++k) {
-		r.t[k] = p.t[k][i];
+		r.t[k] = me.t[k];
 		r.v[k] = pvc.v[k][j];
 	}
 	if (APIC) {
@@ -200,12 +201,13 @@
 k_p2g_atomic(size_t n, ParticleSoA p, float *acc, size_t ncp, GridDims g, float hworld) {
 	size_t i = (size_t)blockIdx.x * blockDim.x + threadIdx.x;
 	if (i >= n) return;
-	const uint32_t key = p.key[i];
+	const PosRec me = pos_load(p.pos, i);
+	const uint32_t key = me.key;
 	const int tile = (int)(key >> 9), l = (int)(key & 511);
 	int tx, ty, tz;
 	tile_coords(g, tile, tx, ty, tz);
 	const int cx = tx * 8 + (l & 7), cy = ty * 8 + ((l >> 3) & 7), cz = tz * 8 + (l >> 6);
-	float t[3] = {p.t[0][i], p.t[1][i], p.t[2][i]};
+	float t[3] = {me.t[0], me.t[1], me.t[2]};
 	float v[3] = {p.v[0][i], p.v[1][i], p.v[2][i]};
 	float c[9];
 	if (APIC) {
diff --git a/libfluid_amd/csrc/particles.hip b/libfluid_amd/csrc/particles.hip
--- a/libfluid_amd/csrc/particles.hip
+++ b/libfluid_amd/csrc/particles.hip
@@ -157,10 +157,11 @@
 	uint32_t src;
 };
 __device__ inline void advect_load(size_t i, const ParticleSoA &p, AdvectSlot &a) {
-	a.key = p.key[i];
+	const PosRec me = pos_load(p.pos, i);
+	a.key = me.key;
 #pragma unroll
 	for (int d = 0; d < 3; ++d) {
-		a.t[d] = p.t[d][i];
+		a.t[d] = me.t[d];
 		a.v[d] = p.v[d][i];
 	}
 }
@@ -201,9 +202,7 @@
 template <bool COERCE>
 __device__ inline void advect_store(size_t i, const ParticleSoA &p, const MoveParams &mp, const AdvectSlot &a) {
 	if (a.key == 0xFFFFFFFFu) return;
-	p.key[i] = a.key;
-#pragma unroll
-	for (int d = 0; d < 3; ++d) p.t[d][i] = a.t[d];
+	pos_store(p.pos, i, a.key, a.t[0], a.t[1], a.t[2]);
 	if (COERCE && a.src) {
 #pragma unroll
 		for (int d = 0; d < 3; ++d) p.v[d][i] = a.v[d];
@@ -314,9 +313,8 @@
 	fine_decode_at(r, (8 * fy) / FT, (8 * fz) / FT, t, l);
 }
 
-__global__ void __launch_bounds__(FIDX_THREADS)
-k_build_fine_index(const int *ptiles, int n_ptiles, const uint32_t *key, const float *t0, const float *t1, const float *t2,
-                   const uint32_t *tile_start, const uint32_t *tile_count, uint32_t *fine_start, float4 *spos, uint32_t *key_copy) {
+__global__ void __launch_bounds__(FIDX_THREADS, 4)
+k_build_fine_index(const int *ptiles, int n_ptiles, const PosRec *pos, const uint32_t *tile_start, const uint32_t *tile_count, uint32_t *fine_start, float4 *spos, uint32_t *key_copy) {
 	__shared__ uint32_t cnt[FIDX_CNT / 2];
 	__shared__ uint32_t wsum[FIDX_THREADS / 64];
 	__shared__ float4 stage[FIDX_STAGE];
@@ -325,9 +323,10 @@
 	constexpr int PER = FIDX_CNT / FIDX_THREADS;
 	uint32_t *cnt_big = (uint32_t *)stage;
 	auto fine_of = [&](uint32_t i, int l[3], float t[3]) -> int {
-		const uint32_t k = key[i];
+		const PosRec me = pos_load(pos, i);
+		const uint32_t k = me.key;
 		l[0] = (int)(k & 7); l[1] = (int)((k >> 3) & 7); l[2] = (int)((k >> 6) & 7);
-		t[0] = t0[i]; t[1] = t1[i]; t[2] = t2[i];
+		t[0] = me.t[0]; t[1] = me.t[1]; t[2] = me.t[2];
 		return fine_coord_x(l[0], t[0]) + FTX * (fine_coord(l[1], t[1]) + FT * fine_coord(l[2], t[2]));
 	};
 	constexpr int RPT = FIDX_STAGE / FIDX_THREADS;
@@ -350,8 +349,9 @@
 #pragma unroll
 			for (int r = 0; r < RPT; ++r) {
 				const uint32_t i = min(b + threadIdx.x + FIDX_THREADS * r, last);
-				rf[r] = key[i];
-				r0[r] = t0[i]; r1[r] = t1[i]; r2[r] = t2[i];
+				const PosRec me = pos_load(pos, i);
+				rf[r] = me.key;
+				r0[r] = me.t[0]; r1[r] = me.t[1]; r2[r] = me.t[2];
 			}
 #pragma unroll
 			for (int r = 0; r < RPT; ++r) {
@@ -423,7 +423,7 @@
 				float t[3];
 				const uint32_t at = atomicAdd(&cnt_big[fine_of(i, l, t)], 1u);
 				spos[b + at] = fine_record(l[0], l[1], l[2], t[0], t[1], t[2], i);
-				if (key_copy) key_copy[i] = key[i];
+				if (key_copy) key_copy[i] = pos[i].key;
 			}
 		}
 		__syncthreads();
@@ -440,13 +440,12 @@
 	return tile_count[tile] ? tile : -1;
 }
 
-__device__ inline void correct_collide_record(size_t rk, const ParticleSoA &p, uint32_t *out_key, float *out_tx, float *out_ty, float *out_tz,
-                                              const GridDims &g, const uint8_t *solid, const uint32_t *tile_count, const uint32_t *fine_start,
+__device__ inline void correct_collide_record(size_t rk, const ParticleSoA &p, PosRec *out, const GridDims &g, const uint8_t *solid, const uint32_t *tile_count, const uint32_t *fine_start,
                                               const float4 *spos, const MoveParams &mp, const uint32_t *only_flagged, const int *tile_pslot,
                                               int p_off, const uint32_t *key_before) {
 	const float4 me = spos[rk];
 	const size_t i = __float_as_uint(me.w);
-	const uint32_t key_i = key_before ? key_before[i] : p.key[i];
+	const uint32_t key_i = key_before ? key_before[i] : p.pos[i].key;
 	if (key_i == 0xFFFFFFFFu) return;
 	const int tile = (int)(key_i >> 9);
 	const int l[3] = {(int)(key_i & 7), (int)((key_i >> 3) & 7), (int)((key_i >> 6) & 7)};
@@ -508,17 +507,16 @@
 	float ntt[3];
 #pragma unroll
 	for (int d = 0; d < 3; ++d) split_position(to[d], nn[d], nc[d], ntt[d]);
-	out_key[i] = blocked_index(g, nc[0], nc[1], nc[2]);
-	out_tx[i] = ntt[0]; out_ty[i] = ntt[1]; out_tz[i] = ntt[2];
+	pos_store(out, i, blocked_index(g, nc[0], nc[1], nc[2]), ntt[0], ntt[1], ntt[2]);
 }
 
 __global__ void __launch_bounds__(256)
-k_correct_collide(size_t n, ParticleSoA p, uint32_t *out_key, float *out_tx, float *out_ty, float *out_tz, GridDims g,
+k_correct_collide(size_t n, ParticleSoA p, PosRec *out, GridDims g,
                    const uint8_t *solid, const uint32_t *tile_count, const uint32_t *fine_start, const float4 *spos, MoveParams mp,
                    const uint32_t *only_flagged, const int *tile_pslot, int p_off, const uint32_t *key_before) {
 	if (only_flagged && only_flagged[0] == 0) return;
 	for (size_t rk = (size_t)blockIdx.x * blockDim.x + threadIdx.x; rk < n; rk += (size_t)gridDim.x * blockDim.x)
-		correct_collide_record(rk, p, out_key, out_tx, out_ty, out_tz, g, solid, tile_count, fine_start, spos, mp, only_flagged, tile_pslot,
+		correct_collide_record(rk, p, out, g, solid, tile_count, fine_start, spos, mp, only_flagged, tile_pslot,
 		                       p_off, key_before);
 }
 
@@ -537,7 +535,7 @@
 #endif
 template <int CAP, bool ONLY>
 __global__ void __launch_bounds__(ONLY ? CORR_THREADS_BIG : CORR_THREADS, 4)
-k_correct_fine(const int *ptiles, int n_ptiles, uint32_t *out_key, float *out_tx, float *out_ty, float *out_tz, GridDims g,
+k_correct_fine(const int *ptiles, int n_ptiles, PosRec *out, GridDims g,
                 const uint8_t *solid, const uint32_t *tile_count, const uint32_t *fine_start, const float4 *spos, MoveParams mp,
                 uint32_t *overflow_tiles, const uint8_t *tile_clear, const uint32_t *only) {
 	constexpr int T = ONLY ? CORR_THREADS_BIG : CORR_THREADS;
@@ -870,8 +868,7 @@
 			float nt[3];
 #pragma unroll
 			for (int d = 0; d < 3; ++d) split_position(to[d], nn[d], nc[d], nt[d]);
-			out_key[jj] = blocked_index(g, nc[0], nc[1], nc[2]);
-			out_tx[jj] = nt[0]; out_ty[jj] = nt[1]; out_tz[jj] = nt[2];
+			pos_store(out, jj, blocked_index(g, nc[0], nc[1], nc[2]), nt[0], nt[1], nt[2]);
 		}
 #ifdef CORR_PROFILE
 		CORR_STAMP(2);
@@ -944,14 +941,15 @@
 	const float *vel = src_vel + 3 * src_of[i];
 	for (uint32_t j = 0; j < cnt; ++j) {
 		const size_t d = base + off[i] + j;
-		p.key[d] = b;
+		float tt[3];
 #pragma unroll
 		for (int a = 0; a < 3; ++a) {
 			const uint64_t r = mix64(seed + ((id_base + (uint64_t)(d - base)) * 3ull + (uint64_t)a + 1ull) * 0x9E3779B97F4A7C15ull + ((uint64_t)b << 40));
 			float t = (float)(r >> 40) * (1.0f / 16777216.0f);
-			p.t[a][d] = t;
+			tt[a] = t;
 			p.v[a][d] = vel[a];
 		}
+		pos_store(p.pos, d, b, tt[0], tt[1], tt[2]);
 		particle_zero_c_set_id(p, d, (uint32_t)(id_base + (uint64_t)(d - base)));
 	}
 }
@@ -1348,39 +1346,37 @@
 
 namespace {
 __global__ void __launch_bounds__(256)
-k_collide_only(size_t n, ParticleSoA p, const uint32_t *old_key, const float *ot0, const float *ot1, const float *ot2, GridDims g,
+k_collide_only(size_t n, ParticleSoA p, const PosRec *old, GridDims g,
                const uint8_t *solid, double skin) {
 	const size_t i = (size_t)blockIdx.x * blockDim.x + threadIdx.x;
 	if (i >= n) return;
-	const uint32_t key = p.key[i];
+	const PosRec me = pos_load(p.pos, i);
+	const uint32_t key = me.key;
 	if (key == 0xFFFFFFFFu) return;
+	const PosRec was = old ? pos_load(old, i) : me;
 	const int nn[3] = {g.nx, g.ny, g.nz};
 	int c[3], oc[3];
 	cell_of_key(g, key, c);
 	double from[3], to[3];
-	const float ot[3] = {ot0 ? ot0[i] : p.t[0][i], ot1 ? ot1[i] : p.t[1][i], ot2 ? ot2[i] : p.t[2][i]};
-	cell_of_key(g, old_key ? old_key[i] : key, oc);
+	cell_of_key(g, was.key, oc);
 #pragma unroll
 	for (int d = 0; d < 3; ++d) {
-		to[d] = (double)c[d] + (double)p.t[d][i];
-		from[d] = (double)oc[d] + (double)ot[d];
+		to[d] = (double)c[d] + (double)me.t[d];
+		from[d] = (double)oc[d] + (double)was.t[d];
 	}
 	collide(g, solid, from, to, skin);
 	int nc[3];
 	float nt[3];
 #pragma unroll
 	for (int d = 0; d < 3; ++d) split_position(to[d], nn[d], nc[d], nt[d]);
-	p.key[i] = blocked_index(g, nc[0], nc[1], nc[2]);
-#pragma unroll
-	for (int d = 0; d < 3; ++d) p.t[d][i] = nt[d];
+	pos_store(p.pos, i, blocked_index(g, nc[0], nc[1], nc[2]), nt[0], nt[1], nt[2]);
 }
 }
 
 static int save_old_positions(lfa_sim *s, size_t n) {
 	if (!n) return LFA_OK;
 	ParticleSoA &cur = s->pb[s->cur], &oth = s->pb[s->cur ^ 1];
-	LFA_HIP(s, hipMemcpyAsync(oth.key, cur.key, n * 4, hipMemcpyDeviceToDevice, s->stream));
-	for (int d = 0; d < 3; ++d) LFA_HIP(s, hipMemcpyAsync(oth.t[d], cur.t[d], n * 4, hipMemcpyDeviceToDevice, s->stream));
+	LFA_HIP(s, hipMemcpyAsync(oth.pos, cur.pos, n * sizeof(PosRec), hipMemcpyDeviceToDevice, s->stream));
 	return LFA_OK;
 }
 
@@ -1395,8 +1391,7 @@
 	LFA_TRY(refresh_tile_clear(s));
 	ParticleSoA &cur = s->pb[s->cur], &oth = s->pb[s->cur ^ 1];
 	hipLaunchKernelGGL(k_collide_only, dim3((unsigned)((n + 255) / 256)), dim3(256), 0, s->stream, n, cur,
-	                   pending ? (const uint32_t *)oth.key : (const uint32_t *)nullptr, pending ? (const float *)oth.t[0] : (const float *)nullptr,
-	                   pending ? (const float *)oth.t[1] : (const float *)nullptr, pending ? (const float *)oth.t[2] : (const float *)nullptr, s->g,
+	                   pending ? (const PosRec *)oth.pos : (const PosRec *)nullptr, s->g,
 	                   (const uint8_t *)s->solid, move_params(s, 0.0).skin);
 	LFA_LAUNCH_CHECK(s);
 	s->unknown_count_valid = false;
@@ -1422,8 +1417,8 @@
 	const int grid = n_index < 16384 ? (n_index > 0 ? n_index : 1) : 16384;
 	ParticleSoA &cur = s->pb[s->cur];
 	if (n) LFA_TRY(lfa_ev_record(s, LFA_EV_CORR_BEGIN));
-	hipLaunchKernelGGL(k_build_fine_index, dim3(grid), dim3(FIDX_THREADS), 0, s->stream, s->dist ? s->ptiles_all : s->ptiles, n_index, cur.key,
-	                   cur.t[0], cur.t[1], cur.t[2], s->tile_start, s->tile_count, s->fine_start, correction_scratch(s), s->pb[s->cur ^ 1].key);
+	hipLaunchKernelGGL(k_build_fine_index, dim3(grid), dim3(FIDX_THREADS), 0, s->stream, s->dist ? s->ptiles_all : s->ptiles, n_index,
+	                   (const PosRec *)cur.pos, s->tile_start, s->tile_count, s->fine_start, correction_scratch(s), s->bkey);
 	LFA_LAUNCH_CHECK(s);
 	return LFA_OK;
 }
@@ -1432,7 +1427,7 @@
 	const size_t n = s->np_live;
 	MoveParams mpc = move_params(s, dt);
 	mpc.collide = with_collide ? 1 : 0;
-	ParticleSoA &cur = s->pb[s->cur], &oth = s->pb[s->cur ^ 1];
+	ParticleSoA &cur = s->pb[s->cur];
 	float4 *spos = correction_scratch(s);
 	if (n) {
 		const size_t ovf_words = ((size_t)CORR_PARTS * s->n_ptiles + 31) / 32 + 2;
@@ -1448,20 +1443,20 @@
 		{
 			const int work = CORR_PARTS * s->n_ptiles, g2 = work < 65536 ? (work > 0 ? work : 1) : 65536;
 			LFA_TRY(lfa_ev_record(s, LFA_EV_CORR_INDEXED));
-			hipLaunchKernelGGL((k_correct_fine<FINE_CAP, false>), dim3(g2), dim3(CORR_THREADS), 0, s->stream, s->ptiles, s->n_ptiles, cur.key,
-			                   cur.t[0], cur.t[1], cur.t[2], s->g, s->solid, s->tile_count, s->fine_start, (const float4 *)spos, mpc, ovf,
+			hipLaunchKernelGGL((k_correct_fine<FINE_CAP, false>), dim3(g2), dim3(CORR_THREADS), 0, s->stream, s->ptiles, s->n_ptiles, cur.pos,
+			                   s->g, s->solid, s->tile_count, s->fine_start, (const float4 *)spos, mpc, ovf,
 			                   (const uint8_t *)s->tile_clear, (const uint32_t *)nullptr);
 			LFA_LAUNCH_CHECK(s);
 			LFA_TRY(lfa_ev_record(s, LFA_EV_CORR_TILED));
 			hipLaunchKernelGGL((k_correct_fine<FINE_CAP_BIG, true>), dim3(std::min(CORR_BIG_SLICES * g2, 2048)), dim3(CORR_THREADS_BIG), 0, s->stream, s->ptiles,
-			                   s->n_ptiles, cur.key, cur.t[0], cur.t[1], cur.t[2], s->g, s->solid, s->tile_count, s->fine_start,
+			                   s->n_ptiles, cur.pos, s->g, s->solid, s->tile_count, s->fine_start,
 			                   (const float4 *)spos, mpc, ovf2, (const uint8_t *)s->tile_clear, (const uint32_t *)ovf);
 			LFA_LAUNCH_CHECK(s);
 		}
 		const uint32_t *fallback = ovf2;
-		hipLaunchKernelGGL(k_correct_collide, dim3((unsigned)std::min<size_t>((n + 255) / 256, 16384)), dim3(256), 0, s->stream, n, cur, cur.key, cur.t[0],
-		                   cur.t[1], cur.t[2], s->g, s->solid, s->tile_count, s->fine_start, (const float4 *)spos, mpc,
-		                   fallback, (const int *)s->tile_pslot, s->p_off, (const uint32_t *)oth.key);
+		hipLaunchKernelGGL(k_correct_collide, dim3((unsigned)std::min<size_t>((n + 255) / 256, 16384)), dim3(256), 0, s->stream, n, cur, cur.pos,
+		                   s->g, s->solid, s->tile_count, s->fine_start, (const float4 *)spos, mpc,
+		                   fallback, (const int *)s->tile_pslot, s->p_off, (const uint32_t *)s->bkey);
 		LFA_LAUNCH_CHECK(s);
 	}
 	if (migrate) LFA_TRY(lfa_dist_migrate(s));
@@ -1487,8 +1482,7 @@
 	s->move_pending = false;
 	if (!s->np_live && !s->dist) return LFA_OK;
 	LFA_TRY(correct_build_index(s));
-	ParticleSoA &cur = s->pb[s->cur], &oth = s->pb[s->cur ^ 1];
-	for (int d = 0; d < 3 && s->np_live; ++d) LFA_HIP(s, hipMemcpyAsync(oth.t[d], cur.t[d], s->np_live * 4, hipMemcpyDeviceToDevice, s->stream));
+	LFA_TRY(save_old_positions(s, s->np_live));
 	LFA_TRY(correct_apply(s, dt, false, false));
 	s->move_pending = true;
 	return LFA_OK;
@@ -1537,15 +1531,15 @@
 
 namespace {
 __global__ void __launch_bounds__(256)
-k_correct_undo(size_t n, const float4 *spos, const uint32_t *old_key, uint32_t *key, float *t0, float *t1, float *t2) {
+k_correct_undo(size_t n, const float4 *spos, const uint32_t *old_key, PosRec *pos) {
 	const size_t k = (size_t)blockIdx.x * blockDim.x + threadIdx.x;
 	if (k >= n) return;
 	const float4 rec = spos[k];
 	const uint32_t i = __float_as_uint(rec.w);
-	t0[i] = __uint_as_float(__float_as_uint(rec.x) & 0x3FFFFFFFu);
-	t1[i] = __uint_as_float(__float_as_uint(rec.y) & 0x3FFFFFFFu);
-	t2[i] = __uint_as_float(__float_as_uint(rec.z) & 0x3FFFFFFFu);
-	key[k] = old_key[k];
+	pos[i].t[0] = __uint_as_float(__float_as_uint(rec.x) & 0x3FFFFFFFu);
+	pos[i].t[1] = __uint_as_float(__float_as_uint(rec.y) & 0x3FFFFFFFu);
+	pos[i].t[2] = __uint_as_float(__float_as_uint(rec.z) & 0x3FFFFFFFu);
+	pos[k].key = old_key[k];
 }
 }
 
@@ -1559,9 +1553,9 @@
 	s->corr_begun = false;
 	const size_t n = s->np_live;
 	if (!n) return LFA_OK;
-	ParticleSoA &cur = s->pb[s->cur], &oth = s->pb[s->cur ^ 1];
+	ParticleSoA &cur = s->pb[s->cur];
 	hipLaunchKernelGGL(k_correct_undo, dim3((unsigned)((n + 255) / 256)), dim3(256), 0, s->stream, n, (const float4 *)correction_scratch(s),
-	                   (const uint32_t *)oth.key, cur.key, cur.t[0], cur.t[1], cur.t[2]);
+	                   (const uint32_t *)s->bkey, cur.pos);
 	LFA_LAUNCH_CHECK(s);
 	return LFA_OK;
 }
diff --git a/libfluid_amd/csrc/seed.hip b/libfluid_amd/csrc/seed.hip
--- a/libfluid_amd/csrc/seed.hip
+++ b/libfluid_amd/csrc/seed.hip
@@ -69,8 +69,7 @@
 	float tx, ty;
 	cell_and_fraction(x[0], ip.off[0], ip.h, g.nx, cx, tx);
 	cell_and_fraction(x[1], ip.off[1], ip.h, g.ny, cy, ty);
-	p.key[d] = blocked_index(g, cx, cy, cz);
-	p.t[0][d] = tx; p.t[1][d] = ty; p.t[2][d] = tz;
+	pos_store(p.pos, d, blocked_index(g, cx, cy, cz), tx, ty, tz);
 	p.v[0][d] = v0; p.v[1][d] = v1; p.v[2][d] = v2;
 	particle_zero_c_set_id(p, d, id);
 	if (pos_out) {
```

Result: faster. 5.593 billion (median of 6 runs) (+2.3%).
